# Algorithmic-Alignment-Lab/sco_py

Measured on AMD Instinct MI355X. Metric: SCO iters/sec (batch of N trajopt QPs), higher is better.
Workload: dtype f64

## Files before the change

### include/sco_hip.h

```cpp
#ifndef SCO_HIP_H
#define SCO_HIP_H

#ifdef __cplusplus
extern "C" {
#endif

#define SCO_OK              0
#define SCO_ERR_ARG        -1
#define SCO_ERR_DEVICE     -2
#define SCO_ERR_NO_GPU     -3
#define SCO_ERR_STATE      -4
#define SCO_ERR_CAPACITY   -5

#define SCO_QP_SOLVED                 1
#define SCO_QP_SOLVED_INACCURATE      2
#define SCO_QP_MAX_ITER_REACHED      -2
#define SCO_QP_PRIMAL_INFEASIBLE     -3
#define SCO_QP_PRIMAL_INFEASIBLE_INACCURATE 3
#define SCO_QP_DUAL_INFEASIBLE       -4
#define SCO_QP_DUAL_INFEASIBLE_INACCURATE   4
#define SCO_QP_NON_CVX               -7
#define SCO_QP_UNSOLVED             -10

const char *sco_last_error(void);
int sco_version(void);
int sco_device_count(int *count);


typedef struct sco_qp_settings {
  double rho;
  double sigma;
  double alpha;
  double eps_abs;
  double eps_rel;
  double eps_prim_inf;
  double eps_dual_inf;
  int max_iter;
  int check_termination;
  int scaling;
  int warm_start;
  int adaptive_rho;
  int adaptive_rho_interval;
  double adaptive_rho_tolerance;
} sco_qp_settings;

void sco_qp_default_settings(sco_qp_settings *s);

typedef struct sco_qp sco_qp;

int sco_qp_create(int device, int batch, int n, int m,
                  const int *P_colptr, const int *P_rowidx,
                  const int *A_colptr, const int *A_rowidx,
                  sco_qp **out);
int sco_qp_destroy(sco_qp *qp);

int sco_qp_load(sco_qp *qp, const double *P_val, const double *q,
                const double *A_val, const double *l, const double *u,
                const int *row_weight);

int sco_qp_set_bounds(sco_qp *qp, const double *l, const double *u);

int sco_qp_solve(sco_qp *qp, const sco_qp_settings *settings,
                 double *x, double *y, int *status, int *iters, double *resid);

int sco_qp_info(const sco_qp *qp, int info[4]);

int sco_qp_adaptive_info(sco_qp *qp, double *rho, int *updates);

int sco_qp_last_timing(const sco_qp *qp, double ms[2]);

#define SCO_QP_POLISH_OK       1
#define SCO_QP_POLISH_FAILED  -1
#define SCO_QP_POLISH_NOT_RUN  0
typedef struct sco_qp_polish_settings {
  double delta;
  int refine_iter;
} sco_qp_polish_settings;
void sco_qp_default_polish_settings(sco_qp_polish_settings *s);
int sco_qp_polish(sco_qp *qp, const sco_qp_polish_settings *s,
                  double *x, double *y, int *polish_status, double *resid);


typedef struct sco_sqp_params {
  double improve_ratio_threshold;
  double min_trust_region_size;
  double min_approx_improve;
  double trust_shrink_ratio;
  double trust_expand_ratio;
  double cnt_tolerance;
  double merit_coeff_increase_ratio;
  double initial_trust_region_size;
  double initial_penalty_coeff;
  int max_merit_coeff_increases;
  int compound_penalty;
  int duplicate_rows;
  int max_sqp_iters;
  int memoize_rounded;
  int warm_start_qps;
  int admm_slice;
} sco_sqp_params;

void sco_sqp_default_params(sco_sqp_params *p);

#define SCO_FAM_ARM_CIRCLES 1
#define SCO_FAM_ARM_REACH 2
#define SCO_FAM_POINT_CIRCLES 3
#define SCO_FAM_STATE_QUADRATIC 4
#define SCO_FAM_STATE_PROGRAM 5
#define SCO_OP_END 0
#define SCO_OP_X 1
#define SCO_OP_P 2
#define SCO_OP_C 3
#define SCO_OP_ADD 4
#define SCO_OP_SUB 5
#define SCO_OP_MUL 6
#define SCO_OP_DIV 7
#define SCO_OP_NEG 8
#define SCO_OP_SIN 9
#define SCO_OP_COS 10
#define SCO_OP_SQRT 11
#define SCO_OP_EXP 12
#define SCO_OP_SQUARE 13
#define SCO_PROGRAM_STACK 16
#define SCO_FAM_ARM_SPATIAL 7

#define SCO_FAM_FLAG_VEL_LIMITS 16
#define SCO_FAM_FLAG_JOINT_LIMITS 32
#define SCO_FAM_FLAG_EE_COST 64

#define SCO_FAM_FLAG_OBJ_PROGRAM 128

#define SCO_FAM_FLAG_ACC_COST 256

#define SCO_FAM_FLAG_OBJ_BLOCK 512

#define SCO_FAM_FLAG_OBJ_WIDE 1024

typedef struct sco_trajopt_desc {
  int batch;
  int dof;
  int horizon;
  int n_points;
  int n_obstacles;
  int family;
  int analytic_jac;
  int prox_count;
  int span;
  int n_eq_rows;
} sco_trajopt_desc;

typedef struct sco_sqp sco_sqp;

int sco_sqp_create(int device, const sco_trajopt_desc *desc, sco_sqp **out);
int sco_sqp_create_rows(int device, const sco_trajopt_desc *desc, int n_rows, const int *row_ptr, const int *col_idx,
                        const int *row_is_eq, sco_sqp **out);
int sco_sqp_load_linear_rows(sco_sqp *h, const double *vals, const double *rhs);
int sco_sqp_set_circle_rows(sco_sqp *h, int n_rows);
int sco_sqp_destroy(sco_sqp *h);

int sco_sqp_load(sco_sqp *h, const double *x0, const double *start, const double *goal,
                 const double *link_len, const int *point_link, const double *point_frac,
                 const double *obstacles);
int sco_sqp_load_target(sco_sqp *h, const double *target);
int sco_sqp_load_quadratic(sco_sqp *h, const double *Q, const double *a, const double *c);
int sco_sqp_load_spatial(sco_sqp *h,
    const double *joint_off,
    const double *joint_axis,
    const double *point_pos,
    const double *point_rad,
    const double *spheres);
int sco_sqp_load_program(sco_sqp *h, int n_words, const int *words, const int *row_ptr, int n_consts, const double *consts,
                         int n_params, const double *params);
int sco_sqp_load_program_steps(sco_sqp *h, int n_words, const int *words, const int *row_ptr, int n_consts, const double *consts,
                               int n_params, const double *params);
int sco_sqp_load_obj_weights(sco_sqp *h, const double *w);
int sco_sqp_load_acc_weights(sco_sqp *h, const double *a);
int sco_sqp_load_vel_limit(sco_sqp *h, const double *vmax);
int sco_sqp_load_joint_limits(sco_sqp *h, const double *lo, const double *hi);
int sco_sqp_load_ee_cost(sco_sqp *h, const double *weight, const double *target);

int sco_sqp_set_groups(sco_sqp *h, int n_groups, const unsigned int *block_mask);
int sco_sqp_fetch_groups(sco_sqp *h, unsigned int *nonconverged);
int sco_sqp_fetch_stalled_groups(sco_sqp *h, unsigned int *stalled);

int sco_sqp_solve(sco_sqp *h, const sco_sqp_params *params, const sco_qp_settings *qp_settings);

int sco_sqp_fetch(sco_sqp *h, double *x, int *success, int *sqp_iters, int *qp_solves,
                  long long *admm_iters, double *merit, double *max_violation);

#define SCO_SQP_FLAG_MEMO_FULL 1
#define SCO_SQP_FLAG_CAPPED 2
#define SCO_SQP_FLAG_TRACE_FULL 4
int sco_sqp_fetch_flags(sco_sqp *h, int *flags);
int sco_sqp_last_rounds(const sco_sqp *h, int *rounds);
int sco_sqp_last_launches(const sco_sqp *h, int *launches, int *groups);

int sco_sqp_last_tiers(const sco_sqp *h, double ms[2], long long iters[2], int launches[2]);

int sco_debug_sqp_mixed(const sco_sqp *h, int out[2]);
int sco_debug_mix_split(int live, int cus, int xcds, int slack, int per_cu);

int sco_debug_wv_gres_slot(int nstep, int pos, int out[5]);

int sco_debug_sqp_schedule(const int in[12], int plan[20], const int round_in[3], int round_out[8]);
int sco_debug_stage_sweep(int n, const double *begin_ms, const double *end_ms, const int *stage, double ms[5]);

int sco_debug_sqp_layout(const sco_trajopt_desc *desc, int n_rows, const int *row_ptr, const int *col_idx, const int *row_is_eq,
                         int dims[22], int sizes[15], int *ints, double *vals);
int sco_debug_sqp_check_program(const sco_trajopt_desc *desc, int n_circle_rows, int n_words, const int *words, const int *row_ptr,
                                int n_consts, int n_params);

int sco_debug_qp_launch_plan(const int *in, const double *tol, int *out);
int sco_debug_plan_tiers(int *mask);

int sco_debug_lanes(int device, int op, const double *a, const double *b, double *out_a, double *out_b);

int sco_sqp_trace(sco_sqp *h, int cap, double *trace, int *n_entries);

int sco_sqp_last_timing(const sco_sqp *h, double ms[5]);

#ifdef __cplusplus
}
#endif
#endif
```

### sco_py_amd/_lib.py

```python
import ctypes as C
import os

import numpy as np

from . import _build

SCO_OK = 0
ERR_NAMES = {-1: "SCO_ERR_ARG", -2: "SCO_ERR_DEVICE", -3: "SCO_ERR_NO_GPU",
             -4: "SCO_ERR_STATE", -5: "SCO_ERR_CAPACITY"}


class ScoHipError(RuntimeError):
    def __init__(self, code, msg):
        super().__init__("%s (%d): %s" % (ERR_NAMES.get(code, "SCO_ERR"), code, msg))
        self.code = code


class QpSettings(C.Structure):
    _fields_ = [
        ("rho", C.c_double), ("sigma", C.c_double), ("alpha", C.c_double),
        ("eps_abs", C.c_double), ("eps_rel", C.c_double),
        ("eps_prim_inf", C.c_double), ("eps_dual_inf", C.c_double),
        ("max_iter", C.c_int), ("check_termination", C.c_int), ("scaling", C.c_int),
        ("warm_start", C.c_int), ("adaptive_rho", C.c_int), ("adaptive_rho_interval", C.c_int),
        ("adaptive_rho_tolerance", C.c_double),
    ]


class PolishSettings(C.Structure):
    _fields_ = [("delta", C.c_double), ("refine_iter", C.c_int)]


class SqpParams(C.Structure):
    _fields_ = [
        ("improve_ratio_threshold", C.c_double), ("min_trust_region_size", C.c_double),
        ("min_approx_improve", C.c_double), ("trust_shrink_ratio", C.c_double),
        ("trust_expand_ratio", C.c_double), ("cnt_tolerance", C.c_double),
        ("merit_coeff_increase_ratio", C.c_double), ("initial_trust_region_size", C.c_double),
        ("initial_penalty_coeff", C.c_double),
        ("max_merit_coeff_increases", C.c_int), ("compound_penalty", C.c_int),
        ("duplicate_rows", C.c_int), ("max_sqp_iters", C.c_int),
        ("memoize_rounded", C.c_int), ("warm_start_qps", C.c_int), ("admm_slice", C.c_int),
    ]


class TrajoptDesc(C.Structure):
    _fields_ = [
        ("batch", C.c_int), ("dof", C.c_int), ("horizon", C.c_int), ("n_points", C.c_int),
        ("n_obstacles", C.c_int), ("family", C.c_int), ("analytic_jac", C.c_int),
        ("prox_count", C.c_int), ("span", C.c_int), ("n_eq_rows", C.c_int),
    ]


_DP = C.POINTER(C.c_double)
_IP = C.POINTER(C.c_int)
_LP = C.POINTER(C.c_longlong)

ABI = {
    "sco_last_error": (C.c_char_p, []),
    "sco_version": (C.c_int, []),
    "sco_device_count": (C.c_int, [_IP]),
    "sco_qp_default_settings": (None, [C.POINTER(QpSettings)]),
    "sco_qp_create": (C.c_int, [C.c_int, C.c_int, C.c_int, C.c_int, _IP, _IP, _IP, _IP, C.POINTER(C.c_void_p)]),
    "sco_qp_destroy": (C.c_int, [C.c_void_p]),
    "sco_qp_load": (C.c_int, [C.c_void_p, _DP, _DP, _DP, _DP, _DP, _IP]),
    "sco_qp_set_bounds": (C.c_int, [C.c_void_p, _DP, _DP]),
    "sco_qp_solve": (C.c_int, [C.c_void_p, C.POINTER(QpSettings), _DP, _DP, _IP, _IP, _DP]),
    "sco_qp_info": (C.c_int, [C.c_void_p, _IP]),
    "sco_qp_adaptive_info": (C.c_int, [C.c_void_p, _DP, _IP]),
    "sco_qp_last_timing": (C.c_int, [C.c_void_p, _DP]),
    "sco_qp_default_polish_settings": (None, [C.POINTER(PolishSettings)]),
    "sco_qp_polish": (C.c_int, [C.c_void_p, C.POINTER(PolishSettings), _DP, _DP, _IP, _DP]),
    "sco_sqp_default_params": (None, [C.POINTER(SqpParams)]),
    "sco_sqp_create": (C.c_int, [C.c_int, C.POINTER(TrajoptDesc), C.POINTER(C.c_void_p)]),
    "sco_sqp_create_rows": (C.c_int, [C.c_int, C.POINTER(TrajoptDesc), C.c_int, _IP, _IP, _IP, C.POINTER(C.c_void_p)]),
    "sco_sqp_destroy": (C.c_int, [C.c_void_p]),
    "sco_sqp_load": (C.c_int, [C.c_void_p, _DP, _DP, _DP, _DP, _IP, _DP, _DP]),
    "sco_sqp_load_target": (C.c_int, [C.c_void_p, _DP]),
    "sco_sqp_load_quadratic": (C.c_int, [C.c_void_p, _DP, _DP, _DP]),
    "sco_sqp_load_spatial": (C.c_int, [C.c_void_p, _DP, _DP, _DP, _DP, _DP]),
    "sco_sqp_load_program": (C.c_int, [C.c_void_p, C.c_int, _IP, _IP, C.c_int, _DP, C.c_int, _DP]),
    "sco_sqp_load_program_steps": (C.c_int, [C.c_void_p, C.c_int, _IP, _IP, C.c_int, _DP, C.c_int, _DP]),
    "sco_sqp_load_obj_weights": (C.c_int, [C.c_void_p, _DP]),
    "sco_sqp_load_acc_weights": (C.c_int, [C.c_void_p, _DP]),
    "sco_sqp_load_linear_rows": (C.c_int, [C.c_void_p, _DP, _DP]),
    "sco_sqp_set_circle_rows": (C.c_int, [C.c_void_p, C.c_int]),
    "sco_sqp_load_vel_limit": (C.c_int, [C.c_void_p, _DP]),
    "sco_sqp_load_joint_limits": (C.c_int, [C.c_void_p, _DP, _DP]),
    "sco_sqp_load_ee_cost": (C.c_int, [C.c_void_p, _DP, _DP]),
    "sco_sqp_set_groups": (C.c_int, [C.c_void_p, C.c_int, C.POINTER(C.c_uint)]),
    "sco_sqp_fetch_groups": (C.c_int, [C.c_void_p, C.POINTER(C.c_uint)]),
    "sco_sqp_fetch_stalled_groups": (C.c_int, [C.c_void_p, C.POINTER(C.c_uint)]),
    "sco_sqp_fetch_flags": (C.c_int, [C.c_void_p, _IP]),
    "sco_sqp_last_rounds": (C.c_int, [C.c_void_p, _IP]),
    "sco_sqp_last_launches": (C.c_int, [C.c_void_p, _IP, _IP]),
    "sco_sqp_last_tiers": (C.c_int, [C.c_void_p, _DP, _LP, _IP]),
    "sco_debug_sqp_mixed": (C.c_int, [C.c_void_p, _IP]),
    "sco_debug_mix_split": (C.c_int, [C.c_int, C.c_int, C.c_int, C.c_int, C.c_int]),
    "sco_debug_wv_gres_slot": (C.c_int, [C.c_int, C.c_int, _IP]),
    "sco_debug_sqp_schedule": (C.c_int, [_IP, _IP, _IP, _IP]),
    "sco_debug_stage_sweep": (C.c_int, [C.c_int, _DP, _DP, _IP, _DP]),
    "sco_debug_sqp_layout": (C.c_int, [C.POINTER(TrajoptDesc), C.c_int, _IP, _IP, _IP, _IP, _IP, _IP, _DP]),
    "sco_debug_sqp_check_program": (C.c_int, [C.POINTER(TrajoptDesc), C.c_int, C.c_int, _IP, _IP, C.c_int, C.c_int]),
    "sco_debug_qp_launch_plan": (C.c_int, [_IP, _DP, _IP]),
    "sco_debug_plan_tiers": (C.c_int, [_IP]),
    "sco_debug_lanes": (C.c_int, [C.c_int, C.c_int, _DP, _DP, _DP, _DP]),
    "sco_sqp_solve": (C.c_int, [C.c_void_p, C.POINTER(SqpParams), C.POINTER(QpSettings)]),
    "sco_sqp_fetch": (C.c_int, [C.c_void_p, _DP, _IP, _IP, _IP, _LP, _DP, _DP]),
    "sco_sqp_trace": (C.c_int, [C.c_void_p, C.c_int, _DP, _IP]),
    "sco_sqp_last_timing": (C.c_int, [C.c_void_p, _DP]),
}

_lib = None


def lib_path():
    return _build.LIB


def load():
    global _lib
    if _lib is not None:
        return _lib
    path = lib_path()
    if not os.path.exists(path):
        raise ScoHipError(-3, "libsco_hip.so not built (%s); run `python __graft_entry__.py` "
                              "or sco_py_amd._build.build() -- there is no CPU fallback" % path)
    lib = C.CDLL(path)
    for name, (res, args) in ABI.items():
        fn = getattr(lib, name)
        fn.restype = res
        fn.argtypes = args
    _lib = lib
    return lib


def check(code):
    if code != SCO_OK:
        msg = load().sco_last_error()
        raise ScoHipError(code, msg.decode() if msg else "")


def dptr(a):
    return None if a is None else a.ctypes.data_as(_DP)


def iptr(a):
    return None if a is None else a.ctypes.data_as(_IP)


def device_count():
    n = C.c_int(0)
    check(load().sco_device_count(C.byref(n)))
    return n.value


def default_qp_settings(**kw):
    s = QpSettings()
    load().sco_qp_default_settings(C.byref(s))
    for k, v in kw.items():
        if not hasattr(s, k):
            raise TypeError("unknown QP setting %r" % k)
        setattr(s, k, v)
    return s


def default_polish_settings(**kw):
    s = PolishSettings()
    load().sco_qp_default_polish_settings(C.byref(s))
    for k, v in kw.items():
        if not hasattr(s, k):
            raise TypeError("unknown polish setting %r" % k)
        setattr(s, k, v)
    return s


def default_sqp_params(**kw):
    p = SqpParams()
    load().sco_sqp_default_params(C.byref(p))
    for k, v in kw.items():
        if not hasattr(p, k):
            raise TypeError("unknown SQP parameter %r" % k)
        setattr(p, k, v)
    return p


class BatchedQP(object):

    def __init__(self, batch, n, m, Pp, Pi, Ap, Ai, device=0):
        self._h = C.c_void_p()
        self.batch, self.n, self.m = int(batch), int(n), int(m)
        self._pat = [np.ascontiguousarray(a, dtype=np.int32) for a in (Pp, Pi, Ap, Ai)]
        self.nnzP, self.nnzA = int(self._pat[0][-1]), int(self._pat[2][-1])
        check(load().sco_qp_create(device, self.batch, self.n, self.m,
                                   iptr(self._pat[0]), iptr(self._pat[1]),
                                   iptr(self._pat[2]), iptr(self._pat[3]), C.byref(self._h)))

    def close(self):
        if self._h:
            load().sco_qp_destroy(self._h)
            self._h = C.c_void_p()

    def __del__(self):
        try:
            self.close()
        except Exception:
            pass

    def _arr(self, a, shape, dtype=np.float64):
        a = np.ascontiguousarray(a, dtype=dtype)
        if a.shape != shape:
            raise ValueError("expected shape %r, got %r" % (shape, a.shape))
        return a

    def load(self, Pval, q, Aval, l, u, row_weight=None):
        B = self.batch
        Pval = self._arr(Pval, (B, self.nnzP)); q = self._arr(q, (B, self.n))
        Aval = self._arr(Aval, (B, self.nnzA)); l = self._arr(l, (B, self.m)); u = self._arr(u, (B, self.m))
        w = None if row_weight is None else self._arr(row_weight, (B, self.m), np.int32)
        check(load().sco_qp_load(self._h, dptr(Pval), dptr(q), dptr(Aval), dptr(l), dptr(u), iptr(w)))

    def set_bounds(self, l, u):
        l = self._arr(l, (self.batch, self.m)); u = self._arr(u, (self.batch, self.m))
        check(load().sco_qp_set_bounds(self._h, dptr(l), dptr(u)))

    def solve(self, settings=None):
        st = settings if settings is not None else default_qp_settings()
        B = self.batch
        x = np.zeros((B, self.n)); y = np.zeros((B, max(self.m, 1)))
        status = np.zeros(B, dtype=np.int32); iters = np.zeros(B, dtype=np.int32)
        resid = np.zeros((B, 2))
        check(load().sco_qp_solve(self._h, C.byref(st), dptr(x), dptr(y), iptr(status), iptr(iters), dptr(resid)))
        return x, y[:, : self.m], status, iters, resid

    def polish(self, settings=None):
        st = settings if settings is not None else default_polish_settings()
        B = self.batch
        x = np.zeros((B, self.n)); y = np.zeros((B, max(self.m, 1)))
        pstat = np.zeros(B, dtype=np.int32); resid = np.zeros((B, 2))
        check(load().sco_qp_polish(self._h, C.byref(st), dptr(x), dptr(y), iptr(pstat), dptr(resid)))
        return x, y[:, : self.m], pstat, resid

    def polish_info(self):
        lib = load()
        lib.sco_debug_polish_info.restype = C.c_int
        lib.sco_debug_polish_info.argtypes = [C.c_void_p, _DP, _IP]
        ms = np.zeros(4); k = np.zeros(self.batch, dtype=np.int32)
        check(lib.sco_debug_polish_info(self._h, dptr(ms), iptr(k)))
        return dict(active_ms=float(ms[0]), assemble_ms=float(ms[1]), factor_ms=float(ms[2]), solve_ms=float(ms[3])), k

    def info(self):
        out = np.zeros(4, dtype=np.int32)
        check(load().sco_qp_info(self._h, iptr(out)))
        return dict(n_elim=int(out[0]), n_core=int(out[1]), lds_admm=int(out[2]), ncpl=int(out[3]))

    def adaptive_info(self):
        rho = np.zeros(self.batch); upd = np.zeros(self.batch, dtype=np.int32)
        check(load().sco_qp_adaptive_info(self._h, dptr(rho), iptr(upd)))
        return rho, upd

    def last_timing(self):
        ms = np.zeros(2)
        check(load().sco_qp_last_timing(self._h, dptr(ms)))
        return dict(setup_ms=float(ms[0]), admm_ms=float(ms[1]))
```

### sco_py_amd/csrc/layout_wv.h

```cpp
#pragma once
#include "layout_qp.h"

#define WV_T 64
#define WV_MAXNS 4
#define WV_MAXNV 4
#ifndef WV_JREG
#define WV_JREG 1
#endif
SCO_HD constexpr bool wv_jreg(int NS, int BS) { return WV_JREG && NS * BS <= 28; }

SCO_HD inline size_t wv_tri(int i, int j) { return (size_t)i * (i + 1) / 2 + j; }

SCO_HD inline int wv_vidx(int npos, int pos, int k) { return (k >> 1) * 2 * npos + 2 * pos + (k & 1); }
SCO_HD inline int wv_gidx(int nstep, int pos, int i, int c) { return 64 * pos + 16 * (((c >> 1) + (pos > nstep ? 1 : 0)) & 3) + 2 * i + (c & 1); }

struct WvGresSlot { int pair, row, slot, vidx, eidx; };
SCO_HD inline WvGresSlot wv_gres_slot(int nstep, int pos) {
  const int hs = (nstep + 1) / 2, npos = 2 * nstep + 2;
  WvGresSlot s = {-1, -1, -1, -1, -1};
  if (pos < 0 || pos > 2 * nstep) return s;
  if (pos == nstep) { s.pair = 1; s.row = 0; s.slot = hs; }
  else {
    const int chain = pos > nstep ? 1 : 0, st = pos - (chain ? nstep + 1 : 0);
    s.pair = st >= hs ? 1 : 0; s.row = chain; s.slot = st - (s.pair ? hs : 0);
  }
  s.vidx = wv_vidx(npos, pos, 0); s.eidx = pos * 8;
  return s;
}
struct WvTab {
  int pos, hrow, hbrow, hevar, heidx, hepos, hbpos, hjpos, vvar, vrow, vpos, vpk, vpkm, vpkp, vpd, vpm, vpp, xrow, xpos, xpk, total;
  int lrow, lplo, lphi;
};
SCO_HD inline WvTab wv_tab_layout(int NS, int NV, int NL = 0) {
  WvTab t; int o = 0;
  t.pos = o; o += 1;
  t.hrow = o; o += NS; t.hbrow = o; o += NS; t.hevar = o; o += NS; t.heidx = o; o += NS; t.hepos = o; o += NS; t.hbpos = o; o += NS;
  t.hjpos = o; o += NS * 8;
  t.vvar = o; o += NV; t.vrow = o; o += NV; t.vpos = o; o += NV; t.vpk = o; o += NV; t.vpkm = o; o += NV; t.vpkp = o; o += NV;
  t.vpd = o; o += NV * 8; t.vpm = o; o += NV; t.vpp = o; o += NV;
  t.xrow = o; o += 1; t.xpos = o; o += 1; t.xpk = o; o += 1;
  t.lrow = o; o += NV * NL; t.lplo = o; o += NV * NL; t.lphi = o; o += NV * NL;
  t.total = o;
  return t;
}
SCO_HD inline int wv_cst_h(int q) { return 3 * q; }
SCO_HD inline int wv_cst_v(int NS, int v) { return 3 * NS + 13 * v; }
SCO_HD inline int wv_cst_x(int NS, int NV) { return 3 * NS + 13 * NV; }
SCO_HD inline int wv_cst_l(int NS, int NV, int i) { return 3 * NS + 13 * NV + 1 + i; }
SCO_HD constexpr int wv_cst_slots(int NS, int NV, int nl) { return 3 * NS + 13 * NV + 1 + nl; }
SCO_HD constexpr int wv_ck_h(int q) { return 3 * q; }
SCO_HD constexpr int wv_ck_v(int NS, int v) { return 3 * NS + 5 * v; }
SCO_HD constexpr int wv_ck_x(int NS, int NV) { return 3 * NS + 5 * NV; }
SCO_HD constexpr int wv_ck_slots(int NS, int NV) { return 3 * NS + 5 * NV + 1; }
SCO_HD constexpr bool wv_link_regs(int BS) { return BS != 7; }
```

### sco_py_amd/csrc/qp_debug.cpp

```cpp
#include "qp_tier_plans.h"
#include "layout_fast.h"
#include "layout_wv.h"

#include <algorithm>
#include <cstring>

static QpPlan g_dbg_plan;
extern "C" int sco_debug_plan_build(int n, int m, const int *Pp, const int *Pi, const int *Ap, const int *Ai,
                                    int allow_elim, int *sizes) {
  int rc = qp_plan_build(n, m, Pp, Pi, Ap, Ai, allow_elim, g_dbg_plan);
  if (rc) return SCO_ERR_ARG;
  const QpPlan &p = g_dbg_plan;
  sizes[0] = p.n_e; sizes[1] = p.n_c; sizes[2] = p.ncpl; sizes[3] = p.nS;
  sizes[4] = (int)p.cp_row.size(); sizes[5] = (int)p.sa_row.size(); sizes[6] = (int)p.ss_k1.size();
  sizes[7] = (int)p.Fi.size();
  return SCO_OK;
}
extern "C" int sco_debug_rl_plan(int *info) {
  RlHost rh;
  const bool ok = rl_plan_build(g_dbg_plan, rh, qp_create_env());
  info[0] = ok ? 1 : 0; info[1] = rh.CW; info[2] = rh.TR; info[3] = rh.TC; info[4] = (int)rh.lds_bytes; info[5] = rh.merged ? 1 : 0; info[6] = rh.aligned ? 1 : rh.lay8 ? 2 : 0; info[7] = rh.NS;
  return SCO_OK;
}
extern "C" int sco_debug_fast_plan(int *info) {
  FastHost fh;
  const bool ok = fast_plan_build(g_dbg_plan, fh);
  const int nq = fast_rows_per_thread(g_dbg_plan.m);
  info[0] = ok ? 1 : 0; info[1] = fh.TR; info[2] = fh.TC; info[3] = (fh.capped && nq == 2) ? 1 : 0; info[4] = nq; info[5] = (int)fh.lds_bytes;
  return SCO_OK;
}
extern "C" int sco_debug_reg_plan(int *info) {
  RegHost rh;
  int CW = 0, RW = 0, PX = 0;
  const bool ok = reg_caps_for(g_dbg_plan, &CW, &RW, &PX) && reg_plan_build(g_dbg_plan, CW, RW, PX, rh);
  info[0] = ok ? 1 : 0; info[1] = rh.TR; info[2] = rh.TC; info[3] = rh.CW; info[4] = rh.RW; info[5] = rh.PX; info[6] = (int)rh.lds_bytes;
  return SCO_OK;
}
static bool dbg_wv_plan(bool allow_links, int *info, WvHost &wh) {
  const bool ok = wv_plan_build(g_dbg_plan, wh, allow_links);
  info[0] = ok ? 1 : 0; info[1] = wh.bs; info[2] = wh.nb; info[3] = wh.lpb; info[4] = wh.BS; info[5] = wh.NS; info[6] = wh.NV;
  info[7] = wh.NSTEP; info[8] = (int)wh.lds_bytes; info[9] = wh.n_extra;
  return ok;
}
extern "C" int sco_debug_wv_plan(int *info) {
  WvHost wh;
  dbg_wv_plan(false, info, wh);
  return SCO_OK;
}
extern "C" int sco_debug_wv_link_plan(int *info) {
  WvHost wh;
  dbg_wv_plan(true, info, wh);
  info[10] = wh.n_link; info[11] = wh.NL; info[12] = wh.per_cu; info[13] = wh.why;
  return SCO_OK;
}
extern "C" int sco_debug_wv_stack_plan(int *info) {
  WvHost wh;
  dbg_wv_plan(true, info, wh);
  info[10] = wh.n_link; info[11] = wh.NL; info[12] = wh.per_cu; info[13] = wh.why; info[14] = wh.n_stack;
  return SCO_OK;
}
extern "C" int sco_debug_bt_plan(int *info) {
  BigHost bh; BtHost th;
  const bool ok = g_dbg_plan.n_c <= 1024 && big_plan_build(g_dbg_plan, bh) && bt_plan_build(g_dbg_plan, bh, th, qp_create_env().no_mfma);
  info[0] = ok ? 1 : 0; info[1] = th.bs; info[2] = th.nb; info[3] = th.use_mfma ? 1 : 0; info[4] = th.mf_why; info[5] = (int)th.lds_bytes;
  return SCO_OK;
}
extern "C" int sco_debug_plan_tiers(int *mask) {
  const QpPlan &p = g_dbg_plan;
  if (!mask || p.n <= 0) return SCO_ERR_ARG;
  QpTiers t;
  std::string err;
  if (const int rc = qp_choose_tiers(p.n, p.m, p.Pp.data(), p.Pi.data(), p.Ap.data(), p.Ai.data(), qp_create_env(), t, &err)) {
    sco_set_error(err);
    return rc;
  }
  *mask = qp_tier_mask(t);
  return SCO_OK;
}
extern "C" int sco_debug_plan_get(const char *name, int *out, int cap) {
  const QpPlan &p = g_dbg_plan;
  const std::vector<int> *v = nullptr;
#define F(x) if (!strcmp(name, #x)) v = &p.x;
  F(Rp) F(Rj) F(Rpos) F(Fp) F(Fi) F(Fpos) F(Pdiag) F(elim_var) F(core_var) F(elim_of) F(core_of)
  F(e_ptr) F(pair_core) F(pair_elim) F(cp_ptr) F(cp_row) F(cp_pa) F(cp_pe) F(a_ptr) F(a_pair)
  F(s_a) F(s_b) F(s_ppos) F(sa_ptr) F(sa_row) F(sa_pa) F(sa_pb) F(ss_ptr) F(ss_k1) F(ss_k2) F(ss_e)
#undef F
  if (!v) return SCO_ERR_ARG;
  if ((int)v->size() > cap) return SCO_ERR_CAPACITY;
  std::copy(v->begin(), v->end(), out);
  return (int)v->size();
}
extern "C" int sco_debug_wv_gres_slot(int nstep, int pos, int out[5]) {
  if (!out || nstep <= 0) return SCO_ERR_ARG;
  const WvGresSlot s = wv_gres_slot(nstep, pos);
  out[0] = s.pair; out[1] = s.row; out[2] = s.slot; out[3] = s.vidx; out[4] = s.eidx;
  return SCO_OK;
}
```

### sco_py_amd/csrc/qp_tier.cpp

```cpp
#include "qp_tier.h"

#include <algorithm>
#include <climits>
#include <cstdlib>

QpCreateEnv qp_create_env() {
  auto on = [](const char *name) { const char *v = getenv(name); return v && v[0] == '1'; };
  QpCreateEnv e;
  e.factor_cholesky = on("SCO_QP_FACTOR_CHOLESKY"); e.no_elim = on("SCO_QP_NO_ELIM");
  e.force_big = on("SCO_QP_FORCE_BIG"); e.no_bt = on("SCO_QP_NO_BT");
  e.no_rl = on("SCO_QP_NO_RL"); e.no_wv = on("SCO_QP_NO_WV"); e.no_reg = on("SCO_QP_NO_REG"); e.no_fast = on("SCO_QP_NO_FAST");
  e.no_mfma = on("SCO_QP_NO_MFMA");
  e.rl_closed = on("SCO_QP_RL_ALIGNED") || on("SCO_QP_RL_CLOSED"); e.rl_lay8 = on("SCO_QP_RL_LAY8");
  { const char *v = getenv("SCO_QP_RL_SPLIT"); e.rl_split_off = v && v[0] == '0'; }
  e.debug_plan = getenv("SCO_DEBUG_PLAN") != nullptr;
  return e;
}

int sco_wv_min_live(int cus, bool adaptive) {
  const char *e = getenv("SCO_WV_MIN_PER_CU");
  if (!e && adaptive) return INT_MAX;
  const double live = (e ? atof(e) : 2.75) * (cus > 0 ? cus : 256);
  return live >= (double)INT_MAX ? INT_MAX : (int)live;
}

int sco_qp_adaptive_interval(const sco_qp_settings *st) {
  if (st->adaptive_rho_interval > 0) {
    if (st->check_termination > 0)
      return std::max(1, (st->adaptive_rho_interval + st->check_termination / 2) / st->check_termination) * st->check_termination;
    return st->adaptive_rho_interval;
  }
  return st->check_termination > 0 ? 4 * st->check_termination : 100;
}

const char *qp_launch_err_text(int err) {
  switch (err) {
    case QP_ERR_WINDOW: return "sco_qp_launch_sliced: launch window not supported by this handle's tier";
    case QP_ERR_ADAPT_DENSE: return "adaptive_rho: the dense form of the global-memory tier cannot park a solve";
    case QP_ERR_ADAPT_SETTINGS: return "adaptive_rho needs adaptive_rho_tolerance > 1 and check_termination > 0";
    case QP_ERR_MIXED: return "sco_qp_launch_sliced: mixed round not supported by this handle or its side window is malformed";
  }
  return "";
}

bool qp_supports_windows(const QpLaunchIn &in) {
  if (in.adaptive_rho) return false;
  if (in.use_big) return in.use_bt;
  return in.kern == QP_K_RL && !in.factor_cholesky;
}

static QpLaunchPlan plan_error(QpLaunchPlan p, int rc, int err) { p.rc = rc; p.err = err; return p; }

QpLaunchPlan qp_launch_plan(const QpLaunchIn &in) {
  QpLaunchPlan p;
  const bool adaptive = in.adaptive_rho != 0;
  if (in.window && (!qp_supports_windows(in) || in.b0 < 0 || in.nb <= 0 || in.b0 + in.nb > in.batch))
    return plan_error(p, SCO_ERR_STATE, QP_ERR_WINDOW);
  if (adaptive) {
    if (in.use_big && !in.use_bt) return plan_error(p, SCO_ERR_CAPACITY, QP_ERR_ADAPT_DENSE);
    if (!(in.adaptive_rho_tolerance > 1.0) || in.check_termination <= 0) return plan_error(p, SCO_ERR_ARG, QP_ERR_ADAPT_SETTINGS);
  }
  const bool can_park = in.use_big ? in.use_bt : true;
  if (!can_park || in.check_termination <= 0 || (in.slice <= 0 && !adaptive)) {
    p.slice = 0;
  } else {
    const int want = in.slice <= 0 ? in.max_iter : in.slice;
    p.slice = std::max(1, (want + in.check_termination - 1) / in.check_termination) * in.check_termination;
  }
  p.nwg = in.window ? in.nb : in.batch;
  if (adaptive) {
    sco_qp_settings st{};
    st.adaptive_rho_interval = in.adaptive_rho_interval; st.check_termination = in.check_termination;
    p.ad_interval = sco_qp_adaptive_interval(&st);
  }
  p.mixed = in.window && in.tier == 3;
  if (p.mixed) {
    const bool at_end = in.side_b0 == in.b0 || in.side_b0 + in.side_nb == in.b0 + in.nb;
    if (!in.use_wv || in.kern != QP_K_RL || adaptive || p.slice <= 0 || !in.has_list || in.side_nb <= 0 || in.side_nb >= in.nb ||
        !at_end || in.side_slices <= 0 || !in.side_ready)
      return plan_error(p, SCO_ERR_STATE, QP_ERR_MIXED);
  }
  p.wv_now = in.use_wv && !(adaptive && in.wv_links) && (in.window && in.tier ? in.tier >= 2 : p.nwg >= in.wv_min);
  p.rho_init = adaptive && in.mask != QP_MASK_NONE;
  p.route = in.use_big ? (in.use_bt ? QP_ROUTE_BIG_BT : QP_ROUTE_BIG_DENSE) : QP_ROUTE_ONCHIP;
  if (p.route != QP_ROUTE_ONCHIP) { p.wv_now = false; return p; }
  p.need = p.wv_now ? (p.mixed ? QP_NEED_SIDE : QP_NEED_NONE) : (in.use_wv ? QP_NEED_WINDOW : QP_NEED_NONE);
  p.cholesky = in.factor_cholesky;
  const int nb4 = (in.n_c + 3) / 4, ntiles = nb4 * (nb4 + 1) / 2;
  p.sweep_nt = ntiles <= SCO_FACTOR_BLOCK ? 1 : ntiles <= 2 * SCO_FACTOR_BLOCK ? 2 : 3;
  switch (in.kern) {
    case QP_K_RL: p.admm = p.mixed ? QP_ADMM_MIXED : p.wv_now ? QP_ADMM_WV_RL : QP_ADMM_RL; break;
    case QP_K_REG: p.admm = QP_ADMM_REG; break;
    case QP_K_FAST: p.admm = QP_ADMM_FAST; break;
    default: p.admm = QP_ADMM_GENERIC;
  }
  return p;
}

// ... 21 lines not shown
```

### sco_py_amd/csrc/qp_tier.h

```cpp
#pragma once
#include "../../include/sco_hip.h"

#define SCO_FACTOR_BLOCK 1024

struct QpCreateEnv {
  bool factor_cholesky = false;
  bool no_elim = false;
  bool force_big = false;
  bool no_bt = false;
  bool no_rl = false, no_wv = false, no_reg = false, no_fast = false;
  bool no_mfma = false;
  bool rl_closed = false;
  bool rl_lay8 = false;
  bool rl_split_off = false;
  bool debug_plan = false;
};
QpCreateEnv qp_create_env();

int sco_wv_min_live(int cus, bool adaptive = false);
int sco_qp_adaptive_interval(const sco_qp_settings *st);

enum QpKernel { QP_K_RL = 0, QP_K_REG = 1, QP_K_FAST = 2, QP_K_GENERIC = 3 };
enum QpMaskKind { QP_MASK_ARRAY = 0, QP_MASK_ALL = 1, QP_MASK_NONE = 2 };

struct QpLaunchIn {
  int kern = QP_K_GENERIC;
  bool use_big = false, use_bt = false;
  bool use_wv = false;
  bool wv_links = false;
  bool factor_cholesky = false;
  int batch = 0, n_c = 0;
  int cus = 0;
  int adaptive_rho = 0, adaptive_rho_interval = 0, check_termination = 0, max_iter = 0;
  double adaptive_rho_tolerance = 0.0;
  int slice = 0;
  int mask = QP_MASK_ARRAY;
  int wv_min = 0;
  bool window = false;
  int b0 = 0, nb = 0, tier = 0;
  bool has_list = false;
  int side_b0 = 0, side_nb = 0, side_slices = 0;
  bool side_ready = false;
};

enum QpLaunchErr { QP_ERR_NONE = 0, QP_ERR_WINDOW, QP_ERR_ADAPT_DENSE, QP_ERR_ADAPT_SETTINGS, QP_ERR_MIXED };
const char *qp_launch_err_text(int err);
enum QpRoute { QP_ROUTE_BIG_DENSE = 0, QP_ROUTE_BIG_BT = 1, QP_ROUTE_ONCHIP = 2 };
enum QpNeed { QP_NEED_NONE = 0, QP_NEED_WINDOW = 1, QP_NEED_SIDE = 2 };
enum QpAdmmSeq { QP_ADMM_GENERIC = 0, QP_ADMM_FAST, QP_ADMM_REG, QP_ADMM_RL, QP_ADMM_WV_RL, QP_ADMM_MIXED };

struct QpLaunchPlan {
  int rc = SCO_OK, err = QP_ERR_NONE;
  int slice = -1;
  int nwg = 0;
  int ad_interval = 0;
  bool rho_init = false;
  int route = QP_ROUTE_ONCHIP;
  bool wv_now = false, mixed = false;
  int need = QP_NEED_NONE;
  bool cholesky = false;
  int sweep_nt = 1;
  int admm = QP_ADMM_GENERIC;
};
QpLaunchPlan qp_launch_plan(const QpLaunchIn &in);
bool qp_supports_windows(const QpLaunchIn &in);
```

### sco_py_amd/csrc/qp_tier_plans.h

```cpp
#pragma once
#include <cstddef>
#include <string>
#include <vector>

#include "../../include/sco_hip.h"
#include "layout_qp.h"
#include "qp_plan.h"
#include "qp_tier.h"

void sco_set_error(const std::string &msg);

struct SellHost {
  int nitems = 0, total = 0;
  std::vector<int> base, width, src;
  std::vector<unsigned short> idx;
};
struct FastHost { SellHost Ac, Ar, Ca, Ce; int TR = 1, TC = 2; bool capped = false; size_t lds_doubles = 0, lds_bytes = 0; };
bool fast_plan_build(const QpPlan &pl, FastHost &fh);

struct RegHost {
  int TR = 1, TC = 2, CW = 0, RW = 0, PX = 0;
  SellHost Ac, Ar, Ca, Ce;
  size_t lds_bytes = 0;
  std::vector<int> role;
  std::vector<unsigned short> off;
};
int reg_caps_for(const QpPlan &pl, int *CW, int *RW, int *PX);
size_t reg_static_lds();
bool reg_plan_build(const QpPlan &pl, int CW, int RW, int PX, RegHost &rh);

struct RlHost {
  int TR = 1, TC = 2, CW = 12;
  int pcw = 0;
  int zpos = 0;
  bool merged = false;
  bool aligned = false;
  bool split = false;
  bool lay8 = false;
  int NS = 2;
  SellHost Ac, Ar[3];
  size_t lds_bytes = 0;
  std::vector<unsigned short> off;
  std::vector<int> role, pc_ptr, pc_pos, pc_core;
};
size_t rl_reported_static_lds();
bool rl_plan_build(const QpPlan &pl, RlHost &rh, const QpCreateEnv &env);

#define SCO_WV_PER_CU 4
struct WvHost {
  int bs = 0, nb = 0, mid = 0, lpb = 0, n_extra = 0;
  int BS = 8, NS = 1, NV = 1, NSTEP = 4;
  int cst_slots = 0;
  size_t g_doubles = 0, lds_doubles = 0, lds_bytes = 0;
  std::vector<int> tab;
  int n_link = 0, NL = 0, per_cu = SCO_WV_PER_CU, why = 0;
  int n_stack = 0;
};
#define WV_NL 2
enum WvWhy { WV_OK = 0, WV_WHY_OTHER = 1, WV_WHY_LINKS_OFF = 2, WV_WHY_THIRD_LINK = 3, WV_WHY_SAME_BLOCK = 4, WV_WHY_FAR_BLOCKS = 5,
             WV_WHY_INDEX = 6, WV_WHY_THREE_CORE = 7, WV_WHY_LDS = 8, WV_WHY_SHAPE = 9,
             WV_WHY_STACKED = 10 };
bool wv_plan_build(const QpPlan &pl, WvHost &wh, bool allow_links);

struct BigHost {
  std::vector<int> row_elim, row_epos, er_ptr, er_row, free_rows, pc_ptr, pc_pos, pc_core;
  size_t ws_doubles = 0;
};
bool big_plan_build(const QpPlan &pl, BigHost &bh);
struct BtHost {
  int bs = 0, nb = 0, nchunks = 0, npart = 0;
  bool use_part = false;
  std::vector<int> cent;
  size_t blk_doubles = 0, ws_doubles = 0, lds_bytes = 0;
  std::vector<int> ch_desc, it;
  bool use_mfma = false;
  int mf_why = 0;
  std::vector<int> mf_id, mf_h0, mf_h1;
};
bool bt_plan_build(const QpPlan &pl, const BigHost &bh, BtHost &th, bool no_mfma);

struct QpTiers {
  QpPlan plan;
  size_t lds_setup = 0, lds_admm = 0;
  bool factor_cholesky = false;
  bool use_big = false, use_bt = false;
  int kern = QP_K_GENERIC;
  bool use_wv = false;
  BigHost big;
  BtHost bt;
  RlHost rl;
  WvHost wv;
  RegHost reg;
  FastHost fast;
};
int qp_choose_tiers(int n, int m, const int *Pp, const int *Pi, const int *Ap, const int *Ai, const QpCreateEnv &env, QpTiers &t,
                    std::string *err);
int qp_tier_mask(const QpTiers &t);
```

### sco_py_amd/csrc/sco_admm_wv.hip

```cpp
#include <algorithm>
#include <cstdio>
#include <cstdlib>
#include <cstring>
#include <type_traits>

#include "sco_admm_check.h"
#include "layout_wv.h"

#ifndef WV_PD
#define WV_PD 3
#endif
typedef double d2 __attribute__((ext_vector_type(2)));

#ifndef WV_KEEP
#define WV_KEEP 8
#endif
#ifndef WV_VARIANT
#define WV_VARIANT 0
#endif
#ifndef WV_GRES
#define WV_GRES 1
#endif
#ifndef WV_ROWS_EARLY
#define WV_ROWS_EARLY 1
#endif
#ifndef WV_MV_INIT
#define WV_MV_INIT 1
#endif
#ifndef WV_HANDOVER
#define WV_HANDOVER 1
#endif
#if WV_VARIANT == 1
#define WV_FMAC_DPP(acc, w, g, k) asm("v_fmac_f64 %0, %1, %2" : "+v"(acc) : "v"(w), "v"(g))
#endif

__device__ __forceinline__ double wv_recip(double x) { return x != 0.0 ? __builtin_amdgcn_rcp(x) : 0.0; }

int wv_upload(const WvHost &wh, int batch, int n, int m, std::vector<void *> &allocs, WvDev &wd) {
  void *p = nullptr;
  SCO_HIP(hipMalloc(&p, wh.tab.size() * sizeof(int))); allocs.push_back(p);
  SCO_HIP(hipMemcpy(p, wh.tab.data(), wh.tab.size() * sizeof(int), hipMemcpyHostToDevice)); wd.tab = (const int *)p;
  SCO_HIP(hipMalloc(&p, (size_t)batch * wh.g_doubles * sizeof(double))); allocs.push_back(p); wd.G = (double *)p;
  SCO_HIP(hipMalloc(&p, (size_t)batch * wh.cst_slots * 64 * sizeof(double))); allocs.push_back(p); wd.cst = (double *)p;
  SCO_HIP(hipMalloc(&p, (size_t)batch * sizeof(double))); allocs.push_back(p); wd.wc = (double *)p;
  SCO_HIP(hipMalloc(&p, (size_t)batch * sizeof(int))); allocs.push_back(p); wd.ok = (int *)p;
  SCO_HIP(hipMemset(p, 0, (size_t)batch * sizeof(int)));
  SCO_HIP(hipMalloc(&p, (size_t)batch * sizeof(int))); allocs.push_back(p); wd.rl_need = (int *)p;
  SCO_HIP(hipMemset(p, 0, (size_t)batch * sizeof(int)));
  SCO_HIP(hipMalloc(&p, sizeof(unsigned long long))); allocs.push_back(p); wd.it_count = (unsigned long long *)p;
  SCO_HIP(hipMemset(p, 0, sizeof(unsigned long long)));
  SCO_HIP(hipMalloc(&p, (size_t)batch * sizeof(int))); allocs.push_back(p); wd.pflag = (int *)p;
  SCO_HIP(hipMemset(p, 0, (size_t)batch * sizeof(int)));
  SCO_HIP(hipMalloc(&p, (size_t)batch * sizeof(int))); allocs.push_back(p); wd.w_ready = (int *)p;
  SCO_HIP(hipMemset(p, 0, (size_t)batch * sizeof(int)));
  SCO_HIP(hipMalloc(&p, (size_t)batch * (size_t)(n + m) * sizeof(double))); allocs.push_back(p); wd.scr = (double *)p;
  return SCO_OK;
}

struct WvArgs {
  int n, m, n_e, n_c, nnzA, nnzP, max_iter, check, slice;
  int b0; const int *list;
  int bs, nb, mid, lpb, n_extra, NS, NV, NSTEP, cst_slots, NL; size_t g_doubles;
  double rho, sigma, alpha, eps_abs, eps_rel, eps_prim_inf, eps_dual_inf;
  const int *tab;
  double *G, *cst, *wc, *scr; int *ok, *rl_need, *w_ready, *pflag; unsigned long long *it_count;
  const double *As, *Ps, *qs, *ls, *us, *rhov, *kee_inv, *cscale, *D, *E, *S;
  const int *w, *active, *setup_active;
  const int *Ap, *Ai, *Rp, *Rj, *Rpos, *Fp, *Fi, *Fpos;
  double *x, *y, *resid; int *status, *iters, *prog;
  double *sx, *sz, *sy, *st, *sg;
  int ablate;
  int warm, ad_interval; double ad_tol; double *rho_b; int *rflag, *smask, *nupd;
};

__device__ __forceinline__ double wv_wmax(double v) { return wave_reduce_all<true>(v); }
__device__ __forceinline__ double wv_wsum(double v) { return wave_reduce_all<false>(v); }
template <bool DIRECT>
__device__ __forceinline__ void wv_meet(double vlast, int chain, double &vA, double &vB) {
  if (DIRECT) {
    vA = vlast; vB = vlast;
    lane_swap<16>(vA, vB);
  } else {
    lane_u2 lo, hi;
    lane_swap_halves<16>(vlast, vlast, lo, hi);
    const double vother = chain ? __hiloint2double((int)hi.x, (int)lo.x) : __hiloint2double((int)hi.y, (int)lo.y);
    vA = chain ? vother : vlast; vB = chain ? vlast : vother;
  }
}
#define WV_BIG (SCO_INFTY * SCO_MIN_SCALING)

template <int LNK>
__global__ __launch_bounds__(WV_T) void qp_wv_factor_kernel(WvArgs a) {
  const int g = blockIdx.x, lane = threadIdx.x;
  const int b = a.list ? a.list[g + a.b0] : g + a.b0;
  if (b < 0) return;
  if (a.setup_active && !a.setup_active[b]) { if (lane == 0) a.rl_need[b] = 0; return; }
  const int n = a.n, m = a.m, bs = a.bs, nb = a.nb, mid = a.mid, NS = a.NS, NV = a.NV, NSTEP = a.NSTEP;
  const WvTab T = wv_tab_layout(NS, NV, LNK);
  const int *tab = a.tab;
  const double *ls = a.ls + (size_t)b * m, *us = a.us + (size_t)b * m, *rho = a.rhov + (size_t)b * m;
  const int *w = a.w + (size_t)b * m;
  const double *D = a.D + (size_t)b * n, *E = a.E + (size_t)b * m, *Ps = a.Ps + (size_t)b * a.nnzP;
  double *cst = a.cst + (size_t)b * a.cst_slots * 64;
  const double rho_base = a.rho_b ? a.rho_b[b] : a.rho;
  int bad = 0, wk = 0, offd = 0;
  for (int q = 0; q < NS; q++) { const int h = tab[(T.hrow + q) * 64 + lane]; if (h >= 0) wk = max(wk, w[h]); }
  wk = (int)wv_wmax((double)wk);
  for (int q = 0; q < NS; q++) {
    const int h = tab[(T.hrow + q) * 64 + lane], br = tab[(T.hbrow + q) * 64 + lane], ev = tab[(T.hevar + q) * 64 + lane];
    double eh = 0.0, eb = 0.0, de = 0.0;
    if (h >= 0) {
      if (!(ls[h] < -WV_BIG) || rho[h] != rho_base || w[h] != wk) bad = 1;
      if (!(us[br] > WV_BIG) || ls[br] != 0.0 || rho[br] != rho_base || w[br] != 1) bad = 1;
      eh = E[h]; eb = E[br]; de = D[ev];
    }
    double *c = cst + (size_t)wv_cst_h(q) * 64 + lane;
    c[0] = h >= 0 ? 1.0 / eh : 0.0; c[64] = h >= 0 ? 1.0 / eb : 0.0; c[128] = h >= 0 ? 1.0 / de : 0.0;
  }
  for (int v = 0; v < NV; v++) {
    const int var = tab[(T.vvar + v) * 64 + lane], r0 = tab[(T.vrow + v) * 64 + lane];
    double *c = cst + (size_t)wv_cst_v(NS, v) * 64 + lane;
    if (r0 >= 0 && (rho[r0] != rho_base || w[r0] != 1)) bad = 1;
    c[0] = var >= 0 ? 1.0 / D[var] : 0.0;
    c[64] = r0 >= 0 ? 1.0 / E[r0] : 0.0;
    const int pm = tab[(T.vpm + v) * 64 + lane], pp = tab[(T.vpp + v) * 64 + lane];
    c[2 * 64] = pm >= 0 ? Ps[pm] : 0.0; c[3 * 64] = pp >= 0 ? Ps[pp] : 0.0;
    const int kown = (tab[(T.vpk + v) * 64 + lane] / (2 * (2 * NSTEP + 2)) << 1) | (tab[(T.vpk + v) * 64 + lane] & 1);
    double pdiag = 0.0;
    for (int k = 0; k < 8; k++) {
      const int pd = tab[(T.vpd + v * 8 + k) * 64 + lane];
      const double pv = pd >= 0 ? Ps[pd] : 0.0;
      c[(5 + k) * 64] = pv;
      if (var >= 0 && k == kown) pdiag = pv; else if (var >= 0 && pv != 0.0) offd = 1;
    }
    c[4 * 64] = pdiag;
  }
  {
    const int xr = tab[T.xrow * 64 + lane];
    double *c = cst + (size_t)wv_cst_x(NS, NV) * 64 + lane;
    c[0] = xr >= 0 ? 1.0 / E[xr] : 0.0;
  }
  if constexpr (LNK > 0) {
    for (int i = 0; i < NV * LNK; i++) {
      const int lr = tab[(T.lrow + i) * 64 + lane];
      if (lr >= 0 && (rho[lr] != rho_base || w[lr] != 1)) bad = 1;
      cst[(size_t)wv_cst_l(NS, NV, i) * 64 + lane] = lr >= 0 ? 1.0 / E[lr] : 0.0;
    }
  }
  bad = (int)wv_wmax((double)bad); offd = (int)wv_wmax((double)offd);
  if (lane == 0) a.pflag[b] = offd;
  if (lane == 0) { a.ok[b] = !bad; a.rl_need[b] = bad; a.w_ready[b] = bad; a.wc[b] = (double)wk; }
  if (bad) return;
  const double *S = a.S + (size_t)b * a.n_c * a.n_c;
  double *G = a.G + (size_t)b * a.g_doubles;
  const int npos = 2 * NSTEP + 2;
  double *ef = G + (size_t)npos * 64, *en = ef + npos * 8, *em = en + npos * 8;
  for (size_t t = lane; t < a.g_doubles; t += WV_T) G[t] = 0.0;
  __threadfence_block(); __syncthreads();
  const int i = lane >> 3, j = lane & 7;
  auto Sblk = [&](int t) -> double {
    if (i >= bs || j >= bs) return i == j ? 1.0 : 0.0;
    const int ca = t * bs + max(i, j), cb = t * bs + min(i, j);
    return S[wv_tri(ca, cb)];
  };
  auto Soff = [&](int t, int k) -> double {
    return (k < bs && t >= 0 && t + 1 < nb) ? S[wv_tri((t + 1) * bs + k, t * bs + k)] : 0.0;
  };
  auto invert = [&](double M) -> double {
    for (int p = 0; p < 8; p++) {
      const double piv = __shfl(M, p * 8 + p), rowp = __shfl(M, p * 8 + j), colp = __shfl(M, i * 8 + p);
      const double inv = 1.0 / piv;
      if (i == p && j == p) M = inv;
      else if (i == p) M = rowp * inv;
      else if (j == p) M = -colp * inv;
      else M = M - colp * rowp * inv;
    }
    return M;
  };
  double Gmid_corr = 0.0;
  for (int chain = 0; chain < 2; chain++) {
    const int len = chain ? nb - 1 - mid : mid, p0 = chain ? 2 * NSTEP + 1 - len : NSTEP - len;
    double Gp = 0.0;
    for (int s = 0; s < len; s++) {
      const int t = chain ? nb - 1 - s : s, p = p0 + s;
      const int tl = chain ? t : t - 1;
      const double ei = s > 0 ? Soff(tl, i) : 0.0, ej = s > 0 ? Soff(tl, j) : 0.0;
      const double M = Sblk(t) - ei * Gp * ej;
      Gp = invert(M);
      G[wv_gidx(NSTEP, p, i, j)] = Gp;
      const int tn = chain ? t - 1 : t;
      if (lane < 8) { ef[p * 8 + lane] = s > 0 ? Soff(tl, lane) : 0.0; en[p * 8 + lane] = Soff(tn, lane); }
    }
    if (len > 0) {
      const int tl = chain ? mid : mid - 1;
      Gmid_corr += Soff(tl, i) * Gp * Soff(tl, j);
    }
  }
// ... 5 lines not shown
}


__device__ __forceinline__ double wv_min(double a, double b) { double r; asm("v_min_f64 %0, %1, %2" : "=v"(r) : "v"(a), "v"(b)); return r; }
__device__ __forceinline__ double wv_max(double a, double b) { double r; asm("v_max_f64 %0, %1, %2" : "=v"(r) : "v"(a), "v"(b)); return r; }

template <int BS> struct WvRow { d2 a, b, c; d2 d; };
template <int BS>
__device__ __forceinline__ WvRow<BS> wv_row(const double *p, const double *pd) {
  WvRow<BS> r;
  r.a = *(const d2 *)p; r.b = *(const d2 *)(p + 16); r.c = *(const d2 *)(p + 32);
  if (BS > 7) r.d = *(const d2 *)pd; else { r.d.x = pd[0]; r.d.y = 0.0; }
  return r;
}

#define WV_DPP_STEP(acc, g, k) "v_fmac_f64_dpp " acc ", %2, " g " row_newbcast:" #k " row_mask:0xf bank_mask:0xf\n\t"
#define WV_DPP_CHAIN7 WV_DPP_STEP("%0", "%3", 0) WV_DPP_STEP("%1", "%4", 1) WV_DPP_STEP("%0", "%5", 2) WV_DPP_STEP("%1", "%6", 3) \
                      WV_DPP_STEP("%0", "%7", 4) WV_DPP_STEP("%1", "%8", 5) WV_DPP_STEP("%0", "%9", 6)
#define WV_G7 "v"(g0.x), "v"(g0.y), "v"(g1.x), "v"(g1.y), "v"(g2.x), "v"(g2.y), "v"(g3.x)

template <int BS, bool ZERO, bool INIT>
__device__ __forceinline__ double wv_matvec(double init, double w, const WvRow<BS> &g) {
  const d2 g0 = g.a, g1 = g.b, g2 = g.c, g3 = g.d;
#if WV_VARIANT == 1
  double acc = ZERO ? 0.0 : init, acc2 = 0.0;
  WV_FMAC_DPP(acc, w, g0.x, 0); WV_FMAC_DPP(acc2, w, g0.y, 1);
  WV_FMAC_DPP(acc, w, g1.x, 2); WV_FMAC_DPP(acc2, w, g1.y, 3);
  WV_FMAC_DPP(acc, w, g2.x, 4); WV_FMAC_DPP(acc2, w, g2.y, 5); WV_FMAC_DPP(acc, w, g3.x, 6);
  if (BS > 7) WV_FMAC_DPP(acc2, w, g3.y, 7);
#else
  double acc = ZERO ? 0.0 : init, acc2 = 0.0;
  if (!INIT) {
    if (BS > 7) asm("s_nop 1\n\t" WV_DPP_CHAIN7 WV_DPP_STEP("%1", "%10", 7) : "+v"(acc), "+v"(acc2) : "v"(w), WV_G7, "v"(g3.y));
    else asm("s_nop 1\n\t" WV_DPP_CHAIN7 : "+v"(acc), "+v"(acc2) : "v"(w), WV_G7);
  } else if (BS > 7) {
    if (ZERO) asm("v_mov_b64 %1, 0\n\tv_mov_b64 %0, 0\n\t" WV_DPP_CHAIN7 WV_DPP_STEP("%1", "%10", 7) : "=&v"(acc), "=&v"(acc2) : "v"(w), WV_G7, "v"(g3.y));
    else asm("v_mov_b64 %1, 0\n\tv_mov_b64 %0, %11\n\t" WV_DPP_CHAIN7 WV_DPP_STEP("%1", "%10", 7) : "=&v"(acc), "=&v"(acc2) : "v"(w), WV_G7, "v"(g3.y), "v"(init));
  } else {
    if (ZERO) asm("v_mov_b64 %1, 0\n\tv_mov_b64 %0, 0\n\t" WV_DPP_CHAIN7 : "=&v"(acc), "=&v"(acc2) : "v"(w), WV_G7);
    else asm("v_mov_b64 %1, 0\n\tv_mov_b64 %0, %10\n\t" WV_DPP_CHAIN7 : "=&v"(acc), "=&v"(acc2) : "v"(w), WV_G7, "v"(init));
  }
#endif
  return acc + acc2;
}
#undef WV_G7
#undef WV_DPP_CHAIN7
#undef WV_DPP_STEP

#define WV_SYNC() do { __builtin_amdgcn_fence(__ATOMIC_ACQ_REL, "wavefront"); __builtin_amdgcn_wave_barrier(); } while (0)

template <typename T>
__device__ __forceinline__ const T *wv_opaque(const T *p) { asm volatile("" : "+v"(p)); return p; }

template <int NV, int LNK, bool REG> struct WvLinks {
  static constexpr int N = NV * LNK;
  double alo[REG ? N : 1], ahi[REG ? N : 1], l[REG ? N : 1], u[REG ? N : 1], z[N], y[N], d[N], xp[NV];
  double *lkl;
  __device__ __forceinline__ void consts(int v, double (&la)[LNK], double (&lh)[LNK], double (&ll)[LNK], double (&lu)[LNK]) const {
#pragma unroll
    for (int s = 0; s < LNK; s++) {
      const int i = v * LNK + s;
      if constexpr (REG) { la[s] = alo[i]; lh[s] = ahi[i]; ll[s] = l[i]; lu[s] = u[i]; }
      else {
        const d2 ca = *(const d2 *)(lkl + (2 * i) * 128), cb = *(const d2 *)(lkl + (2 * i + 1) * 128);
        la[s] = ca.x; lh[s] = ca.y; ll[s] = cb.x; lu[s] = cb.y;
      }
    }
  }
};
template <int NV, bool REG> struct WvLinks<NV, 0, REG> {};

constexpr bool wv_gres_fits(int BS, int NS, int NV, int NSTEP, int LPB, int EXT) {
  return WV_GRES != 0 && NSTEP % 2 == 0 && !(BS == 7 && (EXT & 2));
}
constexpr bool wv_rows_early(int BS, int NS, int NV, int NSTEP, int LPB, int EXT, int LNK) {
  return WV_ROWS_EARLY != 0 && LNK == 0 && LPB > 0 && !(EXT & 2);
}
constexpr int wv_slots(int BS, int NS, int NV, int NSTEP, int LPB, int EXT, int LNK) {
  int sl = (WV_MV_INIT ? 1 : 0) | (WV_HANDOVER ? 4 : 0);
  if (LNK > 0) sl &= 1;
  if (BS == 7 && LPB == 3 && EXT == 1) sl &= 4;
  return sl;
}
template <int BS, int NS, int NV, int NSTEP, int LPB, int EXT, int LNK>
__global__ __launch_bounds__(WV_T) void qp_admm_wv_kernel(WvArgs a) {
  constexpr bool ADAPT = (EXT & 2) != 0;
  static_assert(!(LNK > 0 && ADAPT), "adaptive rho on link patterns stays on the row-local kernel (qp_launch_plan)");
  constexpr int NLK = LNK > 0 ? NV * LNK : 1;
  constexpr bool LREG = wv_link_regs(BS);
  constexpr bool GRES = wv_gres_fits(BS, NS, NV, NSTEP, LPB, EXT);
  constexpr bool EARLY = wv_rows_early(BS, NS, NV, NSTEP, LPB, EXT, LNK);
  constexpr int SL = wv_slots(BS, NS, NV, NSTEP, LPB, EXT, LNK);
  constexpr int HS = (NSTEP + 1) / 2, H2 = NSTEP - HS;
  const int g = blockIdx.x, lane = threadIdx.x;
  const int b = a.list ? a.list[g + a.b0] : g + a.b0;
  if (b < 0 || (a.active && !a.active[b])) return;
  if (!a.ok[b]) return;
#ifdef WV_ABLATE
  const int ablate = a.ablate;
#else
  constexpr int ablate = 0;
#endif
  const int n = a.n, m = a.m, lpb = LPB > 0 ? LPB : a.lpb;
  constexpr int NPOS = 2 * NSTEP + 2;
  constexpr bool JREG = wv_jreg(NS, BS);
  constexpr int oG = 0, oEF = oG + NPOS * 64, oEN = oEF + NPOS * 8, oEM = oEN + NPOS * 8, oR = oEM + 8, oXT = oR + NPOS * 8,
                oXC = oXT + NPOS * 8, oEX = oXC + NPOS * 8, oLK = oEX + NPOS * 8, oJ = oLK + (LNK > 0 ? NPOS * 8 : 0),
                oPART = oJ + (JREG ? 0 : NS * 512);
  constexpr int NVEC = LNK > 0 ? 5 : 4;
  extern __shared__ __attribute__((aligned(16))) double lds[];
  const int *tab0 = a.tab;
  constexpr int oPOS = 0, oHROW = 1, oHBROW = oHROW + NS, oHEVAR = oHBROW + NS, oHEIDX = oHEVAR + NS, oHEPOS = oHEIDX + NS,
                oHBPOS = oHEPOS + NS, oHJPOS = oHBPOS + NS, oVVAR = oHJPOS + 8 * NS, oVROW = oVVAR + NV, oVPOS = oVROW + NV,
                oVPK = oVPOS + NV, oVPKM = oVPK + NV, oVPKP = oVPKM + NV, oXROW = oVPKP + NV + 8 * NV + 2 * NV, oXPOS = oXROW + 1,
                oXPK = oXPOS + 1, oLROW = oXPK + 1, oLPLO = oLROW + NV * LNK, oLPHI = oLPLO + NV * LNK;
  const double *As = a.As + (size_t)b * a.nnzA, *qs = a.qs + (size_t)b * n, *lsg = a.ls + (size_t)b * m, *usg = a.us + (size_t)b * m;
  const double *cstg0 = a.cst + (size_t)b * a.cst_slots * 64 + lane;
  double rho_in = a.rho;
  if constexpr (ADAPT) {
    rho_in = a.rho_b[b];
    if (lane == 0) { a.rflag[b] = 0; a.smask[b] = 0; }
  }
  const double rho0 = rho_in, rinv0 = 1.0 / rho0, wc = a.wc[b], rw = wc * rho0;
  const double sigma = a.sigma, alpha = a.alpha, oma = 1.0 - alpha;
  const double cscale = a.cscale[b], cinv = 1.0 / cscale;
  const int it0 = a.slice > 0 ? a.prog[b] : 0;
  const bool resume = it0 > 0;
  const double *sxg = a.sx + (size_t)b * n, *szg = a.sz + (size_t)b * m, *syg = a.sy + (size_t)b * m;

  {
    const double *Gg = a.G + (size_t)b * a.g_doubles;
    for (int t = lane; t < oR; t += WV_T) lds[t] = Gg[t];
    for (int t = lane; t < NVEC * NPOS * 8; t += WV_T) lds[oR + t] = 0.0;
    for (int t = lane; t < NPOS * lpb * 8; t += WV_T) lds[oPART + t] = 0.0;
  }
  constexpr bool CKG = LNK > 0 && !LREG;
  const int oCK = oPART + NPOS * lpb * 8;
  double *const ckl = lds + oCK + lane;
  if constexpr (!CKG) {
#pragma unroll
    for (int q = 0; q < NS; q++)
#pragma unroll
      for (int k = 0; k < 3; k++) ckl[(wv_ck_h(q) + k) * 64] = cstg0[(wv_cst_h(q) + k) * 64];
#pragma unroll
    for (int v = 0; v < NV; v++)
#pragma unroll
      for (int k = 0; k < 5; k++) ckl[(wv_ck_v(NS, v) + k) * 64] = cstg0[(wv_cst_v(NS, v) + k) * 64];
    ckl[wv_ck_x(NS, NV) * 64] = cstg0[wv_cst_x(NS, NV) * 64];
  }
#define CKH(q, k) (CKG ? wv_opaque(cstg0)[(wv_cst_h(q) + (k)) * 64] : ckl[(wv_ck_h(q) + (k)) * 64])
#define CKV(v, k) (CKG ? wv_opaque(cstg0)[(wv_cst_v(NS, v) + (k)) * 64] : ckl[(wv_ck_v(NS, v) + (k)) * 64])
#define CKX (CKG ? wv_opaque(cstg0)[wv_cst_x(NS, NV) * 64] : ckl[wv_ck_x(NS, NV) * 64])
#define CKL(i) wv_opaque(cstg0)[wv_cst_l(NS, NV, i) * 64]
  const int pos_r = tab0[oPOS * 64 + lane];
  double *const xt_p = lds + oXT + pos_r * 2;
  const int nslot2 = NPOS * lpb * 2;
  double *const part_p = lds + oPART + (pos_r * lpb + (lane & 15) % lpb) * 2;
  double *const jl_p = lds + oJ + lane * 2;
  bool h_on[NS];
  double h_ae[NS], h_ab[NS], h_u[NS], h_q[NS], h_kinv[NS], h_z[NS], h_y[NS], h_zb[NS], h_yb[NS], h_xe[NS], h_ge[NS];
  double hJ[JREG ? NS : 1][8];
#pragma unroll
  for (int q = 0; q < NS; q++) {
    const int h = tab0[(oHROW + q) * 64 + lane], br = tab0[(oHBROW + q) * 64 + lane], ev = tab0[(oHEVAR + q) * 64 + lane];
    const bool on = h >= 0;
    h_on[q] = on;
    h_ae[q] = on ? As[tab0[(oHEPOS + q) * 64 + lane]] : 0.0;
    h_ab[q] = on ? As[tab0[(oHBPOS + q) * 64 + lane]] : 0.0;
    h_u[q] = on ? usg[h] : 0.0;
    h_q[q] = on ? qs[ev] : 0.0;
    h_kinv[q] = on ? a.kee_inv[(size_t)b * a.n_e + tab0[(oHEIDX + q) * 64 + lane]] : 0.0;
    h_z[q] = on && resume ? szg[h] : 0.0; h_y[q] = on && resume ? syg[h] : 0.0;
    h_zb[q] = on && resume ? szg[br] : 0.0; h_yb[q] = on && resume ? syg[br] : 0.0;
    h_xe[q] = on && resume ? sxg[ev] : 0.0; h_ge[q] = 0.0;
#pragma unroll
    for (int k = 0; k < 4; k++) {
      const int j0 = on ? tab0[(oHJPOS + q * 8 + 2 * k) * 64 + lane] : -1, j1 = on ? tab0[(oHJPOS + q * 8 + 2 * k + 1) * 64 + lane] : -1;
      d2 v; v.x = j0 >= 0 ? As[j0] : 0.0; v.y = j1 >= 0 ? As[j1] : 0.0;
      if (JREG) { hJ[q][2 * k] = v.x; hJ[q][2 * k + 1] = v.y; }
      else *(d2 *)(jl_p + (q * 4 + k) * 128) = v;
    }
  }
  double *v_p[NV];
  const double *v_pp[NV];
  bool v_on[NV], v_r0on[NV];
  int v_pkm[NV], v_pkp[NV];
  double v_x[NV], v_q[NV], v_a[NV], v_l[NV], v_u[NV], v_z[NV], v_y[NV];
#pragma unroll
  for (int v = 0; v < NV; v++) {
    const int var = tab0[(oVVAR + v) * 64 + lane], r0 = tab0[(oVROW + v) * 64 + lane];
    const int vix = tab0[(oVPK + v) * 64 + lane], vk = ((vix / (2 * NPOS)) << 1) | (vix & 1), vpos = (vix % (2 * NPOS)) >> 1;
    v_on[v] = var >= 0; v_p[v] = lds + oXT + vix;
    v_pp[v] = lds + oPART + (vk >> 1) * nslot2 + vpos * lpb * 2 + (vk & 1);
    v_q[v] = var >= 0 ? qs[var] : 0.0; v_x[v] = var >= 0 && resume ? sxg[var] : 0.0;
    v_a[v] = r0 >= 0 ? As[tab0[(oVPOS + v) * 64 + lane]] : 0.0;
    v_l[v] = r0 >= 0 ? lsg[r0] : 0.0; v_u[v] = r0 >= 0 ? usg[r0] : 0.0;
    v_z[v] = r0 >= 0 && resume ? szg[r0] : 0.0; v_y[v] = r0 >= 0 && resume ? syg[r0] : 0.0;
    v_r0on[v] = r0 >= 0; v_pkm[v] = tab0[(oVPKM + v) * 64 + lane]; v_pkp[v] = tab0[(oVPKP + v) * 64 + lane];
  }
  const int x_row = tab0[oXROW * 64 + lane];
  double *const x_p = lds + oXT + tab0[oXPK * 64 + lane];
  const double x_a = x_row >= 0 ? As[tab0[oXPOS * 64 + lane]] : 0.0, x_l = x_row >= 0 ? lsg[x_row] : 0.0, x_u = x_row >= 0 ? usg[x_row] : 0.0;
  const double x_rho = x_row >= 0 ? a.rhov[(size_t)b * m + x_row] : 1.0, x_rinv = 1.0 / x_rho, x_w = x_row >= 0 ? (double)a.w[(size_t)b * m + x_row] : 0.0;
  double x_z = x_row >= 0 && resume ? szg[x_row] : 0.0, x_y = x_row >= 0 && resume ? syg[x_row] : 0.0;
  WvLinks<NV, LNK, LREG> lk;
  constexpr int NL1 = LNK > 0 ? LNK : 1;
  if constexpr (LNK > 0) {
    lk.lkl = lds + oCK + lane * 2;
#pragma unroll
    for (int i = 0; i < NLK; i++) {
      const int lr = tab0[(oLROW + i) * 64 + lane], lph = tab0[(oLPHI + i) * 64 + lane];
      d2 ca, cb;
      ca.x = lr >= 0 ? As[tab0[(oLPLO + i) * 64 + lane]] : 0.0; ca.y = lr >= 0 && lph >= 0 ? As[lph] : 0.0;
      cb.x = lr >= 0 ? lsg[lr] : 0.0; cb.y = lr >= 0 ? usg[lr] : 0.0;
      if constexpr (LREG) { lk.alo[i] = ca.x; lk.ahi[i] = ca.y; lk.l[i] = cb.x; lk.u[i] = cb.y; }
      else { *(d2 *)(lk.lkl + (2 * i) * 128) = ca; *(d2 *)(lk.lkl + (2 * i + 1) * 128) = cb; }
      lk.z[i] = lr >= 0 && resume ? szg[lr] : 0.0; lk.y[i] = lr >= 0 && resume ? syg[lr] : 0.0;
    }
  }
  const int srow = lane >> 4, k8 = lane & 7, chain = srow & 1, half = GRES ? srow >> 1 : 0;
  const bool sw_store = (GRES || srow < 2) && (lane & 15) < 8;
  const int pos0 = (chain ? NSTEP + 1 : 0) + half * HS;
  const WvGresSlot sl0 = wv_gres_slot(NSTEP, pos0);
  const double *const sw_g = lds + oG + pos0 * 64 + k8 * 2 + (chain ? 16 : 0);
  const double *const sw_gd = lds + oG + pos0 * 64 + k8 * 2 + (chain ? 0 : 48);
  double *const sw_v = lds + oR + sl0.vidx + wv_vidx(NPOS, 0, k8);
  const double *const sw_e = lds + oEF + sl0.eidx + k8;
  const double *const md_g = lds + oG + NSTEP * 64 + k8 * 2;
  double *const md_v = lds + oR + wv_vidx(NPOS, NSTEP, k8);
  const double *const md_e = lds + oEF + NSTEP * 8 + k8;
  WvRow<BS> gr[GRES ? HS : 1], gmd;
  auto load_g = [&]() {
    static_assert(!GRES || H2 == HS, "the second half recomputes the first on its idle rows: both halves need the same step count");
#pragma unroll
    for (int s = 0; s < HS; s++) gr[s] = wv_row<BS>(sw_g + s * 64, sw_gd + s * 64);
    gmd = wv_row<BS>(md_g, md_g + 48);
  };
  WV_SYNC();

  double c_ndy = 0.0, c_lhs = 0.0, c_ndx = 0.0, c_qdx = 0.0;
  const int pdense = (ablate & 32) ? 1 : a.pflag[b];
  struct { double h[NS], b[NS], e[NS], r0[NV], var[NV], x; } dsv;
  auto rows = [&](auto mode_tag) {
    constexpr int MODE = decltype(mode_tag)::value;
    double xt[8], xtx = 0.0, xtv[NV];
    if (MODE) {
      const d2 a0 = *(const d2 *)xt_p, a1 = *(const d2 *)(xt_p + 2 * NPOS), a2 = *(const d2 *)(xt_p + 4 * NPOS), a3 = *(const d2 *)(xt_p + 6 * NPOS);
      xtx = x_p[0];
#pragma unroll
      for (int v = 0; v < NV; v++) xtv[v] = v_p[v][0];
      xt[0] = a0.x; xt[1] = a0.y; xt[2] = a1.x; xt[3] = a1.y; xt[4] = a2.x; xt[5] = a2.y; xt[6] = a3.x; xt[7] = a3.y;
    }
    if constexpr (LNK > 0) {
      if (MODE) {
#pragma unroll
        for (int v = 0; v < NV; v++) lk.xp[v] = lds[oXT + v_pkp[v]];
      }
    }
    double part[8] = {0, 0, 0, 0, 0, 0, 0, 0};
    d2 jn0, jn1, jn2, jn3;
    if (!JREG) { const d2 *jp = (const d2 *)jl_p; jn0 = jp[0]; jn1 = jp[64]; jn2 = jp[128]; jn3 = jp[192]; }
#pragma unroll
    for (int q = 0; q < NS; q++) {
      double J[8];
      if (JREG) {
#pragma unroll
        for (int k = 0; k < 8; k++) J[k] = hJ[q][k];
      } else {
        J[0] = jn0.x; J[1] = jn0.y; J[2] = jn1.x; J[3] = jn1.y; J[4] = jn2.x; J[5] = jn2.y; J[6] = jn3.x; J[7] = jn3.y;
        if (q + 1 < NS) { const d2 *jp = (const d2 *)(jl_p + (q + 1) * 512); jn0 = jp[0]; jn1 = jp[64]; jn2 = jp[128]; jn3 = jp[192]; }
      }
      const double ae = h_ae[q], ab = h_ab[q], kinv = h_kinv[q];
      const double c2 = rw * ae;
      if (MODE) {
        double s = J[0] * xt[0];
#pragma unroll
        for (int k = 1; k < BS; k++) s = __builtin_fma(J[k], xt[k], s);
        const double xte = h_ge[q] - (kinv * c2) * s;
        const double zth = __builtin_fma(ae, xte, s), ztb = ab * xte;
        {
          const double zr = alpha * zth + oma * h_z[q];
          const double zn = wv_min(zr + rinv0 * h_y[q], h_u[q]);
          const double dy = rho0 * (zr - zn);
          h_y[q] += dy; h_z[q] = zn;
          if (MODE == 2) {
            const double dc = fmax(dy, 0.0);
            c_ndy = fmax(c_ndy, wv_recip(CKH(q, 0)) * fabs(dc)); c_lhs += wc * (h_u[q] * dc);
            dsv.h[q] = dc;
          }
        }
        {
          const double zr = alpha * ztb + oma * h_zb[q];
          const double zn = wv_max(zr + rinv0 * h_yb[q], 0.0);
          const double dy = rho0 * (zr - zn);
          h_yb[q] += dy; h_zb[q] = zn;
          if (MODE == 2) {
            const double dc = fmin(dy, 0.0);
            c_ndy = fmax(c_ndy, wv_recip(CKH(q, 1)) * fabs(dc));
            dsv.b[q] = dc;
          }
        }
        const double xo = h_xe[q], xn = alpha * xte + oma * xo;
        h_xe[q] = xn;
        if (MODE == 2) {
          const double dx = xn - xo;
          c_ndx = fmax(c_ndx, wv_recip(CKH(q, 2)) * fabs(dx)); c_qdx += h_q[q] * dx;
          dsv.e[q] = dx;
        }
      }
      const double th = wc * (rho0 * h_z[q] - h_y[q]);
      const double tb = rho0 * h_zb[q] - h_yb[q];
      const double rhs = ae * th + ab * tb + (sigma * h_xe[q] - h_q[q]);
      const double ge = rhs * kinv;
      h_ge[q] = ge;
      const double tp = th - c2 * ge;
#pragma unroll
      for (int k = 0; k < BS; k++) part[k] = __builtin_fma(J[k], tp, part[k]);
    }
    {
      d2 v0, v1, v2, v3;
      v0.x = part[0]; v0.y = part[1]; v1.x = part[2]; v1.y = part[3]; v2.x = part[4]; v2.y = part[5]; v3.x = part[6]; v3.y = BS > 7 ? part[7] : 0.0;
      *(d2 *)part_p = v0; *(d2 *)(part_p + nslot2) = v1; *(d2 *)(part_p + 2 * nslot2) = v2; *(d2 *)(part_p + 3 * nslot2) = v3;
    }
    {
      if (MODE) {
        const double xtc = xtx;
        const double zt = x_a * xtc, zr = alpha * zt + oma * x_z;
        const double zn = wv_min(wv_max(zr + x_rinv * x_y, x_l), x_u);
        const double dy = x_rho * (zr - zn);
        x_y += dy; x_z = zn;
        if (MODE == 2) {
          const double d1 = upper_is_infinite(x_u) ? fmin(dy, 0.0) : dy, dc = lower_is_infinite(x_l) ? fmax(d1, 0.0) : d1;
          c_ndy = fmax(c_ndy, wv_recip(CKX) * fabs(dc)); c_lhs += x_w * (x_u * fmax(dc, 0.0) + x_l * fmin(dc, 0.0));
          dsv.x = dc;
        }
      }
      const double t = x_w * (x_rho * x_z - x_y);
      if (x_row >= 0) x_p[oEX - oXT] = x_a * t;
    }
    double s_ex[NV], s_pt[NV][LPB > 0 ? LPB : 1];
    if constexpr (EARLY) {
      WV_SYNC();
#pragma unroll
      for (int v = 0; v < NV; v++) {
        s_ex[v] = v_p[v][oEX - oXT];
#pragma unroll
        for (int s2 = 0; s2 < LPB; s2++) s_pt[v][s2] = v_pp[v][s2 * 2];
      }
      __builtin_amdgcn_sched_barrier(0);
    }
    double own[NV];
#pragma unroll
    for (int v = 0; v < NV; v++) {
      if (MODE) {
        const double xtc = xtv[v];
        const double zt = v_a[v] * xtc, zr = alpha * zt + oma * v_z[v];
        const double zn = wv_min(wv_max(zr + rinv0 * v_y[v], v_l[v]), v_u[v]);
        const double dy = rho0 * (zr - zn);
        v_y[v] += dy; v_z[v] = zn;
        const double xo = v_x[v], xn = alpha * xtc + oma * xo;
        v_x[v] = xn;
        if (MODE == 2) {
          const double d1 = upper_is_infinite(v_u[v]) ? fmin(dy, 0.0) : dy, dc = lower_is_infinite(v_l[v]) ? fmax(d1, 0.0) : d1;
          if (v_r0on[v]) { c_ndy = fmax(c_ndy, wv_recip(CKV(v, 1)) * fabs(dc)); c_lhs += v_u[v] * fmax(dc, 0.0) + v_l[v] * fmin(dc, 0.0); }
          dsv.r0[v] = dc;
          const double dx = xn - xo;
          if (v_on[v]) { c_ndx = fmax(c_ndx, wv_recip(CKV(v, 0)) * fabs(dx)); c_qdx += v_q[v] * dx; }
          dsv.var[v] = dx;
        }
      }
      const double t0 = rho0 * v_z[v] - v_y[v];
      own[v] = v_a[v] * t0 + (sigma * v_x[v] - v_q[v]);
      if constexpr (LNK > 0) {
        double ps = 0.0, la[NL1], lh[NL1], ll[NL1], lu[NL1];
        lk.consts(v, la, lh, ll, lu);
#pragma unroll
        for (int s = 0; s < LNK; s++) {
          const int i = v * LNK + s;
          if (MODE) {
            const double zt = __builtin_fma(lh[s], lk.xp[v], la[s] * xtv[v]), zr = alpha * zt + oma * lk.z[i];
            const double zn = wv_min(wv_max(zr + rinv0 * lk.y[i], ll[s]), lu[s]);
            const double dy = rho0 * (zr - zn);
            lk.y[i] += dy; lk.z[i] = zn;
            if (MODE == 2) {
              const double d1 = upper_is_infinite(lu[s]) ? fmin(dy, 0.0) : dy, dc = lower_is_infinite(ll[s]) ? fmax(d1, 0.0) : d1;
              c_ndy = fmax(c_ndy, wv_recip(CKL(i)) * fabs(dc)); c_lhs += lu[s] * fmax(dc, 0.0) + ll[s] * fmin(dc, 0.0);
              lk.d[i] = dc;
            }
          }
          const double t = rho0 * lk.z[i] - lk.y[i];
          own[v] = __builtin_fma(la[s], t, own[v]); ps = __builtin_fma(lh[s], t, ps);
        }
        lds[oLK + v_pkp[v]] = ps;
      }
    }
    if constexpr (EARLY) __builtin_amdgcn_sched_barrier(0); else WV_SYNC();
    double rsum[NV];
#pragma unroll
    for (int v = 0; v < NV; v++) {
      double r = own[v] + (EARLY ? s_ex[v] : v_p[v][oEX - oXT]);
// ... 98 lines not shown
      const double rr = rq[i % PD], ee = eq[i % PD];
      fetch_fwd(i + PD, rq[i % PD], eq[i % PD]);
      const double w = __builtin_fma(-ee, vprev, rr);
      vprev = wv_matvec<BS, true, (SL & 1) != 0>(0.0, w, gr[s]);
      vs[s] = vprev;
    }
    const double emk = lds[oEM + k8], vlast = vprev;
    double vA, vB;
    wv_meet<(SL & 4) != 0>(vlast, chain, vA, vB);
    const double rm = rq[NSTEP % PD], em_ = eq[NSTEP % PD];
#pragma unroll
    for (int j = 0; j < PD; j++) fetch_bwd(j, eb[j]);
    double w = __builtin_fma(-em_, vA, rm);
    w = __builtin_fma(-emk, vB, w);
    double xn = wv_matvec<BS, true, (SL & 1) != 0>(0.0, w, gmd);
    double xmid = xn;
#pragma unroll
    for (int j = 0; j < NSTEP; j++) {
      if (j == H2) {
        double sx = xn, sy = (SL & 4) ? xmid : xn;
        lane_swap<32>(sx, sy);
        xn = (SL & 4) ? sy : (half ? xmid : sy);
        if (SL & 4) xmid = sy;
      }
      const int s = bslot(j);
      const double ee = eb[j % PD];
      fetch_bwd(j + PD, eb[j % PD]);
      const double u = -(ee * xn);
      xn = wv_matvec<BS, false, (SL & 1) != 0>(vs[s], u, gr[s]);
      xs[s] = xn;
    }
    if (sw_store) {
#pragma unroll
      for (int s = 0; s < HS; s++) sw_v[s * 2 + (oXT - oR)] = xs[s];
      if (srow == 2) md_v[oXT - oR] = xmid;
    }
    WV_SYNC();
  };
  auto sweep = [&]() { if constexpr (GRES) sweep_res(); else sweep_lds(); };

  if ((EXT & 1) && a.warm && !resume) {
    const double *Dg = a.D + (size_t)b * n, *Eg = a.E + (size_t)b * m;
    const double *xg = a.x + (size_t)b * n, *yg = a.y + (size_t)b * m;
#pragma unroll
    for (int v = 0; v < NV; v++) {
      const int var = tab0[(oVVAR + v) * 64 + lane], r0 = tab0[(oVROW + v) * 64 + lane];
      v_x[v] = var >= 0 ? xg[var] / Dg[var] : 0.0;
      v_z[v] = v_a[v] * v_x[v];
      v_y[v] = r0 >= 0 ? yg[r0] * cscale / Eg[r0] : 0.0;
      v_p[v][oXC - oXT] = v_x[v];
    }
    WV_SYNC();
    if (x_row >= 0) { x_z = x_a * x_p[oXC - oXT]; x_y = yg[x_row] * cscale / (Eg[x_row] * x_w); }
    if constexpr (LNK > 0) {
#pragma unroll
      for (int v = 0; v < NV; v++) {
        double la[NL1], lh[NL1], ll[NL1], lu[NL1];
        lk.consts(v, la, lh, ll, lu);
#pragma unroll
        for (int s = 0; s < LNK; s++) {
          const int i = v * LNK + s, lr = tab0[(oLROW + i) * 64 + lane];
          lk.z[i] = __builtin_fma(lh[s], lds[oXC + v_pkp[v]], la[s] * v_x[v]);
          lk.y[i] = lr >= 0 ? yg[lr] * cscale / Eg[lr] : 0.0;
        }
      }
    }
    const double *xq = xt_p + (oXC - oXT);
    const d2 a0 = *(const d2 *)xq, a1 = *(const d2 *)(xq + 2 * NPOS), a2 = *(const d2 *)(xq + 4 * NPOS), a3 = *(const d2 *)(xq + 6 * NPOS);
    const double xc[8] = {a0.x, a0.y, a1.x, a1.y, a2.x, a2.y, a3.x, a3.y};
#pragma unroll
    for (int q = 0; q < NS; q++) {
      const int h = tab0[(oHROW + q) * 64 + lane], br = tab0[(oHBROW + q) * 64 + lane], ev = tab0[(oHEVAR + q) * 64 + lane];
      double J[8];
      if (JREG) {
#pragma unroll
        for (int k = 0; k < 8; k++) J[k] = hJ[q][k];
      } else {
        const d2 *jp = (const d2 *)(jl_p + q * 512);
        const d2 j0 = jp[0], j1 = jp[64], j2 = jp[128], j3 = jp[192];
        J[0] = j0.x; J[1] = j0.y; J[2] = j1.x; J[3] = j1.y; J[4] = j2.x; J[5] = j2.y; J[6] = j3.x; J[7] = j3.y;
      }
      double s = J[0] * xc[0];
#pragma unroll
      for (int k = 1; k < BS; k++) s = __builtin_fma(J[k], xc[k], s);
      if (h >= 0) {
        h_xe[q] = xg[ev] / Dg[ev];
        h_z[q] = s + h_ae[q] * h_xe[q]; h_zb[q] = h_ab[q] * h_xe[q];
        h_y[q] = yg[h] * cscale / (Eg[h] * wc); h_yb[q] = yg[br] * cscale / Eg[br];
      }
    }
    WV_SYNC();
  }
  rows(std::integral_constant<int, 0>{});

  int status = 0, iter = it0;
  double pri = 0.0, dua = 0.0;
  double rho_new = 0.0;
  const int stop = (a.slice > 0 && it0 + a.slice < a.max_iter) ? it0 + a.slice : a.max_iter;
  while (!status && iter < stop && !(ADAPT && rho_new > 0.0)) {
    int next = stop;
    if constexpr (GRES) load_g();
    if (a.check > 0) { next = (iter / a.check + 1) * a.check; if (next > stop) next = stop; }
    while (iter + 2 < next) { iter++; if (!(ablate & 1)) sweep(); if (!(ablate & 2)) rows(std::integral_constant<int, 1>{}); }
    if (iter + 1 < next) { iter++; if (!(ablate & 1)) sweep(); if (!(ablate & 2)) rows(std::integral_constant<int, 1>{}); }
    iter++;
    c_ndy = 0.0; c_lhs = 0.0; c_ndx = 0.0; c_qdx = 0.0;
    sweep(); rows(std::integral_constant<int, 2>{});
    if (ablate & 16) continue;
    const bool adapt_pt = ADAPT && iter % a.ad_interval == 0 && iter < a.max_iter;
    double v_pri = 0.0, v_pn = 0.0, v_dua = 0.0, v_dn = 0.0;
    for (int approximate = 0; approximate < 2 && !status; approximate++) {
      if (approximate && iter < a.max_iter) break;
      double ea = a.eps_abs, er = a.eps_rel, epi = a.eps_prim_inf, edi = a.eps_dual_inf;
      if (approximate) { ea *= 10; er *= 10; epi *= 10; edi *= 10; }
      double w_pri = 0.0, w_pn = 0.0, w_dua = 0.0, w_dn = 0.0;
      {
        const double *xq = xt_p + (oXC - oXT);
        const d2 a0 = *(const d2 *)xq, a1 = *(const d2 *)(xq + 2 * NPOS), a2 = *(const d2 *)(xq + 4 * NPOS), a3 = *(const d2 *)(xq + 6 * NPOS);
        const double xc[8] = {a0.x, a0.y, a1.x, a1.y, a2.x, a2.y, a3.x, a3.y};
        double part[8] = {0, 0, 0, 0, 0, 0, 0, 0};
#pragma unroll
        for (int q = 0; q < NS; q++) {
          double J[8];
          if (JREG) {
#pragma unroll
            for (int k = 0; k < 8; k++) J[k] = hJ[q][k];
          } else {
            const d2 *jp = (const d2 *)(jl_p + q * 512);
            const d2 j0 = jp[0], j1 = jp[64], j2 = jp[128], j3 = jp[192];
            J[0] = j0.x; J[1] = j0.y; J[2] = j1.x; J[3] = j1.y; J[4] = j2.x; J[5] = j2.y; J[6] = j3.x; J[7] = j3.y;
          }
          double s = J[0] * xc[0];
#pragma unroll
          for (int k = 1; k < BS; k++) s = __builtin_fma(J[k], xc[k], s);
          const double ax = s + h_ae[q] * h_xe[q], axb = h_ab[q] * h_xe[q];
          const double eh = CKH(q, 0), eb = CKH(q, 1), de = CKH(q, 2);
          w_pri = fmax(w_pri, fmax(eh * fabs(ax - h_z[q]), eb * fabs(axb - h_zb[q])));
          w_pn = fmax(w_pn, fmax(eh * fmax(fabs(h_z[q]), fabs(ax)), eb * fmax(fabs(h_zb[q]), fabs(axb))));
          const double wy = wc * h_y[q];
          const double aty = h_ae[q] * wy + h_ab[q] * h_yb[q];
          w_dua = fmax(w_dua, de * fabs(h_q[q] + aty));
          w_dn = fmax(w_dn, de * fmax(fabs(h_q[q]), fabs(aty)));
          if (ADAPT && adapt_pt) {
            v_pri = fmax(v_pri, fmax(fabs(ax - h_z[q]), fabs(axb - h_zb[q])));
            v_pn = fmax(v_pn, fmax(fmax(fabs(h_z[q]), fabs(h_zb[q])), fmax(fabs(ax), fabs(axb))));
            v_dua = fmax(v_dua, fabs(h_q[q] + aty)); v_dn = fmax(v_dn, fmax(fabs(h_q[q]), fabs(aty)));
          }
#pragma unroll
          for (int k = 0; k < BS; k++) part[k] = __builtin_fma(J[k], wy, part[k]);
        }
        d2 v0, v1, v2, v3;
        v0.x = part[0]; v0.y = part[1]; v1.x = part[2]; v1.y = part[3]; v2.x = part[4]; v2.y = part[5]; v3.x = part[6]; v3.y = BS > 7 ? part[7] : 0.0;
        *(d2 *)part_p = v0; *(d2 *)(part_p + nslot2) = v1; *(d2 *)(part_p + 2 * nslot2) = v2; *(d2 *)(part_p + 3 * nslot2) = v3;
      }
      {
        const double xcv = x_p[oXC - oXT], ax = x_a * xcv, ex = CKX;
        w_pri = fmax(w_pri, ex * fabs(ax - x_z)); w_pn = fmax(w_pn, ex * fmax(fabs(x_z), fabs(ax)));
        if (ADAPT && adapt_pt) { v_pri = fmax(v_pri, fabs(ax - x_z)); v_pn = fmax(v_pn, fmax(fabs(x_z), fabs(ax))); }
        if (x_row >= 0) x_p[oEX - oXT] = x_a * (x_w * x_y);
      }
      if constexpr (LNK > 0) {
#pragma unroll
        for (int v = 0; v < NV; v++) {
          double ps = 0.0, la[NL1], lh[NL1], ll[NL1], lu[NL1];
          lk.consts(v, la, lh, ll, lu);
#pragma unroll
          for (int s = 0; s < LNK; s++) ps = __builtin_fma(lh[s], lk.y[v * LNK + s], ps);
          lds[oLK + v_pkp[v]] = ps;
        }
      }
      WV_SYNC();
#pragma unroll
      for (int v = 0; v < NV; v++) {
        const double c[5] = {CKV(v, 0), CKV(v, 1), CKV(v, 2), CKV(v, 3), CKV(v, 4)};
        const int vix = (int)(v_p[v] - (lds + oXT)), p = (vix % (2 * NPOS)) >> 1;
        const double dj = c[0], e0 = c[1];
        const double ax = v_a[v] * v_x[v];
        w_pri = fmax(w_pri, e0 * fabs(ax - v_z[v])); w_pn = fmax(w_pn, e0 * fmax(fabs(v_z[v]), fabs(ax)));
        if (ADAPT && adapt_pt) { v_pri = fmax(v_pri, fabs(ax - v_z[v])); v_pn = fmax(v_pn, fmax(fabs(v_z[v]), fabs(ax))); }
        double aty = v_a[v] * v_y[v] + v_p[v][oEX - oXT];
        if constexpr (LNK > 0) {
          const double xp = lds[oXC + v_pkp[v]];
          double la[NL1], lh[NL1], ll[NL1], lu[NL1];
          lk.consts(v, la, lh, ll, lu);
          aty += v_p[v][oLK - oXT];
#pragma unroll
          for (int s = 0; s < LNK; s++) {
            const int i = v * LNK + s;
            const double axl = __builtin_fma(lh[s], xp, la[s] * v_x[v]), el = CKL(i);
            w_pri = fmax(w_pri, el * fabs(axl - lk.z[i])); w_pn = fmax(w_pn, el * fmax(fabs(lk.z[i]), fabs(axl)));
            aty = __builtin_fma(la[s], lk.y[i], aty);
          }
        }
        const double *pp = v_pp[v];
        if (LPB > 0) {
#pragma unroll
          for (int s2 = 0; s2 < LPB; s2++) aty += pp[s2 * 2];
        } else {
          for (int s2 = 0; s2 < lpb; s2++) aty += pp[s2 * 2];
        }
        double px = c[2] * lds[oXC + v_pkm[v]] + c[3] * lds[oXC + v_pkp[v]];
        if (pdense) {
          const double *cd = wv_opaque(cstg0) + (size_t)(wv_cst_v(NS, v) + 5) * 64;
#pragma unroll
          for (int k2 = 0; k2 < BS; k2++) px = __builtin_fma(cd[k2 * 64], lds[oXC + wv_vidx(NPOS, p, k2)], px);
        } else {
          px = __builtin_fma(c[4], v_x[v], px);
        }
        if (v_on[v]) {
          w_dua = fmax(w_dua, dj * fabs(v_q[v] + px + aty));
          w_dn = fmax(w_dn, dj * fmax(fabs(v_q[v]), fmax(fabs(aty), fabs(px))));
          if (ADAPT && adapt_pt) {
            v_dua = fmax(v_dua, fabs(v_q[v] + px + aty));
            v_dn = fmax(v_dn, fmax(fabs(v_q[v]), fmax(fabs(aty), fabs(px))));
          }
        }
      }
      WV_SYNC();
      w_pri = wv_wmax(w_pri); w_pn = wv_wmax(w_pn); w_dua = wv_wmax(w_dua); w_dn = wv_wmax(w_dn);
      const double ndy = wv_wmax(c_ndy), ndx = wv_wmax(c_ndx), lhs = wv_wsum(c_lhs), qdx = wv_wsum(c_qdx);
      pri = w_pri; dua = cinv * w_dua;
      if (!(pri <= SCO_INFTY) || !(dua <= SCO_INFTY)) { status = SCO_QP_NON_CVX; break; }
      const double eps_p = ea + er * w_pn, eps_d = ea + er * cinv * w_dn;
      const bool prim_ok = (m == 0) || (pri < eps_p), dual_ok = dua < eps_d;
      if (prim_ok && dual_ok) { status = approximate ? SCO_QP_SOLVED_INACCURATE : SCO_QP_SOLVED; break; }
      if ((ablate & 64) == 0 && !prim_ok && ndy > epi && lhs < -epi * ndy) {
        double nat = 0.0;
        {
          double part[8] = {0, 0, 0, 0, 0, 0, 0, 0};
#pragma unroll
          for (int q = 0; q < NS; q++) {
            double J[8];
            if (JREG) {
#pragma unroll
              for (int k = 0; k < 8; k++) J[k] = hJ[q][k];
            } else {
              const d2 *jp = (const d2 *)(jl_p + q * 512);
              const d2 j0 = jp[0], j1 = jp[64], j2 = jp[128], j3 = jp[192];
              J[0] = j0.x; J[1] = j0.y; J[2] = j1.x; J[3] = j1.y; J[4] = j2.x; J[5] = j2.y; J[6] = j3.x; J[7] = j3.y;
            }
            const double wd = wc * dsv.h[q];
            nat = fmax(nat, CKH(q, 2) * fabs(h_ae[q] * wd + h_ab[q] * dsv.b[q]));
#pragma unroll
            for (int k = 0; k < BS; k++) part[k] = __builtin_fma(J[k], wd, part[k]);
          }
          d2 v0, v1, v2, v3;
          v0.x = part[0]; v0.y = part[1]; v1.x = part[2]; v1.y = part[3]; v2.x = part[4]; v2.y = part[5]; v3.x = part[6]; v3.y = BS > 7 ? part[7] : 0.0;
          *(d2 *)part_p = v0; *(d2 *)(part_p + nslot2) = v1; *(d2 *)(part_p + 2 * nslot2) = v2; *(d2 *)(part_p + 3 * nslot2) = v3;
        }
        if (x_row >= 0) x_p[oEX - oXT] = x_a * (x_w * dsv.x);
        if constexpr (LNK > 0) {
#pragma unroll
          for (int v = 0; v < NV; v++) {
            double ps = 0.0, la[NL1], lh[NL1], ll[NL1], lu[NL1];
            lk.consts(v, la, lh, ll, lu);
#pragma unroll
            for (int s = 0; s < LNK; s++) ps = __builtin_fma(lh[s], lk.d[v * LNK + s], ps);
            lds[oLK + v_pkp[v]] = ps;
          }
        }
        WV_SYNC();
#pragma unroll
        for (int v = 0; v < NV; v++) {
          double aty = v_a[v] * dsv.r0[v] + v_p[v][oEX - oXT];
          if constexpr (LNK > 0) {
            double la[NL1], lh[NL1], ll[NL1], lu[NL1];
            lk.consts(v, la, lh, ll, lu);
            aty += v_p[v][oLK - oXT];
#pragma unroll
            for (int s = 0; s < LNK; s++) aty = __builtin_fma(la[s], lk.d[v * LNK + s], aty);
          }
          const double *pp = v_pp[v];
          if (LPB > 0) {
#pragma unroll
            for (int s2 = 0; s2 < LPB; s2++) aty += pp[s2 * 2];
          } else {
            for (int s2 = 0; s2 < lpb; s2++) aty += pp[s2 * 2];
          }
          if (v_on[v]) nat = fmax(nat, CKV(v, 0) * fabs(aty));
        }
        WV_SYNC();
        nat = wv_wmax(nat);
        if ((status = osqp_primal_inf_status(nat, ndy, epi, approximate))) break;
      }
      if ((ablate & 64) == 0 && !dual_ok && ndx > edi && qdx < -cscale * edi * ndx) {
#pragma unroll
        for (int v = 0; v < NV; v++) v_p[v][oXC - oXT] = dsv.var[v];
        WV_SYNC();
        double npx = 0.0;
#pragma unroll
        for (int v = 0; v < NV; v++) {
          const double c[5] = {CKV(v, 0), CKV(v, 1), CKV(v, 2), CKV(v, 3), CKV(v, 4)};
          const int vix = (int)(v_p[v] - (lds + oXT)), p = (vix % (2 * NPOS)) >> 1;
          double px = c[2] * lds[oXC + v_pkm[v]] + c[3] * lds[oXC + v_pkp[v]];
          if (pdense) {
            const double *cd = wv_opaque(cstg0) + (size_t)(wv_cst_v(NS, v) + 5) * 64;
#pragma unroll
            for (int k2 = 0; k2 < BS; k2++) px = __builtin_fma(cd[k2 * 64], lds[oXC + wv_vidx(NPOS, p, k2)], px);
          } else {
            px = __builtin_fma(c[4], dsv.var[v], px);
          }
          if (v_on[v]) npx = fmax(npx, c[0] * fabs(px));
        }
        npx = wv_wmax(npx);
        if (npx < cscale * edi * ndx) {
          const double thr = edi * ndx;
          double badv = 0.0;
          const double *xq = xt_p + (oXC - oXT);
          const d2 a0 = *(const d2 *)xq, a1 = *(const d2 *)(xq + 2 * NPOS), a2 = *(const d2 *)(xq + 4 * NPOS), a3 = *(const d2 *)(xq + 6 * NPOS);
          const double dxb[8] = {a0.x, a0.y, a1.x, a1.y, a2.x, a2.y, a3.x, a3.y};
#pragma unroll
          for (int q = 0; q < NS; q++) {
            double J[8];
            if (JREG) {
#pragma unroll
              for (int k = 0; k < 8; k++) J[k] = hJ[q][k];
            } else {
              const d2 *jp = (const d2 *)(jl_p + q * 512);
              const d2 j0 = jp[0], j1 = jp[64], j2 = jp[128], j3 = jp[192];
              J[0] = j0.x; J[1] = j0.y; J[2] = j1.x; J[3] = j1.y; J[4] = j2.x; J[5] = j2.y; J[6] = j3.x; J[7] = j3.y;
            }
            double s2 = J[0] * dxb[0];
#pragma unroll
            for (int k = 1; k < BS; k++) s2 = __builtin_fma(J[k], dxb[k], s2);
            const double adh = CKH(q, 0) * (s2 + h_ae[q] * dsv.e[q]), adb = CKH(q, 1) * (h_ab[q] * dsv.e[q]);
            if (h_on[q] && ((h_u[q] < WV_BIG && adh > thr) || adb < -thr)) badv = 1.0;
          }
#pragma unroll
          for (int v = 0; v < NV; v++) {
            const double adx = CKV(v, 1) * (v_a[v] * dsv.var[v]);
            if (v_r0on[v] && ((v_u[v] < WV_BIG && adx > thr) || (v_l[v] > -WV_BIG && adx < -thr))) badv = 1.0;
            if constexpr (LNK > 0) {
              const double dxp = lds[oXC + v_pkp[v]];
              double la[NL1], lh[NL1], ll[NL1], lu[NL1];
              lk.consts(v, la, lh, ll, lu);
#pragma unroll
              for (int s = 0; s < LNK; s++) {
                const double adl = CKL(v * LNK + s) * __builtin_fma(lh[s], dxp, la[s] * dsv.var[v]);
                if (osqp_row_leaves_cone(adl, ll[s], lu[s], thr)) badv = 1.0;
              }
            }
          }
          if (x_row >= 0) {
            const double adx = CKX * (x_a * x_p[oXC - oXT]);
            if ((x_u < WV_BIG && adx > thr) || (x_l > -WV_BIG && adx < -thr)) badv = 1.0;
          }
          badv = wv_wmax(badv);
          if ((status = osqp_dual_inf_status(badv, approximate))) break;
        }
        WV_SYNC();
#pragma unroll
        for (int v = 0; v < NV; v++) v_p[v][oXC - oXT] = v_x[v];
        WV_SYNC();
      }
    }
    if (ADAPT && adapt_pt && !status) {
      const double vs[7] = {wv_wmax(v_pri), wv_wmax(v_pn), 0.0, wv_wmax(v_dua), wv_wmax(v_dn), 0.0, 0.0};
      const double est = osqp_rho_estimate(vs, rho0);
      if (osqp_rho_must_change(est, rho0, a.ad_tol)) rho_new = est;
    }
  }
  if (!status && iter < a.max_iter) {
    if (ADAPT && rho_new > 0.0 && lane == 0) { a.rho_b[b] = rho_new; a.rflag[b] = 1; a.smask[b] = 1; a.nupd[b] += 1; }
    double *sx = a.sx + (size_t)b * n, *sz = a.sz + (size_t)b * m, *sy = a.sy + (size_t)b * m;
    double *stp = a.st + (size_t)b * m, *sgp = a.sg + (size_t)b * a.n_e;
    const int *tab = wv_opaque(tab0);
#pragma unroll
    for (int q = 0; q < NS; q++) {
      const int h = tab[(oHROW + q) * 64 + lane], br = tab[(oHBROW + q) * 64 + lane], ev = tab[(oHEVAR + q) * 64 + lane];
      if (h >= 0) {
        sz[h] = h_z[q]; sy[h] = h_y[q]; sz[br] = h_zb[q]; sy[br] = h_yb[q]; sx[ev] = h_xe[q];
        const double th = wc * (rho0 * h_z[q] - h_y[q]), tb = rho0 * h_zb[q] - h_yb[q];
        stp[h] = th - (rw * h_ae[q]) * h_ge[q]; stp[br] = tb - (rho0 * h_ab[q]) * h_ge[q];
        sgp[tab[(oHEIDX + q) * 64 + lane]] = h_ge[q];
      }
    }
#pragma unroll
    for (int v = 0; v < NV; v++) {
      const int var = tab[(oVVAR + v) * 64 + lane], r0 = tab[(oVROW + v) * 64 + lane];
      if (var >= 0) sx[var] = v_x[v];
      if (r0 >= 0) { sz[r0] = v_z[v]; sy[r0] = v_y[v]; stp[r0] = rho0 * v_z[v] - v_y[v]; }
    }
    if (x_row >= 0) { sz[x_row] = x_z; sy[x_row] = x_y; stp[x_row] = x_w * (x_rho * x_z - x_y); }
    if constexpr (LNK > 0) {
#pragma unroll
      for (int i = 0; i < NLK; i++) {
        const int lr = tab[(oLROW + i) * 64 + lane];
        if (lr >= 0) { sz[lr] = lk.z[i]; sy[lr] = lk.y[i]; stp[lr] = rho0 * lk.z[i] - lk.y[i]; }
      }
    }
    if (lane == 0) { a.prog[b] = iter; a.status[b] = 0; a.iters[b] = iter; atomicAdd(a.it_count, (unsigned long long)(iter - it0)); }
    return;
  }
  if (a.slice > 0 && lane == 0) a.prog[b] = 0;
  if (!status) status = SCO_QP_MAX_ITER_REACHED;
  if (iter > a.max_iter) iter = a.max_iter;
  {
    const double *Dg = a.D + (size_t)b * n, *Eg = a.E + (size_t)b * m;
    double *xo = a.x + (size_t)b * n, *yo = a.y + (size_t)b * m;
    const int *tab = wv_opaque(tab0);
#pragma unroll
    for (int q = 0; q < NS; q++) {
      const int h = tab[(oHROW + q) * 64 + lane], br = tab[(oHBROW + q) * 64 + lane], ev = tab[(oHEVAR + q) * 64 + lane];
      if (h >= 0) {
        xo[ev] = Dg[ev] * h_xe[q];
        yo[h] = cinv * Eg[h] * h_y[q] * wc;
        yo[br] = cinv * Eg[br] * h_yb[q];
      }
    }
#pragma unroll
    for (int v = 0; v < NV; v++) {
      const int var = tab[(oVVAR + v) * 64 + lane], r0 = tab[(oVROW + v) * 64 + lane];
      if (var >= 0) xo[var] = Dg[var] * v_x[v];
      if (r0 >= 0) yo[r0] = cinv * Eg[r0] * v_y[v];
    }
    if (x_row >= 0) yo[x_row] = cinv * Eg[x_row] * x_y * x_w;
    if constexpr (LNK > 0) {
#pragma unroll
      for (int i = 0; i < NLK; i++) {
        const int lr = tab[(oLROW + i) * 64 + lane];
        if (lr >= 0) yo[lr] = cinv * Eg[lr] * lk.y[i];
      }
    }
    if (lane == 0) {
      a.status[b] = status; a.iters[b] = iter; a.resid[2 * (size_t)b] = pri; a.resid[2 * (size_t)b + 1] = dua;
      atomicAdd(a.it_count, (unsigned long long)(iter - it0));
    }
  }
}

static void wv_fill_args(const AdmmArgs &aa, const WvHost &wh, const WvDev &wd, const int *setup_mask, WvArgs &a) {
  const QpDev &d = aa.d;
  a.n = d.n; a.m = d.m; a.n_e = d.n_e; a.n_c = d.n_c; a.nnzA = d.nnzA; a.nnzP = d.nnzP;
  a.max_iter = aa.max_iter; a.check = aa.check; a.slice = aa.slice; a.b0 = d.b0; a.list = d.list;
  a.bs = wh.bs; a.nb = wh.nb; a.mid = wh.mid; a.lpb = wh.lpb; a.n_extra = wh.n_extra; a.NS = wh.NS; a.NV = wh.NV; a.NSTEP = wh.NSTEP;
  a.cst_slots = wh.cst_slots; a.NL = wh.NL; a.g_doubles = wh.g_doubles;
  a.rho = aa.rho; a.sigma = aa.sigma; a.alpha = aa.alpha; a.eps_abs = aa.eps_abs; a.eps_rel = aa.eps_rel;
  a.eps_prim_inf = aa.eps_prim_inf; a.eps_dual_inf = aa.eps_dual_inf;
  a.tab = wd.tab; a.G = wd.G; a.cst = wd.cst; a.wc = wd.wc; a.scr = wd.scr; a.ok = wd.ok; a.rl_need = wd.rl_need; a.w_ready = wd.w_ready; a.pflag = wd.pflag; a.it_count = wd.it_count;
  a.As = d.As; a.Ps = d.Ps; a.qs = d.qs; a.ls = d.ls; a.us = d.us; a.rhov = d.rho; a.kee_inv = d.kee_inv; a.cscale = d.cscale;
  a.D = d.D; a.E = d.E; a.S = d.W; a.w = d.w; a.active = d.active; a.setup_active = setup_mask;
  a.Ap = d.Ap; a.Ai = d.Ai; a.Rp = d.Rp; a.Rj = d.Rj; a.Rpos = d.Rpos; a.Fp = d.Fp; a.Fi = d.Fi; a.Fpos = d.Fpos;
  a.x = d.x; a.y = d.y; a.resid = d.resid; a.status = d.status; a.iters = d.iters; a.prog = d.prog;
  a.sx = d.sx; a.sz = d.sz; a.sy = d.sy; a.st = d.st; a.sg = d.sg;
  a.warm = aa.warm; a.ad_interval = aa.adaptive ? aa.ad_interval : 0; a.ad_tol = aa.ad_tol;
  a.rho_b = aa.adaptive ? d.rho_b : nullptr; a.rflag = aa.adaptive ? d.rflag : nullptr;
  a.smask = aa.adaptive ? d.smask : nullptr; a.nupd = aa.adaptive ? d.nupd : nullptr;
#ifdef WV_ABLATE
  { const char *ab = getenv("SCO_WV_ABLATE"); a.ablate = ab ? atoi(ab) : 0; }
#else
  a.ablate = 0;
#endif
}

__global__ void qp_wv_need_kernel(int b0, const int *list, int nb, const int *setup_mask, const int *active, int *w_ready, int *need) {
  const int g = blockIdx.x * blockDim.x + threadIdx.x;
  if (g >= nb) return;
  const int b = list ? list[g + b0] : g + b0;
  if (b < 0) return;
  const int nd = (setup_mask ? setup_mask[b] != 0 : 1) || ((!active || active[b]) && !w_ready[b]);
  need[b] = nd;
  if (nd) w_ready[b] = 1;
}

int wv_launch_need(const AdmmArgs &aa, const int *setup_mask, const WvDev &wd, hipStream_t st) {
  const int nwg = qp_launch_nwg(aa.d);
  hipLaunchKernelGGL(qp_wv_need_kernel, dim3((nwg + 255) / 256), dim3(256), 0, st, aa.d.b0, aa.d.list, nwg, setup_mask, aa.d.active,
                     wd.w_ready, wd.rl_need);
  SCO_HIP(hipGetLastError());
  return SCO_OK;
}

int wv_launch_factor(const AdmmArgs &aa, const int *setup_mask, const WvHost &wh, const WvDev &wd, hipStream_t st) {
  WvArgs a; wv_fill_args(aa, wh, wd, setup_mask, a);
  const int nwg = qp_launch_nwg(aa.d);
  if (wh.NL) hipLaunchKernelGGL(qp_wv_factor_kernel<WV_NL>, dim3(nwg), dim3(WV_T), 0, st, a);
  else hipLaunchKernelGGL(qp_wv_factor_kernel<0>, dim3(nwg), dim3(WV_T), 0, st, a);
  SCO_HIP(hipGetLastError());
  return SCO_OK;
}

template <int BS, int NS, int NV, int NSTEP, int LPB, int EXT, int LNK>
static int wv_launch_k(const WvArgs &a, int nwg, size_t lds, hipStream_t st) {
  static bool attr_done[64] = {};
  SCO_LDS_ATTR((qp_admm_wv_kernel<BS, NS, NV, NSTEP, LPB, EXT, LNK>), 64 * 1024, attr_done);
  hipLaunchKernelGGL((qp_admm_wv_kernel<BS, NS, NV, NSTEP, LPB, EXT, LNK>), dim3(nwg), dim3(WV_T), lds, st, a);
  SCO_HIP(hipGetLastError());
  return SCO_OK;
}

template <int BS, int NS, int NV, int NSTEP, int LPB>
static int wv_launch_one(const WvArgs &a, int nwg, size_t lds, hipStream_t st) {
  if (a.NL) {
    if (LPB > 0 || a.ad_interval > 0) { sco_set_error("wv_launch: no instantiation with link rows for this launch"); return SCO_ERR_STATE; }
    if constexpr (LPB == 0 && BS == 7) return wv_launch_k<BS, NS, NV, NSTEP, LPB, 1, WV_NL>(a, nwg, lds, st);
    else if constexpr (LPB == 0) return a.warm ? wv_launch_k<BS, NS, NV, NSTEP, LPB, 1, WV_NL>(a, nwg, lds, st) : wv_launch_k<BS, NS, NV, NSTEP, LPB, 0, WV_NL>(a, nwg, lds, st);
  }
  if (a.ad_interval > 0) return wv_launch_k<BS, NS, NV, NSTEP, LPB, 3, 0>(a, nwg, lds, st);
  return a.warm ? wv_launch_k<BS, NS, NV, NSTEP, LPB, 1, 0>(a, nwg, lds, st) : wv_launch_k<BS, NS, NV, NSTEP, LPB, 0, 0>(a, nwg, lds, st);
}

int wv_launch(const AdmmArgs &aa, const WvHost &wh, const WvDev &wd, hipStream_t st) {
  WvArgs a; wv_fill_args(aa, wh, wd, nullptr, a);
  const int nwg = qp_launch_nwg(aa.d);
  const size_t lds = std::max(wh.lds_bytes, (size_t)36 * 1024);
  if (wh.NSTEP == 10 && wh.NS == 4 && wh.lpb == 3 && !wh.NL) return wv_launch_one<7, 4, 3, 10, 3>(a, nwg, lds, st);
  if (wh.NSTEP == 10 && wh.NS == 4) return wv_launch_one<7, 4, 3, 10, 0>(a, nwg, lds, st);
  if (wh.NSTEP == 10) return wv_launch_one<8, 2, 2, 10, 0>(a, nwg, lds, st);
  if (wh.NSTEP == 4) return wv_launch_one<8, 1, 1, 4, 0>(a, nwg, lds, st);
  return wv_launch_one<8, 2, 2, 8, 0>(a, nwg, lds, st);
}
```

### sco_py_amd/csrc/sco_qp.hip

```cpp
#include "sco_admm_check.h"

#include <algorithm>
#include <climits>
#include <cmath>
#include <cstdio>
#include <cstdlib>
#include <cstring>

static thread_local std::string g_err;
void sco_set_error(const std::string &msg) { g_err = msg; }
int sco_hip_fail(hipError_t e, const char *what) {
  g_err = std::string(what) + ": " + hipGetErrorString(e);
  return SCO_ERR_DEVICE;
}
extern "C" const char *sco_last_error(void) { return g_err.c_str(); }
extern "C" int sco_version(void) { return 100; }

extern "C" int sco_device_count(int *count) {
  if (!count) return SCO_ERR_ARG;
  int n = 0;
  hipError_t e = hipGetDeviceCount(&n);
  if (e != hipSuccess) { *count = 0; (void)hipGetLastError(); return SCO_OK; }
  *count = n;
  return SCO_OK;
// ... 636 lines not shown
  UP(s_a) UP(s_b) UP(s_ppos) UP(sa_ptr) UP(sa_row) UP(sa_pa) UP(sa_pb) UP(ss_ptr) UP(ss_k1) UP(ss_k2) UP(ss_e)
#undef UP
  SCO_TRY(sco_upload<int>(qp->allocs, pl.Pp, &qp->Pp_dev));
  SCO_TRY(sco_upload<int>(qp->allocs, pl.Pi, &qp->Pi_dev));
  const size_t B = (size_t)batch;
#define AL(field, count) SCO_TRY(sco_alloc_zeroed(qp->allocs, (count), &d.field));
  AL(Pval, B * pl.nnzP) AL(q, B * n) AL(Aval, B * pl.nnzA) AL(l, B * m) AL(u, B * m) AL(w, B * m)
  AL(Ps, B * pl.nnzP) AL(As, B * pl.nnzA) AL(qs, B * n) AL(ls, B * m) AL(us, B * m) AL(D, B * n) AL(E, B * m)
  AL(cscale, B) AL(rho, B * m) AL(kee_inv, B * pl.n_e) AL(cpl, B * pl.ncpl) AL(W, (qp->use_bt ? 1 : B) * pl.n_c * pl.n_c)
  AL(x, B * n) AL(y, B * m) AL(resid, B * 2) AL(status, B) AL(iters, B)
  AL(prog, B) AL(sx, B * n) AL(sz, B * m) AL(sy, B * m) AL(st, B * m) AL(sg, B * pl.n_e)
  AL(rho_b, B) AL(rflag, B) AL(smask, B) AL(nupd, B) AL(amask, B)
#undef AL
  SCO_HIP(hipFuncSetAttribute((const void *)qp_setup_kernel, hipFuncAttributeMaxDynamicSharedMemorySize, (int)LDS_CAP));
  SCO_HIP(hipFuncSetAttribute((const void *)qp_factor_kernel, hipFuncAttributeMaxDynamicSharedMemorySize, (int)LDS_CAP));
  SCO_HIP(hipFuncSetAttribute((const void *)qp_admm_kernel, hipFuncAttributeMaxDynamicSharedMemorySize, (int)LDS_CAP));
  if (qp->use_big) {
    SCO_TRY(big_upload(qp->big, qp->use_bt ? 1 : batch, qp->allocs, qp->bigd));
    if (qp->use_bt) SCO_TRY(bt_upload(qp->bt, batch, qp->allocs, qp->btd));
    return SCO_OK;
  }
  if (qp->kern == QP_K_RL) SCO_TRY(rl_upload(qp->rl, qp->allocs, qp->rld));
  if (qp->use_wv) SCO_TRY(wv_upload(qp->wv, batch, n, m, qp->allocs, qp->wvd));
  if (qp->kern == QP_K_REG) SCO_TRY(reg_upload(qp->reg, qp->allocs, qp->regd));
  if (qp->kern == QP_K_FAST) SCO_TRY(fast_upload(qp->fast, qp->allocs, qp->fastd));
  return SCO_OK;
}

extern "C" int sco_qp_create(int device, int batch, int n, int m, const int *Pp, const int *Pi,
                             const int *Ap, const int *Ai, sco_qp **out) {
  return sco_qp_create_on_stream(device, batch, n, m, Pp, Pi, Ap, Ai, nullptr, out);
}

extern "C" int sco_qp_destroy(sco_qp *qp) {
  if (!qp) return SCO_OK;
  ScoDeviceGuard sco_guard_(qp->device);
  if (qp->stream) (void)hipStreamSynchronize(qp->stream);
  for (void *p : qp->allocs) (void)hipFree(p);
  qp_polish_free(qp);
  for (auto &e : qp->ev) if (e) (void)hipEventDestroy(e);
  if (qp->own_stream && qp->stream) (void)hipStreamDestroy(qp->stream);
  delete qp;
  return SCO_OK;
}

extern "C" int sco_qp_load(sco_qp *qp, const double *P_val, const double *q, const double *A_val,
                           const double *l, const double *u, const int *row_weight) {
  if (!qp || !q || (qp->d.nnzP && !P_val) || (qp->d.nnzA && !A_val) || (qp->d.m && (!l || !u))) {
    sco_set_error("sco_qp_load: null pointer"); return SCO_ERR_ARG;
  }
  SCO_ON_DEVICE(qp->device);
  const QpDev &d = qp->d; const size_t B = d.batch;
  if (d.nnzP) SCO_HIP(hipMemcpyAsync(d.Pval, P_val, B * d.nnzP * sizeof(double), hipMemcpyHostToDevice, qp->stream));
  SCO_HIP(hipMemcpyAsync(d.q, q, B * d.n * sizeof(double), hipMemcpyHostToDevice, qp->stream));
  if (d.nnzA) SCO_HIP(hipMemcpyAsync(d.Aval, A_val, B * d.nnzA * sizeof(double), hipMemcpyHostToDevice, qp->stream));
  if (d.m) {
    SCO_HIP(hipMemcpyAsync(d.l, l, B * d.m * sizeof(double), hipMemcpyHostToDevice, qp->stream));
    SCO_HIP(hipMemcpyAsync(d.u, u, B * d.m * sizeof(double), hipMemcpyHostToDevice, qp->stream));
    if (row_weight) SCO_HIP(hipMemcpyAsync(d.w, row_weight, B * d.m * sizeof(int), hipMemcpyHostToDevice, qp->stream));
    else {
      std::vector<int> ones(B * d.m, 1);
      SCO_HIP(hipMemcpyAsync(d.w, ones.data(), ones.size() * sizeof(int), hipMemcpyHostToDevice, qp->stream));
      SCO_HIP(hipStreamSynchronize(qp->stream));
    }
  }
  SCO_HIP(hipStreamSynchronize(qp->stream));
  qp->loaded = true;
  qp->polish_ready = false;
  return SCO_OK;
}

extern "C" int sco_qp_set_bounds(sco_qp *qp, const double *l, const double *u) {
  if (!qp || !l || !u) { sco_set_error("sco_qp_set_bounds: null pointer"); return SCO_ERR_ARG; }
  if (!qp->loaded) { sco_set_error("sco_qp_set_bounds: call sco_qp_load first"); return SCO_ERR_STATE; }
  SCO_ON_DEVICE(qp->device);
  qp->polish_ready = false;
  const QpDev &d = qp->d; const size_t B = d.batch;
  SCO_HIP(hipMemcpyAsync(d.l, l, B * d.m * sizeof(double), hipMemcpyHostToDevice, qp->stream));
  SCO_HIP(hipMemcpyAsync(d.u, u, B * d.m * sizeof(double), hipMemcpyHostToDevice, qp->stream));
  SCO_HIP(hipStreamSynchronize(qp->stream));
  return SCO_OK;
}

int sco_qp_launch(sco_qp *qp, const sco_qp_settings *st, const int *active_dev, hipEvent_t mid) {
  return sco_qp_launch_sliced(qp, st, active_dev, active_dev, 0, mid, nullptr);
}

int sco_qp_wv_iters(const sco_qp *qp, unsigned long long *out) {
  *out = 0;
  if (!qp->use_wv) return SCO_OK;
  SCO_HIP(hipMemcpy(out, qp->wvd.it_count, sizeof(unsigned long long), hipMemcpyDeviceToHost));
  return SCO_OK;
}
void sco_qp_wv_iters_reset(sco_qp *qp, hipStream_t st) { if (qp->use_wv) (void)hipMemsetAsync(qp->wvd.it_count, 0, sizeof(unsigned long long), st); }
bool sco_qp_has_wv(const sco_qp *qp) { return qp->use_wv; }
bool sco_qp_wv_links(const sco_qp *qp) { return qp->use_wv && qp->wv.NL > 0; }
bool sco_qp_can_adapt(const sco_qp *qp) { return !(qp->use_big && !qp->use_bt); }

static QpLaunchIn qp_launch_in(const sco_qp *qp, const sco_qp_settings *st) {
  QpLaunchIn in;
  in.kern = qp->kern; in.use_big = qp->use_big; in.use_bt = qp->use_bt; in.use_wv = qp->use_wv; in.wv_links = sco_qp_wv_links(qp);
  in.factor_cholesky = qp->factor_cholesky; in.batch = qp->d.batch; in.n_c = qp->d.n_c; in.cus = qp->cus;
  in.adaptive_rho = st->adaptive_rho; in.adaptive_rho_interval = st->adaptive_rho_interval;
  in.adaptive_rho_tolerance = st->adaptive_rho_tolerance; in.check_termination = st->check_termination; in.max_iter = st->max_iter;
  return in;
}

bool sco_qp_supports_groups(const sco_qp *qp, const sco_qp_settings *st) { return qp_supports_windows(qp_launch_in(qp, st)); }

static QpLaunchPlan qp_plan_launch(const sco_qp *qp, const sco_qp_settings *st, const int *setup_mask, int slice, const QpGroup *grp) {
  QpLaunchIn in = qp_launch_in(qp, st);
  in.slice = slice;
  in.mask = setup_mask == SCO_MASK_ALL ? QP_MASK_ALL : setup_mask == SCO_MASK_NONE ? QP_MASK_NONE : QP_MASK_ARRAY;
  in.wv_min = sco_wv_min_live(qp->cus, st->adaptive_rho != 0);
  if (grp) {
    in.window = true; in.b0 = grp->b0; in.nb = grp->nb; in.tier = grp->tier; in.has_list = grp->list != nullptr;
    in.side_b0 = grp->side_b0; in.side_nb = grp->side_nb; in.side_slices = grp->side_slices;
    in.side_ready = grp->side_stream && grp->side_ev[0] && grp->side_ev[1] && grp->side_ev[2];
  }
  return qp_launch_plan(in);
}

static int qp_launch_rho_init(const QpDev &d, const int *setup_mask, double rho, hipStream_t stream) {
  RhoInitArgs ra{d, setup_mask == SCO_MASK_ALL ? nullptr : setup_mask, setup_mask == SCO_MASK_ALL ? 1 : 0, rho};
  hipLaunchKernelGGL(qp_rho_init_kernel, dim3((d.batch + 255) / 256), dim3(256), 0, stream, ra);
  SCO_HIP(hipGetLastError());
  return SCO_OK;
}

static int qp_launch_setup_factor(sco_qp *qp, const QpLaunchPlan &pl, const sco_qp_settings *st, const AdmmArgs &aa,
                                  const int *setup_active, const QpGroup *grp, hipStream_t stream) {
  QpDev dsetup = aa.d; dsetup.active = setup_active;
  const size_t ntri = (size_t)dsetup.n_c * (dsetup.n_c + 1) / 2;
  SetupArgs sa{dsetup, qp->Pp_dev, qp->Pi_dev, st->rho, st->sigma, st->scaling, st->adaptive_rho ? 1 : 0};
  hipLaunchKernelGGL(qp_setup_kernel, dim3(pl.nwg), dim3(SCO_BLOCK), qp->lds_setup - ntri * sizeof(double), stream, sa);
  SCO_HIP(hipGetLastError());
  if (pl.wv_now) SCO_TRY(wv_launch_factor(aa, setup_active, qp->wv, qp->wvd, stream));
  if (pl.need == QP_NEED_SIDE) {
    AdmmArgs as = aa; as.d.b0 = grp->side_b0; as.d.nb = grp->side_nb;
    SCO_TRY(wv_launch_need(as, setup_active, qp->wvd, stream));
  } else if (pl.need == QP_NEED_WINDOW) {
    SCO_TRY(wv_launch_need(aa, setup_active, qp->wvd, stream));
  }
  if (pl.wv_now || pl.need != QP_NEED_NONE) dsetup.active = qp->wvd.rl_need;
  if (pl.cholesky)
    hipLaunchKernelGGL(qp_factor_kernel, dim3(dsetup.batch), dim3(SCO_FACTOR_BLOCK), (ntri + dsetup.n_c) * sizeof(double), stream, dsetup);
  else if (pl.sweep_nt == 1) hipLaunchKernelGGL(qp_sweep_kernel<1>, dim3(pl.nwg), dim3(SCO_FACTOR_BLOCK), 0, stream, dsetup);
  else if (pl.sweep_nt == 2) hipLaunchKernelGGL(qp_sweep_kernel<2>, dim3(pl.nwg), dim3(SCO_FACTOR_BLOCK), 0, stream, dsetup);
  else hipLaunchKernelGGL(qp_sweep_kernel<3>, dim3(pl.nwg), dim3(SCO_FACTOR_BLOCK), 0, stream, dsetup);
  SCO_HIP(hipGetLastError());
  return SCO_OK;
}

static int qp_launch_mixed(sco_qp *qp, const AdmmArgs &aa, const QpGroup *grp, hipStream_t stream) {
  AdmmArgs as = aa; as.d.b0 = grp->side_b0; as.d.nb = grp->side_nb; as.slice = grp->side_slices * aa.slice;
  AdmmArgs aw = aa;
  aw.d.b0 = grp->side_b0 == grp->b0 ? grp->b0 + grp->side_nb : grp->b0; aw.d.nb = grp->nb - grp->side_nb;
  SCO_HIP(hipEventRecord(grp->side_ev[0], stream));
  SCO_HIP(hipStreamWaitEvent(grp->side_stream, grp->side_ev[0], 0));
  SCO_HIP(hipEventRecord(grp->side_ev[1], grp->side_stream));
  SCO_TRY(rl_launch(as, qp->rl, qp->rld, grp->side_stream));
  SCO_HIP(hipEventRecord(grp->side_ev[2], grp->side_stream));
  SCO_HIP(hipStreamWaitEvent(stream, grp->side_ev[1], 0));
  SCO_TRY(wv_launch(aw, qp->wv, qp->wvd, stream));
  aw.skip = qp->wvd.ok;
  SCO_TRY(rl_launch(aw, qp->rl, qp->rld, stream));
// ... 64 lines not shown
  if (settings->max_iter <= 0 || !(settings->rho > 0) || !(settings->sigma > 0) || settings->scaling < 0) {
    sco_set_error("sco_qp_solve: bad settings"); return SCO_ERR_ARG;
  }
  SCO_ON_DEVICE(qp->device);
  qp->polish_ready = false;
  const QpDev &d = qp->d; const size_t B = d.batch;
  int rc;
  if (settings->adaptive_rho) {
    SCO_HIP(hipMemsetAsync(d.prog, 0, B * sizeof(int), qp->stream));
    std::vector<int> prog(B);
    const long long cap = (long long)settings->max_iter / sco_qp_adaptive_interval(settings) + 2;
    float ms_setup = 0, ms_admm = 0;
    for (long long round = 0; round < cap; round++) {
      rc = sco_qp_launch_sliced(qp, settings, round == 0 ? SCO_MASK_ALL : SCO_MASK_NONE, round == 0 ? nullptr : d.amask,
                                0, nullptr, nullptr);
      if (rc) return rc;
      SCO_HIP(hipMemcpyAsync(prog.data(), d.prog, B * sizeof(int), hipMemcpyDeviceToHost, qp->stream));
      SCO_HIP(hipStreamSynchronize(qp->stream));
      float t0 = 0, t1 = 0;
      SCO_HIP(hipEventElapsedTime(&t0, qp->ev[0], qp->ev[1]));
      SCO_HIP(hipEventElapsedTime(&t1, qp->ev[1], qp->ev[2]));
      ms_setup += t0; ms_admm += t1;
      bool parked = false;
      for (size_t b = 0; b < B; b++) { prog[b] = prog[b] > 0 ? 1 : 0; parked = parked || prog[b]; }
      if (!parked) break;
      SCO_HIP(hipMemcpyAsync(d.amask, prog.data(), B * sizeof(int), hipMemcpyHostToDevice, qp->stream));
    }
    SCO_TRY(qp_copy_back(qp, x, y, status, iters, resid));
    qp->last_ms[0] = ms_setup; qp->last_ms[1] = ms_admm;
    qp->polish_ready = true;
    return SCO_OK;
  }
  rc = sco_qp_launch(qp, settings, nullptr, nullptr);
  if (rc) return rc;
  SCO_TRY(qp_copy_back(qp, x, y, status, iters, resid));
  float ms0 = 0, ms1 = 0;
  SCO_HIP(hipEventElapsedTime(&ms0, qp->ev[0], qp->ev[1]));
  SCO_HIP(hipEventElapsedTime(&ms1, qp->ev[1], qp->ev[2]));
  qp->last_ms[0] = ms0; qp->last_ms[1] = ms1;
  qp->polish_ready = true;
  return SCO_OK;
}

extern "C" int sco_qp_adaptive_info(sco_qp *qp, double *rho, int *updates) {
  if (!qp) return SCO_ERR_ARG;
  SCO_ON_DEVICE(qp->device);
  const QpDev &d = qp->d;
  if (rho) SCO_HIP(hipMemcpy(rho, d.rho_b, (size_t)d.batch * sizeof(double), hipMemcpyDeviceToHost));
  if (updates) SCO_HIP(hipMemcpy(updates, d.nupd, (size_t)d.batch * sizeof(int), hipMemcpyDeviceToHost));
  return SCO_OK;
}

static size_t qp_admm_lds_bytes(const sco_qp *qp) {
  if (qp->use_big) return qp->use_bt ? qp->bt.lds_bytes : 0;
  switch (qp->kern) {
    case QP_K_RL: return rl_reported_static_lds() + qp->rl.lds_bytes;
    case QP_K_REG: return reg_static_lds() + qp->reg.lds_bytes;
    case QP_K_FAST: return qp->fast.lds_bytes;
  }
  return qp->lds_admm;
}

extern "C" int sco_qp_info(const sco_qp *qp, int info[4]) {
  if (!qp || !info) return SCO_ERR_ARG;
  info[0] = qp->plan.n_e; info[1] = qp->plan.n_c;
  info[2] = (int)qp_admm_lds_bytes(qp); info[3] = qp->plan.ncpl;
  return SCO_OK;
}

extern "C" int sco_qp_last_timing(const sco_qp *qp, double ms[2]) {
  if (!qp || !ms) return SCO_ERR_ARG;
  ms[0] = qp->last_ms[0]; ms[1] = qp->last_ms[1];
  return SCO_OK;
}

extern "C" int sco_debug_qp_tiers(const sco_qp *qp) {
  if (!qp) return SCO_ERR_ARG;
  return qp_tier_mask(*qp);
}
extern "C" int sco_debug_qp_wv_iters(const sco_qp *qp, unsigned long long *out) {
  if (!qp || !out) return SCO_ERR_ARG;
  return sco_qp_wv_iters(qp, out);
}
```

### sco_py_amd/csrc/sco_sqp.hip

```cpp
#include "sco_admm_check.h"
#include "sqp_layout.h"
#include "sqp_rows.h"
#include "sqp_sched.h"

#include <algorithm>

#include <cmath>
#include <cstdio>
#include <cstdlib>
#include <cstring>

enum { ST_PROJECT = 0, ST_CONVEXIFY = 1, ST_TRIAL = 2, ST_DONE = 3 };
enum { STEP_PROJECT = 0, STEP_ACCEPT = 1, STEP_SHRINK = 2, STEP_YCONV = 3, STEP_XCONV = 4, STEP_BAD = 5, STEP_GROUP = 6 };

#define TRACE_W 8

struct SqpScalars {
  double penalty, trust, slack_cost, merit, merit_viol;
  long long admm_iters;
  int state, k, sqp_iters, qp_solves, success, escalations, n_trace, spawned;
  int flags;
};

struct EventPool {
// ... 847 lines not shown
  AL(bmod, (size_t)B * m_nl) AL(trace, (size_t)B * s.trace_cap * TRACE_W) AL(mask, (size_t)B * m_nl * ds)
  AL(sc, (size_t)B) AL(active, (size_t)B) AL(n_active, SQP_MAX_GROUPS) AL(newqp, (size_t)B) AL(list_buf, (size_t)B)
  s.H = 40; s.HC = 24;
  AL(hkey, (size_t)B * s.NB * s.H * ds) AL(hval, (size_t)B * s.NB * s.H * s.RM) AL(ckey, (size_t)B * s.NB * s.HC * ds)
  AL(cJ, (size_t)B * s.NB * s.HC * s.RM * ds) AL(cb, (size_t)B * s.NB * s.HC * s.RM) AL(hn, (size_t)B * s.NB)
  AL(cn, (size_t)B * s.NB)
  AL(cw, (size_t)B) AL(ctgt, (size_t)B * 2)
  {
    const size_t NO = oblk ? NBt : T, dO = oblk ? ds : d;
    if (desc->family & SCO_FAM_FLAG_OBJ_WIDE) {
      void *p = nullptr;
      const size_t bytes = (size_t)B * NO * dO * dO * sizeof(double);
      if (hipMalloc(&p, bytes) != hipSuccess) {
        (void)hipGetLastError();
        char buf[200];
        snprintf(buf, sizeof buf, "sco_sqp_create: the objective terms' Hessians (batch x terms x n^2 doubles) need %zu bytes of "
                 "device memory; use a smaller batch", bytes);
        sco_set_error(buf); return SCO_ERR_CAPACITY;
      }
      h->allocs.push_back(p); s.oH = (double *)p;
      SCO_HIP(hipMemset(p, 0, bytes));
    } else {
      AL(oH, cost ? (size_t)B * NO * dO * dO : 1)
    }
    AL(oA, cost ? (size_t)B * NO * dO : 1) AL(ob, cost ? (size_t)B * NO : 1)
  }
  AL(mvec, (size_t)B * 32) AL(nonconv, (size_t)B) AL(stalled, (size_t)B)
#undef AL
  { int *p; if ((rc = sq_alloc(h, (size_t)K, &p))) return rc; s.point_link = p; }
  { double *p; if ((rc = sq_alloc(h, (size_t)K, &p))) return rc; s.point_frac = p; }
  { unsigned int *p; if ((rc = sq_alloc(h, (size_t)s.NB, &p))) return rc; s.gmask = p; }
  { unsigned int *p; if ((rc = sq_alloc(h, (size_t)32, &p))) return rc; s.goverlap = p; }
  s.G = 0;
  if ((rc = sq_upload(h, L.ppos, &s.ppos)) || (rc = sq_upload(h, L.jpos, &s.jpos)) || (rc = sq_upload(h, L.epos, &s.epos)) ||
      (rc = sq_upload(h, L.a0c, &s.a0c)) || (rc = sq_upload(h, L.a1c, &s.a1c))) return rc;
  s.gen_eq = s.gpos0 = s.gpos1 = nullptr; s.gen_rhs = s.gen_val = nullptr;
  if (L.m_gen) {
    double *q;
    if ((rc = sq_upload(h, L.gen_eq, &s.gen_eq)) || (rc = sq_upload(h, L.gpos0, &s.gpos0)) || (rc = sq_upload(h, L.gpos1, &s.gpos1))) return rc;
    if ((rc = sq_alloc(h, (size_t)B * L.m_gen, &q))) return rc; s.gen_rhs = q;
    if ((rc = sq_alloc(h, (size_t)B * L.nnz_gen, &q))) return rc; s.gen_val = q;
  }
  return SCO_OK;
}

extern "C" int sco_sqp_destroy(sco_sqp *h) {
  if (!h) return SCO_OK;
  ScoDeviceGuard sco_guard_(h->device);
  if (h->stream) (void)hipStreamSynchronize(h->stream);
  if (h->qp0) sco_qp_destroy(h->qp0);
  if (h->qp1) sco_qp_destroy(h->qp1);
  for (void *p : h->allocs) (void)hipFree(p);
  for (void *p : h->prog_buf) if (p) (void)hipFree(p);
  if (h->objw_buf) (void)hipFree(h->objw_buf);
  if (h->accw_buf) (void)hipFree(h->accw_buf);
  h->events.destroy(); h->done.destroy(); h->mix_events.destroy();
  for (auto &ge : h->gevents) ge.destroy();
  for (auto gs : h->gstream) if (gs) { (void)hipStreamSynchronize(gs); (void)hipStreamDestroy(gs); }
  if (h->host_active) (void)hipHostFree(h->host_active);
  if (h->stream) (void)hipStreamDestroy(h->stream);
  delete h;
  return SCO_OK;
}

extern "C" int sco_sqp_load(sco_sqp *h, const double *x0, const double *start, const double *goal,
                            const double *link_len, const int *point_link, const double *point_frac,
                            const double *obstacles) {
  if (!h || !x0 || !start || !goal || !link_len || !point_link || !point_frac || !obstacles) {
    sco_set_error("sco_sqp_load: null pointer"); return SCO_ERR_ARG;
  }
  const SqpDev &s = h->d;
  for (int k = 0; k < s.K; k++)
    if (point_link[k] < 0 || point_link[k] >= s.d) { sco_set_error("sco_sqp_load: point_link out of range"); return SCO_ERR_ARG; }
  SCO_ON_DEVICE(h->device);
  const size_t B = s.batch;
  SCO_HIP(hipMemcpyAsync(s.x0, x0, B * s.n_x * sizeof(double), hipMemcpyHostToDevice, h->stream));
  SCO_HIP(hipMemcpyAsync(s.start, start, B * s.d * sizeof(double), hipMemcpyHostToDevice, h->stream));
  SCO_HIP(hipMemcpyAsync(s.goal, goal, B * s.d * sizeof(double), hipMemcpyHostToDevice, h->stream));
  SCO_HIP(hipMemcpyAsync(s.link_len, link_len, B * s.d * sizeof(double), hipMemcpyHostToDevice, h->stream));
  SCO_HIP(hipMemcpyAsync(s.obstacles, obstacles, B * s.O * 3 * sizeof(double), hipMemcpyHostToDevice, h->stream));
  SCO_HIP(hipMemcpyAsync((void *)s.point_link, point_link, s.K * sizeof(int), hipMemcpyHostToDevice, h->stream));
  SCO_HIP(hipMemcpyAsync((void *)s.point_frac, point_frac, s.K * sizeof(double), hipMemcpyHostToDevice, h->stream));
  SCO_HIP(hipStreamSynchronize(h->stream));
  h->loaded = true; h->solved = false;
  return SCO_OK;
}

extern "C" int sco_sqp_load_ee_cost(sco_sqp *h, const double *weight, const double *target) {
  if (!h || !weight || !target) { sco_set_error("sco_sqp_load_ee_cost: null pointer"); return SCO_ERR_ARG; }
  if (!(h->desc.family & SCO_FAM_FLAG_EE_COST)) { sco_set_error("sco_sqp_load_ee_cost: family has no objective term"); return SCO_ERR_ARG; }
  if (!h->loaded) { sco_set_error("sco_sqp_load_ee_cost: call sco_sqp_load first"); return SCO_ERR_STATE; }
  for (int b = 0; b < h->d.batch; b++)
    if (!(weight[b] >= 0.0)) { sco_set_error("sco_sqp_load_ee_cost: weight must be >= 0"); return SCO_ERR_ARG; }
  SCO_ON_DEVICE(h->device);
  SCO_HIP(hipMemcpyAsync(h->d.cw, weight, (size_t)h->d.batch * sizeof(double), hipMemcpyHostToDevice, h->stream));
  SCO_HIP(hipMemcpyAsync(h->d.ctgt, target, (size_t)h->d.batch * 2 * sizeof(double), hipMemcpyHostToDevice, h->stream));
  SCO_HIP(hipStreamSynchronize(h->stream));
  h->cost_loaded = true; h->solved = false;
  return SCO_OK;
}

extern "C" int sco_sqp_load_target(sco_sqp *h, const double *target) {
  if (!h || !target) { sco_set_error("sco_sqp_load_target: null pointer"); return SCO_ERR_ARG; }
  if ((h->desc.family & 15) != SCO_FAM_ARM_REACH) { sco_set_error("sco_sqp_load_target: family has no target"); return SCO_ERR_ARG; }
  if (!h->loaded) { sco_set_error("sco_sqp_load_target: call sco_sqp_load first"); return SCO_ERR_STATE; }
  SCO_ON_DEVICE(h->device);
  SCO_HIP(hipMemcpyAsync(h->d.target, target, (size_t)h->d.batch * 2 * sizeof(double), hipMemcpyHostToDevice, h->stream));
  SCO_HIP(hipStreamSynchronize(h->stream));
  h->target_loaded = true; h->solved = false;
  return SCO_OK;
}

extern "C" int sco_sqp_load_vel_limit(sco_sqp *h, const double *vmax) {
  if (!h || !vmax) { sco_set_error("sco_sqp_load_vel_limit: null pointer"); return SCO_ERR_ARG; }
  if (!(h->desc.family & SCO_FAM_FLAG_VEL_LIMITS)) { sco_set_error("sco_sqp_load_vel_limit: family has no velocity limits"); return SCO_ERR_ARG; }
  if (!h->loaded) { sco_set_error("sco_sqp_load_vel_limit: call sco_sqp_load first"); return SCO_ERR_STATE; }
  for (int b = 0; b < h->d.batch; b++)
    if (!(vmax[b] > 0.0)) { sco_set_error("sco_sqp_load_vel_limit: vmax must be positive"); return SCO_ERR_ARG; }
  SCO_ON_DEVICE(h->device);
  SCO_HIP(hipMemcpyAsync(h->d.vmax, vmax, (size_t)h->d.batch * sizeof(double), hipMemcpyHostToDevice, h->stream));
  SCO_HIP(hipStreamSynchronize(h->stream));
  h->vel_loaded = true; h->solved = false;
  return SCO_OK;
}

extern "C" int sco_sqp_load_joint_limits(sco_sqp *h, const double *lo, const double *hi) {
  if (!h || !lo || !hi) { sco_set_error("sco_sqp_load_joint_limits: null pointer"); return SCO_ERR_ARG; }
  if (!(h->desc.family & SCO_FAM_FLAG_JOINT_LIMITS)) { sco_set_error("sco_sqp_load_joint_limits: family has no joint limits"); return SCO_ERR_ARG; }
  if (!h->loaded) { sco_set_error("sco_sqp_load_joint_limits: call sco_sqp_load first"); return SCO_ERR_STATE; }
  const size_t cnt = (size_t)h->d.batch * h->d.d;
  for (size_t k = 0; k < cnt; k++)
    if (!(lo[k] < hi[k])) { sco_set_error("sco_sqp_load_joint_limits: need lo < hi"); return SCO_ERR_ARG; }
  SCO_ON_DEVICE(h->device);
  SCO_HIP(hipMemcpyAsync(h->d.jlo, lo, cnt * sizeof(double), hipMemcpyHostToDevice, h->stream));
  SCO_HIP(hipMemcpyAsync(h->d.jhi, hi, cnt * sizeof(double), hipMemcpyHostToDevice, h->stream));
  SCO_HIP(hipStreamSynchronize(h->stream));
  h->jl_loaded = true; h->solved = false;
  return SCO_OK;
}

extern "C" int sco_sqp_load_quadratic(sco_sqp *h, const double *Q, const double *a, const double *c) {
  if (!h || !Q || !a || !c) { sco_set_error("sco_sqp_load_quadratic: null pointer"); return SCO_ERR_ARG; }
  if ((h->desc.family & 15) != SCO_FAM_STATE_QUADRATIC) { sco_set_error("sco_sqp_load_quadratic: family has no quadratic rows"); return SCO_ERR_ARG; }
  if (!h->loaded) { sco_set_error("sco_sqp_load_quadratic: call sco_sqp_load first"); return SCO_ERR_STATE; }
  const size_t B = h->d.batch, O = h->d.O, d = h->d.d;
  for (size_t k = 0; k < B * O; k++)
    for (size_t i = 0; i < d; i++)
      for (size_t j = 0; j < i; j++)
        if (Q[k * d * d + i * d + j] != Q[k * d * d + j * d + i]) { sco_set_error("sco_sqp_load_quadratic: Q must be symmetric"); return SCO_ERR_ARG; }
  SCO_ON_DEVICE(h->device);
  SCO_HIP(hipMemcpyAsync(h->d.qQ, Q, B * O * d * d * sizeof(double), hipMemcpyHostToDevice, h->stream));
  SCO_HIP(hipMemcpyAsync(h->d.qa, a, B * O * d * sizeof(double), hipMemcpyHostToDevice, h->stream));
  SCO_HIP(hipMemcpyAsync(h->d.qc, c, B * O * sizeof(double), hipMemcpyHostToDevice, h->stream));
  SCO_HIP(hipStreamSynchronize(h->stream));
  h->quad_loaded = true; h->solved = false;
  return SCO_OK;
}

extern "C" int sco_sqp_load_spatial(sco_sqp *h, const double *joint_off, const double *joint_axis, const double *point_pos,
                                    const double *point_rad, const double *spheres) {
  if (!h || !joint_off || !joint_axis || !point_pos || !point_rad || !spheres) { sco_set_error("sco_sqp_load_spatial: null pointer"); return SCO_ERR_ARG; }
  if ((h->desc.family & 15) != SCO_FAM_ARM_SPATIAL) { sco_set_error("sco_sqp_load_spatial: family has no spatial arm"); return SCO_ERR_ARG; }
  if (!h->loaded) { sco_set_error("sco_sqp_load_spatial: call sco_sqp_load first"); return SCO_ERR_STATE; }
  const SqpDev &s = h->d;
  const size_t B = s.batch, d = s.d, K = s.K, O = s.O;
  const double *arr[5] = {joint_off, joint_axis, point_pos, point_rad, spheres};
// ... 548 lines not shown
  h->rounds = 1;
  SCO_TRY(sqp_reset_penalty_qp(h, params, qs, &L.qsl));
  L.sc = sqp_plan(h, params->admm_slice, L.qsl, L.p.max_qp_solves, n_active);
  SCO_TRY(sqp_loop_start(L));
  if (n_active > 0) SCO_TRY(sqp_run_rounds(L));
  SCO_TRY(sqp_store_counters(L));
  sqp_stage_times(L);
  h->solved = true;
  return SCO_OK;
}

extern "C" int sco_sqp_fetch(sco_sqp *h, double *x, int *success, int *sqp_iters, int *qp_solves,
                             long long *admm_iters, double *merit, double *max_violation) {
  if (!h) return SCO_ERR_ARG;
  if (!h->solved) { sco_set_error("sco_sqp_fetch: call sco_sqp_solve first"); return SCO_ERR_STATE; }
  SCO_ON_DEVICE(h->device);
  const SqpDev &s = h->d; const size_t B = s.batch;
  if (x) SCO_HIP(hipMemcpy(x, s.x, B * s.n_x * sizeof(double), hipMemcpyDeviceToHost));
  std::vector<SqpScalars> sc(B);
  SCO_HIP(hipMemcpy(sc.data(), s.sc, B * sizeof(SqpScalars), hipMemcpyDeviceToHost));
  for (size_t b = 0; b < B; b++) {
    if (success) success[b] = sc[b].success;
    if (sqp_iters) sqp_iters[b] = sc[b].sqp_iters;
    if (qp_solves) qp_solves[b] = sc[b].qp_solves;
    if (admm_iters) admm_iters[b] = sc[b].admm_iters;
  }
  if (merit || max_violation) {
    double *dm = h->fetch_buf, *dv = h->fetch_buf + B;
    hipLaunchKernelGGL(sqp_final_kernel, dim3(s.batch), dim3(SCO_BLOCK), 0, h->stream, s, dm, dv);
    SCO_HIP(hipGetLastError());
    SCO_HIP(hipStreamSynchronize(h->stream));
    if (merit) SCO_HIP(hipMemcpy(merit, dm, B * sizeof(double), hipMemcpyDeviceToHost));
    if (max_violation) SCO_HIP(hipMemcpy(max_violation, dv, B * sizeof(double), hipMemcpyDeviceToHost));
  }
  return SCO_OK;
}

extern "C" int sco_sqp_trace(sco_sqp *h, int cap, double *trace, int *n_entries) {
  if (!h || !trace || !n_entries || cap <= 0) return SCO_ERR_ARG;
  if (!h->solved) { sco_set_error("sco_sqp_trace: call sco_sqp_solve first"); return SCO_ERR_STATE; }
  SCO_ON_DEVICE(h->device);
  const SqpDev &s = h->d; const size_t B = s.batch;
  std::vector<double> tr(B * s.trace_cap * TRACE_W);
  std::vector<SqpScalars> sc(B);
  SCO_HIP(hipMemcpy(tr.data(), s.trace, tr.size() * sizeof(double), hipMemcpyDeviceToHost));
  SCO_HIP(hipMemcpy(sc.data(), s.sc, B * sizeof(SqpScalars), hipMemcpyDeviceToHost));
  for (size_t b = 0; b < B; b++) {
    n_entries[b] = sc[b].n_trace;
    const int rows = std::min(std::min(sc[b].n_trace, s.trace_cap), cap);
    for (int r = 0; r < rows; r++)
      memcpy(trace + (b * cap + r) * TRACE_W, tr.data() + (b * s.trace_cap + r) * TRACE_W, TRACE_W * sizeof(double));
  }
  return SCO_OK;
}

extern "C" int sco_sqp_last_rounds(const sco_sqp *h, int *rounds) {
  if (!h || !rounds) return SCO_ERR_ARG;
  *rounds = h->rounds;
  return SCO_OK;
}

extern "C" int sco_debug_sqp_layout(const sco_trajopt_desc *desc, int n_rows, const int *row_ptr, const int *col_idx, const int *row_is_eq,
                                    int dims[22], int sizes[15], int *ints, double *vals) {
  if (!dims || !sizes) { sco_set_error("sco_debug_sqp_layout: null pointer"); return SCO_ERR_ARG; }
  const char *err = "";
  if (int rc = sqp_check_desc(desc, n_rows, row_ptr, col_idx, row_is_eq, &err)) { sco_set_error(err); return rc; }
  const SqpLayout L = sqp_layout_build(*desc, n_rows, row_ptr, col_idx, row_is_eq);
  const int dm[22] = {L.NE, L.S, L.ds, L.NBt, L.Req, L.m_pin, L.m_vel, L.m_jl, L.m_gen, L.nnz_gen, L.R, L.n_x, L.n_slack, L.n,
                      L.m_lin, L.m_nl, L.m, L.NB, L.RM, L.point, L.cost, L.acc};
  memcpy(dims, dm, sizeof dm);
  const std::vector<int> *iv[13] = {&L.qp0.Pp, &L.qp0.Pi, &L.qp0.Ap, &L.qp0.Ai, &L.qp1.Pp, &L.qp1.Pi, &L.qp1.Ap, &L.qp1.Ai,
                                    &L.jpos, &L.epos, &L.ppos, &L.gpos0, &L.gpos1};
  const std::vector<double> *dv[2] = {&L.a0c, &L.a1c};
  for (int k = 0; k < 13; k++) {
    sizes[k] = (int)iv[k]->size();
    if (ints) ints = std::copy(iv[k]->begin(), iv[k]->end(), ints);
  }
  for (int k = 0; k < 2; k++) {
    sizes[13 + k] = (int)dv[k]->size();
    if (vals) vals = std::copy(dv[k]->begin(), dv[k]->end(), vals);
  }
  return SCO_OK;
}
extern "C" int sco_debug_sqp_check_program(const sco_trajopt_desc *desc, int n_circle_rows, int n_words, const int *words,
                                           const int *row_ptr, int n_consts, int n_params) {
  const char *err = "";
  if (int rc = sqp_check_desc(desc, 0, nullptr, nullptr, nullptr, &err)) { sco_set_error(err); return rc; }
  if (!words || !row_ptr) { sco_set_error("sco_sqp_load_program: null pointer"); return SCO_ERR_ARG; }
  if ((desc->family & 15) != SCO_FAM_STATE_PROGRAM) { sco_set_error("sco_sqp_load_program: family has no row programs"); return SCO_ERR_ARG; }
  const SqpLayout L = sqp_layout_build(*desc, 0, nullptr, nullptr, nullptr);
  if (n_circle_rows < 0 || n_circle_rows >= desc->n_obstacles) { sco_set_error("sco_debug_sqp_check_program: bad circle-row count"); return SCO_ERR_ARG; }
  const int rc = sqp_check_program(desc->n_obstacles - n_circle_rows, L.cost, L.ds, desc->dof, n_words, words, row_ptr, n_consts, n_params, &err);
  if (rc) sco_set_error(err);
  return rc;
}

extern "C" int sco_debug_sqp_wv_rounds(const sco_sqp *h) { return h ? h->wv_rounds : -1; }
extern "C" int sco_debug_sqp_mixed(const sco_sqp *h, int out[2]) {
  if (!h || !out) return SCO_ERR_ARG;
  out[0] = h->mixed_rounds; out[1] = h->mixed_side;
  return SCO_OK;
}
extern "C" int sco_sqp_last_tiers(const sco_sqp *h, double ms[2], long long iters[2], int launches[2]) {
  if (!h || !ms || !iters || !launches) return SCO_ERR_ARG;
  SCO_ON_DEVICE(h->device);
  unsigned long long wv_it = 0;
  if (sco_qp_wv_iters(h->qp1, &wv_it)) return SCO_ERR_DEVICE;
  ms[0] = h->wv_ms; ms[1] = h->last_ms[2] - h->wv_ms;
  iters[0] = (long long)wv_it; iters[1] = -1;
  launches[0] = h->wv_rounds; launches[1] = h->launches - h->wv_rounds + h->mixed_rounds;
  return SCO_OK;
}
extern "C" int sco_sqp_last_launches(const sco_sqp *h, int *launches, int *groups) {
  if (!h) return SCO_ERR_ARG;
  if (launches) *launches = h->launches;
  if (groups) *groups = h->groups_used;
  return SCO_OK;
}

extern "C" int sco_sqp_last_timing(const sco_sqp *h, double ms[5]) {
  if (!h || !ms) return SCO_ERR_ARG;
  memcpy(ms, h->last_ms, 5 * sizeof(double));
  return SCO_OK;
}
```

### sco_py_amd/csrc/sqp_layout.cpp

```cpp
#include "sqp_layout.h"

#include <algorithm>
#include <utility>

int sqp_check_desc(const sco_trajopt_desc *desc, int n_rows, const int *row_ptr, const int *col_idx, const int *row_is_eq,
                   const char **err) {
  auto refuse = [&](const char *text) { *err = text; return SCO_ERR_ARG; };
  if (!desc) return refuse("sco_sqp_create: null pointer");
  if (n_rows < 0 || n_rows > 65536 || (n_rows > 0 && (!row_ptr || !col_idx || !row_is_eq))) return refuse("sco_sqp_create_rows: bad row pattern");
  if (n_rows > 0) {
    if (row_ptr[0] != 0) return refuse("sco_sqp_create_rows: bad row pattern");
    const long long nx = (long long)desc->dof * desc->horizon;
    for (int r = 0; r < n_rows; r++) {
      if (row_ptr[r + 1] <= row_ptr[r] || row_ptr[r + 1] - row_ptr[r] > nx) return refuse("sco_sqp_create_rows: bad row pattern (empty row or row_ptr not increasing)");
      for (int k = row_ptr[r]; k < row_ptr[r + 1]; k++)
        if (col_idx[k] < 0 || col_idx[k] >= nx || (k > row_ptr[r] && col_idx[k] <= col_idx[k - 1]))
          return refuse("sco_sqp_create_rows: column indices must lie in [0, dof * horizon) and increase inside a row");
    }
  }
  const int family = desc->family, fam = family & 15, span = desc->span > 0 ? desc->span : 1, dof = desc->dof;
  const bool arm = fam == SCO_FAM_ARM_CIRCLES || fam == SCO_FAM_ARM_REACH, pointfam = fam == SCO_FAM_POINT_CIRCLES;
  const bool spatial = fam == SCO_FAM_ARM_SPATIAL;
  const bool progfam = fam == SCO_FAM_STATE_PROGRAM, statefam = fam == SCO_FAM_STATE_QUADRATIC || progfam;
  const bool ee = (family & SCO_FAM_FLAG_EE_COST) != 0, objprog = (family & SCO_FAM_FLAG_OBJ_PROGRAM) != 0;
// ... 59 lines not shown
      if (t >= 1) { Ai.push_back(m_pin + (t - 1) * d + j); Av.push_back(1.0); }
      if (t <= T - 2) { Ai.push_back(m_pin + t * d + j); Av.push_back(-1.0); }
      if (t >= 1) { Ai.push_back(m_pin + dT1 + (t - 1) * d + j); Av.push_back(-1.0); }
      if (t <= T - 2) { Ai.push_back(m_pin + dT1 + t * d + j); Av.push_back(1.0); }
    }
    if (jl) {
      Ai.push_back(m_pin + m_vel + t * d + j); Av.push_back(1.0);
      Ai.push_back(m_pin + m_vel + d * T + t * d + j); Av.push_back(-1.0);
    }
    for (const auto &rk : gen_of_col[t * d + j]) {
      gpos[rk.second] = (int)Ai.size();
      Ai.push_back(m_pin + m_vel + m_jl + rk.first); Av.push_back(0.0);
    }
  };
  {
    std::vector<int> &Pp = L.qp0.Pp, &Pi = L.qp0.Pi, &Ap = L.qp0.Ap, &Ai = L.qp0.Ai;
    Pp.resize(n_x + 1); Pi.resize(n_x); Ap.resize(n_x + 1);
    for (int i = 0; i < n_x; i++) { Pp[i] = i; Pi[i] = i; }
    Pp[n_x] = n_x;
    for (int col = 0; col < n_x; col++) {
      Ap[col] = (int)Ai.size();
      const int t = col / d, j = col % d;
      linear_entries(t, j, Ai, L.a0c, L.gpos0);
      Ai.push_back(m_lin + col); L.a0c.push_back(1.0);
    }
    Ap[n_x] = (int)Ai.size();
  }
  L.jpos.assign(n_x, 0); L.epos.assign(d, 0); L.ppos.assign(n_x, 0);
  {
    std::vector<int> &Pp = L.qp1.Pp, &Pi = L.qp1.Pi, &Ap = L.qp1.Ap, &Ai = L.qp1.Ai;
    std::vector<int> &jpos = L.jpos, &epos = L.epos, &ppos = L.ppos;
    std::vector<double> &a1c = L.a1c;
    Pp.resize(n + 1); Ap.resize(n + 1);
    for (int col = 0; col < n; col++) {
      Pp[col] = (int)Pi.size();
      if (col < n_x && oblk) {
        const int t = col / d, r0 = std::max(0, t - S + 1) * d;
        if (acc && S == 2 && t > 1) Pi.push_back(col - 2 * d);
        ppos[col] = (int)Pi.size() - r0;
        for (int r = r0; r <= col; r++) Pi.push_back(r);
      } else if (col < n_x) {
        if (acc && col / d > 1) Pi.push_back(col - 2 * d);
        if (col / d > 0) Pi.push_back(col - d);
        ppos[col] = (int)Pi.size();
        if (cost) for (int i = 0; i < col % d; i++) Pi.push_back(col - col % d + i);
        else ppos[col] -= col % d;
        Pi.push_back(col);
      }
    }
    Pp[n] = (int)Pi.size();
    for (int col = 0; col < n; col++) {
      Ap[col] = (int)Ai.size();
      if (col < n_x) {
        const int t = col / d, j = col % d;
        linear_entries(t, j, Ai, a1c, L.gpos1);
        jpos[col] = (int)Ai.size();
        for (int blk = std::max(0, t - S + 1); blk <= std::min(t, NBt - 1); blk++)
          for (int r = 0; r < R; r++) { Ai.push_back(m_lin + blk * R + r); a1c.push_back(0.0); }
        if (t == T - 1 && reach) {
          epos[j] = (int)Ai.size();
          for (int r = 0; r < NE; r++) { Ai.push_back(m_lin + NBt * R + r); a1c.push_back(0.0); }
        }
        Ai.push_back(m_lin + m_nl + col); a1c.push_back(1.0);
      } else {
        const int sidx = col - n_x;
        int row; double sgn = -1.0;
        if (sidx < NBt * SB) {
          const int blk = sidx / SB, k = sidx % SB, nh = R - Req;
          if (k < nh) row = blk * R + k;
          else { row = blk * R + nh + (k - nh) / 2; if ((k - nh) & 1) sgn = 1.0; }
        } else {
          const int ke = sidx - NBt * SB;
          row = NBt * R + ke / 2; if (ke & 1) sgn = 1.0;
        }
        Ai.push_back(m_lin + row); a1c.push_back(sgn);
        Ai.push_back(m_lin + m_nl + col); a1c.push_back(1.0);
      }
    }
    Ap[n] = (int)Ai.size();
  }
  return L;
}

int sqp_check_program(int n_prog_rows, int cost, int ds, int dof, int n_words, const int *words, const int *row_ptr,
                      int n_consts, int n_params, const char **err) {
  auto refuse = [&](const char *text) { *err = text; return SCO_ERR_ARG; };
  const int R = n_prog_rows + (obj_is_program(cost) ? 1 : 0);
  if (n_words <= 0 || n_consts < 0 || n_params < 0) return refuse("sco_sqp_load_program: bad program layout");
  if (row_ptr[0] != 0) return refuse("sco_sqp_load_program: bad program layout");
  for (int r = 0; r < R; r++)
    if (row_ptr[r + 1] <= row_ptr[r] || row_ptr[r + 1] > n_words) return refuse("sco_sqp_load_program: bad program layout");
  if (row_ptr[R] != n_words) return refuse("sco_sqp_load_program: bad program layout");
  for (int r = 0; r < R; r++) {
    if (words[2 * (row_ptr[r + 1] - 1)] != SCO_OP_END) return refuse("sco_sqp_load_program: a row's program must end with SCO_OP_END");
    const int nx = (r < n_prog_rows || cost == OBJ_BLOCK) ? ds : dof;
    int sp = 0;
    for (int w = row_ptr[r]; w < row_ptr[r + 1] - 1; w++) {
      const int op = words[2 * w], arg = words[2 * w + 1];
      bool ok = true;
      if (op == SCO_OP_X) { ok = arg >= 0 && arg < nx; sp++; }
      else if (op == SCO_OP_P) { ok = arg >= 0 && arg < n_params; sp++; }
      else if (op == SCO_OP_C) { ok = arg >= 0 && arg < n_consts; sp++; }
      else if (op >= SCO_OP_ADD && op <= SCO_OP_DIV) { ok = sp >= 2; sp--; }
      else if (op >= SCO_OP_NEG && op <= SCO_OP_SQUARE) ok = sp >= 1;
      else ok = false;
      if (!ok || sp > SCO_PROGRAM_STACK) return refuse("sco_sqp_load_program: malformed program (operand index, stack depth or opcode)");
    }
    if (sp != 1) return refuse("sco_sqp_load_program: a row's program must leave exactly one value");
  }
  return SCO_OK;
}
```

### sco_py_amd/csrc/sqp_layout.h

```cpp
#pragma once
#include "../../include/sco_hip.h"

#include <vector>

#define OBJ_DMAX 16
#define SPATIAL_DMAX 16
#define SCO_STATE_MAX 32

enum RowFamily {
  ROWS_ARM = 0,
  ROWS_POINT = 1,
  ROWS_QUADRATIC = 2,
  ROWS_PROGRAM = 3,
  ROWS_SPATIAL = 4
};
enum ObjKind {
  OBJ_NONE = 0,
  OBJ_EE = 1,
  OBJ_PROGRAM = 2,
  OBJ_BLOCK = 3
};
constexpr bool obj_is_program(int kind) { return kind >= OBJ_PROGRAM; }

int sqp_check_desc(const sco_trajopt_desc *desc, int n_rows, const int *row_ptr, const int *col_idx, const int *row_is_eq,
                   const char **err);

struct SqpQpPattern { std::vector<int> Pp, Pi, Ap, Ai; };

struct SqpLayout {
  int NE, S, ds, NBt, Req;
  int m_pin, m_vel, m_jl, m_gen, nnz_gen;
  int R, n_x, n_slack, n, m_lin, m_nl, m, NB, RM;
  int point, cost, acc;
  SqpQpPattern qp0, qp1;
  std::vector<double> a0c, a1c;
  std::vector<int> jpos, epos, ppos, gpos0, gpos1;
  std::vector<int> gen_eq;
};
SqpLayout sqp_layout_build(const sco_trajopt_desc &desc, int m_gen, const int *gen_ptr, const int *gen_col, const int *gen_iseq);

int sqp_check_program(int n_prog_rows, int cost, int ds, int dof, int n_words, const int *words, const int *row_ptr,
                      int n_consts, int n_params, const char **err);
```

### sco_py_amd/csrc/sqp_rows.h

```cpp
#pragma once
#include <hip/hip_runtime.h>

#include "sqp_layout.h"

#define FD_LEVELS 4
#define FD_BASE (1.0 / 64.0)

__device__ __forceinline__ double arm_row(const double *th, const double *len, int lk, double frac,
                                          double cx, double cy, double rad, int pert, double h) {
  double phi = 0.0, px = 0.0, py = 0.0;
  for (int i = 0; i <= lk; i++) {
    double a = th[i];
    if (i == pert) a += h;
    phi += a;
    double s, c;
    sincos(phi, &s, &c);
    const double L = (i == lk) ? frac * len[i] : len[i];
    px += L * c; py += L * s;
  }
  const double dx = px - cx, dy = py - cy;
  return rad - sqrt(dx * dx + dy * dy);
}

__device__ __forceinline__ double arm_row_grad(const double *th, const double *len, int lk, double frac,
// ... 187 lines not shown
    }
  }
  return st[0];
}
__device__ __forceinline__ double prog_dual(const RowCtx &c, const double *par, int o, const double *th, int j) {
#pragma clang fp contract(off)
  double sv[SCO_PROGRAM_STACK], sd[SCO_PROGRAM_STACK];
  int sp = 0;
  for (int w = c.pptr[o];; w++) {
    const int op = c.pw[2 * w], arg = c.pw[2 * w + 1];
    if (op == SCO_OP_END) break;
    switch (op) {
      case SCO_OP_X: sv[sp] = th[arg]; sd[sp++] = (arg == j) ? 1.0 : 0.0; break;
      case SCO_OP_P: sv[sp] = par[arg]; sd[sp++] = 0.0; break;
      case SCO_OP_C: sv[sp] = c.pconst[arg]; sd[sp++] = 0.0; break;
      case SCO_OP_ADD: sp--; sv[sp - 1] = sv[sp - 1] + sv[sp]; sd[sp - 1] = sd[sp - 1] + sd[sp]; break;
      case SCO_OP_SUB: sp--; sv[sp - 1] = sv[sp - 1] - sv[sp]; sd[sp - 1] = sd[sp - 1] - sd[sp]; break;
      case SCO_OP_MUL: sp--; sd[sp - 1] = sd[sp - 1] * sv[sp] + sv[sp - 1] * sd[sp]; sv[sp - 1] = sv[sp - 1] * sv[sp]; break;
      case SCO_OP_DIV: { sp--; const double qv = sv[sp - 1] / sv[sp]; sd[sp - 1] = (sd[sp - 1] - qv * sd[sp]) / sv[sp]; sv[sp - 1] = qv; break; }
      case SCO_OP_NEG: sv[sp - 1] = -sv[sp - 1]; sd[sp - 1] = -sd[sp - 1]; break;
      case SCO_OP_SIN: sd[sp - 1] = cos(sv[sp - 1]) * sd[sp - 1]; sv[sp - 1] = sin(sv[sp - 1]); break;
      case SCO_OP_COS: sd[sp - 1] = -(sin(sv[sp - 1]) * sd[sp - 1]); sv[sp - 1] = cos(sv[sp - 1]); break;
      case SCO_OP_SQRT: { const double r = sqrt(sv[sp - 1]); sd[sp - 1] = sd[sp - 1] / (2.0 * r); sv[sp - 1] = r; break; }
      case SCO_OP_EXP: { const double ev = exp(sv[sp - 1]); sd[sp - 1] = ev * sd[sp - 1]; sv[sp - 1] = ev; break; }
      default: sd[sp - 1] = (2.0 * sv[sp - 1]) * sd[sp - 1]; sv[sp - 1] = sv[sp - 1] * sv[sp - 1]; break;
    }
  }
  return sd[0];
}
__device__ __forceinline__ double row_value(const RowCtx &c, const RowRef &q, const double *th, int pert, double h) {
  if (q.eq == ROW_REACH_EQ) return arm_ee(th, c.len, c.d, q.r, pert, h);
  const int kp = q.r / c.O, o = q.r % c.O;
  if (c.point == ROWS_SPATIAL)
    return spatial_row(th, c.joff, c.jaxis, c.point_link[kp], c.ppos + 3 * kp, c.prad[kp], c.sph + 4 * o, pert, h);
  if (c.point == ROWS_PROGRAM) {
    if (q.r < c.R1) {
      const double dx = th[0] + (pert == 0 ? h : 0.0) - c.obs[3 * q.r], dy = th[1] + (pert == 1 ? h : 0.0) - c.obs[3 * q.r + 1];
      return c.obs[3 * q.r + 2] - sqrt(dx * dx + dy * dy);
    }
    return prog_eval(c, c.ppar + q.t * c.par_step, q.r - c.R1, th, pert, h, -1, 0.0);
  }
  if (c.point == ROWS_QUADRATIC) {
    const double *Q = c.qQ + (size_t)o * c.d * c.d, *av = c.qa + (size_t)o * c.d;
    double val = c.qc[o];
    for (int i = 0; i < c.d; i++) {
      const double xi = th[i] + (i == pert ? h : 0.0);
      double qx = 0.0;
      for (int j2 = 0; j2 < c.d; j2++) qx += Q[i * c.d + j2] * (th[j2] + (j2 == pert ? h : 0.0));
      val += xi * (av[i] + 0.5 * qx);
    }
    return val;
  }
  if (c.point == ROWS_POINT) {
    const double dx = th[0] + (pert == 0 ? h : 0.0) - c.obs[3 * o], dy = th[1] + (pert == 1 ? h : 0.0) - c.obs[3 * o + 1];
    return c.obs[3 * o + 2] - sqrt(dx * dx + dy * dy);
  }
  return arm_row(th, c.len, c.point_link[kp], c.point_frac[kp], c.obs[3 * o], c.obs[3 * o + 1], c.obs[3 * o + 2], pert, h);
}
__device__ __forceinline__ double row_grad(const RowCtx &c, const RowRef &q, const double *th, int j) {
  if (q.eq == ROW_REACH_EQ) return arm_ee_grad(th, c.len, c.d, q.r, j);
  const int kp = q.r / c.O, o = q.r % c.O;
  if (c.point == ROWS_SPATIAL) return spatial_row_grad(th, c.joff, c.jaxis, c.point_link[kp], c.ppos + 3 * kp, c.sph + 4 * o, j);
  if (c.point == ROWS_PROGRAM) {
    if (q.r < c.R1) {
      if (j > 1) return 0.0;
      const double dx = th[0] - c.obs[3 * q.r], dy = th[1] - c.obs[3 * q.r + 1];
      return -(j == 0 ? dx : dy) / sqrt(dx * dx + dy * dy);
    }
    return prog_dual(c, c.ppar + q.t * c.par_step, q.r - c.R1, th, j);
  }
  if (c.point == ROWS_QUADRATIC) {
    const double *Q = c.qQ + (size_t)o * c.d * c.d;
    double g = c.qa[(size_t)o * c.d + j];
    for (int i = 0; i < c.d; i++) g += Q[j * c.d + i] * th[i];
    return g;
  }
  if (c.point == ROWS_POINT) {
    if (j > 1) return 0.0;
    const double dx = th[0] - c.obs[3 * o], dy = th[1] - c.obs[3 * o + 1];
    return -(j == 0 ? dx : dy) / sqrt(dx * dx + dy * dy);
  }
  return arm_row_grad(th, c.len, c.point_link[kp], c.point_frac[kp], c.obs[3 * o], c.obs[3 * o + 1], j);
}
__device__ __forceinline__ bool row_ignores(const RowCtx &c, const RowRef &q, int j) {
  return c.point == ROWS_SPATIAL && j > c.point_link[q.r / c.O];
}
struct ObjCtx { int kind ; const double *len; int d; double tx, ty, w; };
__device__ __forceinline__ double obj_value(const ObjCtx &oc, const RowCtx &c, int t, const double *th, int pi, double hi, int pj, double hj) {
  if (obj_is_program(oc.kind)) return prog_eval(c, c.ppar + t * c.par_step, c.O - c.R1, th, pi, hi, pj, hj);
  return arm_ee_cost(th, oc.len, oc.d, oc.tx, oc.ty, oc.w, pi, hi, pj, hj);
}
__device__ __forceinline__ double row_rhs(const RowCtx &c, const RowRef &q) { return q.eq == ROW_REACH_EQ ? c.target[q.r] : 0.0; }
__device__ __forceinline__ double row_viol(const RowRef &q, double g) { return q.eq != ROW_HINGE ? fabs(g) : fmax(g, 0.0); }
```

### sco_py_amd/csrc/wv_plan.cpp

```cpp
#include "qp_tier_plans.h"
#include "layout_wv.h"

#include <algorithm>
#include <cstdlib>

static int wv_why_no_blocks(const QpPlan &pl) {
  int bs = 0;
  for (int c = 0; c < pl.n; c++)
    for (int t = pl.Pp[c]; t < pl.Pp[c + 1]; t++) {
      const int r = pl.Pi[t];
      if (r != c && pl.core_of[r] >= 0 && pl.core_of[c] >= 0) bs = std::max(bs, std::abs(pl.core_of[c] - pl.core_of[r]));
    }
  if (bs <= 0 || pl.n_c % bs) return WV_WHY_OTHER;
  int why = WV_WHY_OTHER;
  for (int i = 0; i < pl.m; i++) {
    int nc = 0, c0 = -1, c1 = -1; bool slack = false;
    for (int s = pl.Rp[i]; s < pl.Rp[i + 1]; s++) {
      const int j = pl.Rj[s];
      if (pl.elim_of[j] >= 0) { slack = true; continue; }
      const int c = pl.core_of[j];
      if (!nc) c0 = c1 = c; else { c0 = std::min(c0, c); c1 = std::max(c1, c); }
      nc++;
    }
    if (slack || nc < 2) continue;
    if (nc >= 3) return WV_WHY_THREE_CORE;
    if (c1 / bs == c0 / bs) why = WV_WHY_SAME_BLOCK;
    else if (c1 % bs != c0 % bs) why = WV_WHY_INDEX;
    else if (c1 / bs > c0 / bs + 1) why = WV_WHY_FAR_BLOCKS;
  }
  return why;
}

bool wv_plan_build(const QpPlan &pl, WvHost &wh, bool allow_links) {
  wh = WvHost();
  wh.why = WV_WHY_OTHER;
  const int n_c = pl.n_c, n_e = pl.n_e, m = pl.m;
  if (n_e <= 0 || n_c <= 0) return false;
  int hb = 0;
  for (int id = 0; id < pl.nS; id++) hb = std::max(hb, pl.s_a[id] - pl.s_b[id]);
  auto valid = [&](int bs) {
    if (bs <= 0 || bs > 8 || n_c % bs) return false;
    for (int id = 0; id < pl.nS; id++) {
      const int a = pl.s_a[id], b = pl.s_b[id], ta = a / bs, tb = b / bs;
      if (!(ta == tb || (ta == tb + 1 && a % bs == b % bs))) return false;
    }
    return true;
  };
  int bs = 0;
  if (valid(hb)) bs = hb; else if (valid(n_c)) bs = n_c; else { wh.why = wv_why_no_blocks(pl); return false; }
  const int nb = n_c / bs;
  for (int e = 0; e < n_e; e++) if (pl.Pdiag[pl.elim_var[e]] >= 0) return false;
  std::vector<int> h_of(n_e, -1), b_of(n_e, -1), hblk(n_e, -1);
  std::vector<std::vector<int>> single(n_c), link(n_c);
  for (int i = 0; i < m; i++) {
    int ne = 0, nc = 0, e = -1, blk = -1, c0 = -1, c1 = -1; bool one_blk = true;
    for (int s = pl.Rp[i]; s < pl.Rp[i + 1]; s++) {
      const int j = pl.Rj[s];
      if (pl.elim_of[j] >= 0) { ne++; e = pl.elim_of[j]; }
      else {
        const int c = pl.core_of[j], t = c / bs;
        if (nc && t != blk) one_blk = false;
        if (!nc) c0 = c1 = c; else { c0 = std::min(c0, c); c1 = std::max(c1, c); }
        blk = t; nc++;
      }
    }
    if (ne == 1 && nc >= 1 && one_blk) { if (h_of[e] >= 0) return false; h_of[e] = i; hblk[e] = blk; }
    else if (ne == 1 && nc == 0) { if (b_of[e] >= 0) return false; b_of[e] = i; }
    else if (ne == 0 && nc == 1) single[pl.core_of[pl.Rj[pl.Rp[i]]]].push_back(i);
    else if (ne == 0 && nc == 2) {
      if (one_blk) { wh.why = WV_WHY_SAME_BLOCK; return false; }
      if (c1 % bs != c0 % bs) { wh.why = WV_WHY_INDEX; return false; }
      if (c1 != c0 + bs) { wh.why = WV_WHY_FAR_BLOCKS; return false; }
      if (!allow_links) { wh.why = WV_WHY_LINKS_OFF; return false; }
      if ((int)link[c0].size() >= WV_NL) { wh.why = WV_WHY_THIRD_LINK; return false; }
      link[c0].push_back(i); wh.n_link++;
    }
    else { if (ne == 0 && nc >= 3) wh.why = WV_WHY_THREE_CORE; return false; }
  }
  wh.NL = wh.n_link > 0 ? WV_NL : 0;
  for (int e = 0; e < n_e; e++)
    if (h_of[e] < 0 || b_of[e] < 0 || pl.Ap[pl.elim_var[e] + 1] - pl.Ap[pl.elim_var[e]] != 2) return false;
  int n_extra = 0; bool plain = true;
  std::vector<int> xrow(n_c, -1);
  std::vector<std::vector<int>> stack(n_c);
  for (int c = 0; c < n_c; c++) { if (single[c].size() > 2) plain = false; if (single[c].size() == 2) n_extra++; }
  if (plain && n_extra <= WV_T) {
    for (int c = 0; c < n_c; c++) if (single[c].size() == 2) xrow[c] = single[c][0];
  } else {
    if (!allow_links) return false;
    int n_left = 0;
    for (int c = 0; c < n_c; c++) {
      const int k = (int)single[c].size(), free_slots = WV_NL - (int)link[c].size();
      if (k < 3) continue;
      if (k - 1 > free_slots + 1) { wh.why = WV_WHY_STACKED; return false; }
      const int ns = std::min(free_slots, k - 1);
      stack[c].assign(single[c].end() - 1 - ns, single[c].end() - 1);
      if (k - 1 > ns) { xrow[c] = single[c][0]; n_left++; }
    }
    if (n_left > WV_T) { wh.why = WV_WHY_STACKED; return false; }
    n_extra = n_left;
    for (int c = 0; c < n_c; c++) {
      if (single[c].size() != 2) continue;
      if (n_extra < WV_T) { xrow[c] = single[c][0]; n_extra++; }
      else if ((int)link[c].size() < WV_NL) stack[c].push_back(single[c][0]);
      else { wh.why = WV_WHY_STACKED; return false; }
    }
    for (int c = 0; c < n_c; c++) wh.n_stack += (int)stack[c].size();
  }
  wh.NL = wh.n_link + wh.n_stack > 0 ? WV_NL : 0;
  int lpb = 0;
  for (int L = 8; L >= 1; L--) if (nb <= 4 * (16 / L)) { lpb = L; break; }
  if (!lpb) return false;
  const int bpr = 16 / lpb;
  std::vector<std::vector<int>> hin(nb);
  for (int e = 0; e < n_e; e++) hin[hblk[e]].push_back(e);
  int maxh = 0;
  for (auto &v : hin) maxh = std::max(maxh, (int)v.size());
  const int NS = std::max(1, (maxh + lpb - 1) / lpb), NV = (bs + lpb - 1) / lpb;
  const int mid = nb / 2;
  if (NS <= 1 && NV <= 1 && mid <= 4) { wh.BS = 8; wh.NS = 1; wh.NV = 1; wh.NSTEP = 4; }
  else if (NS <= 2 && NV <= 2 && mid <= 8) { wh.BS = 8; wh.NS = 2; wh.NV = 2; wh.NSTEP = 8; }
  else if (NS <= 2 && NV <= 2 && mid <= 10) { wh.BS = 8; wh.NS = 2; wh.NV = 2; wh.NSTEP = 10; }
  else if (bs == 7 && NS <= 4 && NV <= 3 && mid <= 10) { wh.BS = 7; wh.NS = 4; wh.NV = 3; wh.NSTEP = 10; }
  else { wh.why = WV_WHY_SHAPE; return false; }
  wh.bs = bs; wh.nb = nb; wh.mid = mid; wh.lpb = lpb; wh.n_extra = n_extra;
  const int NSTEP = wh.NSTEP, lenB = nb - 1 - mid, npos = 2 * NSTEP + 2, dummy = npos - 1;
  auto pos_of = [&](int t) { return t < mid ? NSTEP - mid + t : t == mid ? NSTEP : 2 * NSTEP + 1 - lenB + (nb - 1 - t); };
  auto apos = [&](int row, int var) {
    for (int s = pl.Rp[row]; s < pl.Rp[row + 1]; s++) if (pl.Rj[s] == var) return pl.Rpos[s];
    return -1;
  };
  auto ppos = [&](int va, int vb) {
    const int r = std::min(va, vb), c = std::max(va, vb);
    for (int t = pl.Pp[c]; t < pl.Pp[c + 1]; t++) if (pl.Pi[t] == r) return t;
    return -1;
  };
  const WvTab T = wv_tab_layout(wh.NS, wh.NV, wh.NL);
  wh.tab.assign((size_t)T.total * 64, -1);
  auto at = [&](int off, int lane) -> int & { return wh.tab[(size_t)off * 64 + lane]; };
  for (int l = 0; l < 64; l++) {
    at(T.pos, l) = dummy;
    for (int v = 0; v < wh.NV; v++) { at(T.vpk + v, l) = wv_vidx(npos, dummy, v & 7); at(T.vpkm + v, l) = wv_vidx(npos, dummy, 0); at(T.vpkp + v, l) = wv_vidx(npos, dummy, 0); }
    at(T.xpk, l) = wv_vidx(npos, dummy, 0);
  }
  int xl = 0;
  for (int t = 0; t < nb; t++) {
    const int base = 16 * (t / bpr) + lpb * (t % bpr), p = pos_of(t);
    for (int sub = 0; sub < lpb; sub++) at(T.pos, base + sub) = p;
    for (int r = 0; r < (int)hin[t].size(); r++) {
      const int e = hin[t][r], l = base + r % lpb, q = r / lpb, ve = pl.elim_var[e];
      at(T.hrow + q, l) = h_of[e]; at(T.hbrow + q, l) = b_of[e]; at(T.hevar + q, l) = ve; at(T.heidx + q, l) = e;
      at(T.hepos + q, l) = apos(h_of[e], ve); at(T.hbpos + q, l) = apos(b_of[e], ve);
      for (int k = 0; k < bs; k++) at(T.hjpos + q * 8 + k, l) = apos(h_of[e], pl.core_var[t * bs + k]);
    }
    for (int k = 0; k < bs; k++) {
      const int l = base + k % lpb, v = k / lpb, c = t * bs + k, var = pl.core_var[c];
      at(T.vvar + v, l) = var; at(T.vpk + v, l) = wv_vidx(npos, p, k);
      at(T.vpkm + v, l) = t > 0 ? wv_vidx(npos, pos_of(t - 1), k) : wv_vidx(npos, dummy, 0);
      at(T.vpkp + v, l) = t + 1 < nb ? wv_vidx(npos, pos_of(t + 1), k) : wv_vidx(npos, dummy, 0);
      if (!single[c].empty()) { at(T.vrow + v, l) = single[c].back(); at(T.vpos + v, l) = apos(single[c].back(), var); }
      for (int k2 = 0; k2 < bs; k2++) at(T.vpd + v * 8 + k2, l) = ppos(var, pl.core_var[t * bs + k2]);
      at(T.vpm + v, l) = t > 0 ? ppos(var, pl.core_var[(t - 1) * bs + k]) : -1;
      at(T.vpp + v, l) = t + 1 < nb ? ppos(var, pl.core_var[(t + 1) * bs + k]) : -1;
      if (xrow[c] >= 0) { at(T.xrow, xl) = xrow[c]; at(T.xpos, xl) = apos(xrow[c], var); at(T.xpk, xl) = wv_vidx(npos, p, k); xl++; }
      const int nlk = (int)link[c].size();
      for (int s = 0; s < nlk; s++) {
        const int i = v * wh.NL + s, row = link[c][s];
        at(T.lrow + i, l) = row; at(T.lplo + i, l) = apos(row, var); at(T.lphi + i, l) = apos(row, pl.core_var[c + bs]);
      }
      for (int s = 0; s < (int)stack[c].size(); s++) {
        const int i = v * wh.NL + nlk + s, row = stack[c][s];
        at(T.lrow + i, l) = row; at(T.lplo + i, l) = apos(row, var); at(T.lphi + i, l) = -1;
      }
    }
  }
  const bool jreg = wv_jreg(wh.NS, wh.BS);
  wh.g_doubles = (size_t)npos * 64 + 2 * (size_t)npos * 8 + 8;
  wh.lds_doubles = wh.g_doubles + 4 * (size_t)npos * 8 + (jreg ? 0 : (size_t)wh.NS * 512) + (size_t)npos * lpb * 8 + (size_t)wv_ck_slots(wh.NS, wh.NV) * 64;
  wh.cst_slots = wv_cst_slots(wh.NS, wh.NV, 0);
  if (wh.NL) {
    const int nl = wh.NV * wh.NL;
    wh.lds_doubles += (size_t)npos * 8;
    if (!wv_link_regs(wh.BS)) wh.lds_doubles = wh.lds_doubles - (size_t)wv_ck_slots(wh.NS, wh.NV) * 64 + (size_t)nl * 4 * 64;
    wh.cst_slots = wv_cst_slots(wh.NS, wh.NV, nl);
  }
  wh.lds_bytes = wh.lds_doubles * sizeof(double);
  wh.per_cu = SCO_WV_PER_CU;
  const bool fits = wh.lds_bytes <= 40 * 1024;
  wh.why = fits ? WV_OK : WV_WHY_LDS;
  return fits;
}
```

Before: 6960.

## Specialize wave ADMM kernel on per-slot Jacobian row widths

Computes per-row nonzero widths for arm/spatial collision rows, where a row depends only on joints up to its point's link. The wave plan can sort rows within a block by width, and a compile-time width profile is chosen for each of the four row slots. FMAs on columns known to be zero are then skipped in the register-resident Jacobian loops. This adds kernel instantiations and a device check that flags a nonzero in a skipped column. It only applies to the BS=7/NS=4/lpb=3 shape without adaptive rho.

```diff
diff --git a/include/sco_hip.h b/include/sco_hip.h
--- a/include/sco_hip.h
+++ b/include/sco_hip.h
@@ -59,6 +59,8 @@
                 const int *row_weight);
 
 int sco_qp_set_bounds(sco_qp *qp, const double *l, const double *u);
+
+int sco_qp_set_row_widths(sco_qp *qp, const int *row_width);
 
 int sco_qp_solve(sco_qp *qp, const sco_qp_settings *settings,
                  double *x, double *y, int *status, int *iters, double *resid);
@@ -202,6 +204,9 @@
 
 int sco_debug_wv_gres_slot(int nstep, int pos, int out[5]);
 
+int sco_debug_wv_widths(const int *row_width, int info[12]);
+int sco_debug_sqp_row_widths(const sco_trajopt_desc *desc, const int *point_link, int *out);
+
 int sco_debug_sqp_schedule(const int in[12], int plan[20], const int round_in[3], int round_out[8]);
 int sco_debug_stage_sweep(int n, const double *begin_ms, const double *end_ms, const int *stage, double ms[5]);
 
diff --git a/sco_py_amd/_lib.py b/sco_py_amd/_lib.py
--- a/sco_py_amd/_lib.py
+++ b/sco_py_amd/_lib.py
@@ -65,6 +65,7 @@
     "sco_qp_destroy": (C.c_int, [C.c_void_p]),
     "sco_qp_load": (C.c_int, [C.c_void_p, _DP, _DP, _DP, _DP, _DP, _IP]),
     "sco_qp_set_bounds": (C.c_int, [C.c_void_p, _DP, _DP]),
+    "sco_qp_set_row_widths": (C.c_int, [C.c_void_p, _IP]),
     "sco_qp_solve": (C.c_int, [C.c_void_p, C.POINTER(QpSettings), _DP, _DP, _IP, _IP, _DP]),
     "sco_qp_info": (C.c_int, [C.c_void_p, _IP]),
     "sco_qp_adaptive_info": (C.c_int, [C.c_void_p, _DP, _IP]),
@@ -98,6 +99,8 @@
     "sco_debug_sqp_mixed": (C.c_int, [C.c_void_p, _IP]),
     "sco_debug_mix_split": (C.c_int, [C.c_int, C.c_int, C.c_int, C.c_int, C.c_int]),
     "sco_debug_wv_gres_slot": (C.c_int, [C.c_int, C.c_int, _IP]),
+    "sco_debug_wv_widths": (C.c_int, [_IP, _IP]),
+    "sco_debug_sqp_row_widths": (C.c_int, [C.POINTER(TrajoptDesc), _IP, _IP]),
     "sco_debug_sqp_schedule": (C.c_int, [_IP, _IP, _IP, _IP]),
     "sco_debug_stage_sweep": (C.c_int, [C.c_int, _DP, _DP, _IP, _DP]),
     "sco_debug_sqp_layout": (C.c_int, [C.POINTER(TrajoptDesc), C.c_int, _IP, _IP, _IP, _IP, _IP, _IP, _DP]),
@@ -224,6 +227,10 @@
         l = self._arr(l, (self.batch, self.m)); u = self._arr(u, (self.batch, self.m))
         check(load().sco_qp_set_bounds(self._h, dptr(l), dptr(u)))
 
+    def set_row_widths(self, row_width):
+        w = None if row_width is None else self._arr(row_width, (self.m,), np.int32)
+        check(load().sco_qp_set_row_widths(self._h, iptr(w)))
+
     def solve(self, settings=None):
         st = settings if settings is not None else default_qp_settings()
         B = self.batch
diff --git a/sco_py_amd/csrc/layout_wv.h b/sco_py_amd/csrc/layout_wv.h
--- a/sco_py_amd/csrc/layout_wv.h
+++ b/sco_py_amd/csrc/layout_wv.h
@@ -8,6 +8,12 @@
 #define WV_JREG 1
 #endif
 SCO_HD constexpr bool wv_jreg(int NS, int BS) { return WV_JREG && NS * BS <= 28; }
+
+#define WV_JW_PACK(a, b, c, d) ((a) | ((b) << 4) | ((c) << 8) | ((d) << 12))
+#define WV_JW_PROFILES(X) \
+  X(3, 5, 7, 7)       \
+  X(7, 6, 3, 2)
+SCO_HD constexpr int wv_jw(int JW, int q, int BS) { return JW ? (JW >> (4 * q)) & 15 : BS; }
 
 SCO_HD inline size_t wv_tri(int i, int j) { return (size_t)i * (i + 1) / 2 + j; }
 
diff --git a/sco_py_amd/csrc/qp_debug.cpp b/sco_py_amd/csrc/qp_debug.cpp
--- a/sco_py_amd/csrc/qp_debug.cpp
+++ b/sco_py_amd/csrc/qp_debug.cpp
@@ -59,6 +59,18 @@
   info[10] = wh.n_link; info[11] = wh.NL; info[12] = wh.per_cu; info[13] = wh.why; info[14] = wh.n_stack;
   return SCO_OK;
 }
+extern "C" int sco_debug_wv_widths(const int *row_width, int info[12]) {
+  if (!info) return SCO_ERR_ARG;
+  WvHost wh;
+  const QpCreateEnv env = qp_create_env();
+  const bool ok = wv_plan_build(g_dbg_plan, wh, true, env.wv_jsort && !env.wv_jw_off ? row_width : nullptr);
+  if (ok) wv_plan_widths(wh, row_width, env.wv_jw_off);
+  info[0] = ok ? 1 : 0;
+  for (int q = 0; q < 4; q++) info[1 + q] = wh.jw[q];
+  info[5] = wh.jw_profile; info[6] = (int)wh.lds_bytes; info[7] = wh.BS; info[8] = wh.NS; info[9] = wh.NV; info[10] = wh.NSTEP;
+  info[11] = wh.lpb;
+  return SCO_OK;
+}
 extern "C" int sco_debug_bt_plan(int *info) {
   BigHost bh; BtHost th;
   const bool ok = g_dbg_plan.n_c <= 1024 && big_plan_build(g_dbg_plan, bh) && bt_plan_build(g_dbg_plan, bh, th, qp_create_env().no_mfma);
diff --git a/sco_py_amd/csrc/qp_tier.cpp b/sco_py_amd/csrc/qp_tier.cpp
--- a/sco_py_amd/csrc/qp_tier.cpp
+++ b/sco_py_amd/csrc/qp_tier.cpp
@@ -14,6 +14,8 @@
   e.rl_closed = on("SCO_QP_RL_ALIGNED") || on("SCO_QP_RL_CLOSED"); e.rl_lay8 = on("SCO_QP_RL_LAY8");
   { const char *v = getenv("SCO_QP_RL_SPLIT"); e.rl_split_off = v && v[0] == '0'; }
   e.debug_plan = getenv("SCO_DEBUG_PLAN") != nullptr;
+  { const char *v = getenv("SCO_WV_JW"); e.wv_jw_off = v && v[0] == '0'; }
+  { const char *v = getenv("SCO_WV_JSORT"); e.wv_jsort = !(v && v[0] == '0'); }
   return e;
 }
 
diff --git a/sco_py_amd/csrc/qp_tier.h b/sco_py_amd/csrc/qp_tier.h
--- a/sco_py_amd/csrc/qp_tier.h
+++ b/sco_py_amd/csrc/qp_tier.h
@@ -14,6 +14,8 @@
   bool rl_lay8 = false;
   bool rl_split_off = false;
   bool debug_plan = false;
+  bool wv_jsort = true;
+  bool wv_jw_off = false;
 };
 QpCreateEnv qp_create_env();
 
diff --git a/sco_py_amd/csrc/qp_tier_plans.h b/sco_py_amd/csrc/qp_tier_plans.h
--- a/sco_py_amd/csrc/qp_tier_plans.h
+++ b/sco_py_amd/csrc/qp_tier_plans.h
@@ -55,12 +55,15 @@
   std::vector<int> tab;
   int n_link = 0, NL = 0, per_cu = SCO_WV_PER_CU, why = 0;
   int n_stack = 0;
+  int jw[4] = {0, 0, 0, 0}, jw_profile = 0;
+  bool jsorted = false;
 };
+void wv_plan_widths(WvHost &wh, const int *row_width, bool off);
 #define WV_NL 2
 enum WvWhy { WV_OK = 0, WV_WHY_OTHER = 1, WV_WHY_LINKS_OFF = 2, WV_WHY_THIRD_LINK = 3, WV_WHY_SAME_BLOCK = 4, WV_WHY_FAR_BLOCKS = 5,
              WV_WHY_INDEX = 6, WV_WHY_THREE_CORE = 7, WV_WHY_LDS = 8, WV_WHY_SHAPE = 9,
              WV_WHY_STACKED = 10 };
-bool wv_plan_build(const QpPlan &pl, WvHost &wh, bool allow_links);
+bool wv_plan_build(const QpPlan &pl, WvHost &wh, bool allow_links, const int *sort_width = nullptr);
 
 struct BigHost {
   std::vector<int> row_elim, row_epos, er_ptr, er_row, free_rows, pc_ptr, pc_pos, pc_core;
diff --git a/sco_py_amd/csrc/sco_admm_wv.hip b/sco_py_amd/csrc/sco_admm_wv.hip
--- a/sco_py_amd/csrc/sco_admm_wv.hip
+++ b/sco_py_amd/csrc/sco_admm_wv.hip
@@ -29,6 +29,9 @@
 #endif
 #ifndef WV_HANDOVER
 #define WV_HANDOVER 1
+#endif
+#ifndef WV_JWIDTH
+#define WV_JWIDTH 1
 #endif
 #if WV_VARIANT == 1
 #define WV_FMAC_DPP(acc, w, g, k) asm("v_fmac_f64 %0, %1, %2" : "+v"(acc) : "v"(w), "v"(g))
@@ -71,6 +74,7 @@
   double *sx, *sz, *sy, *st, *sg;
   int ablate;
   int warm, ad_interval; double ad_tol; double *rho_b; int *rflag, *smask, *nupd;
+  int jw;
 };
 
 __device__ __forceinline__ double wv_wmax(double v) { return wave_reduce_all<true>(v); }
@@ -113,6 +117,11 @@
       if (!(ls[h] < -WV_BIG) || rho[h] != rho_base || w[h] != wk) bad = 1;
       if (!(us[br] > WV_BIG) || ls[br] != 0.0 || rho[br] != rho_base || w[br] != 1) bad = 1;
       eh = E[h]; eb = E[br]; de = D[ev];
+      if (a.jw)
+        for (int k = wv_jw(a.jw, q, bs); k < bs; k++) {
+          const int jp = tab[(T.hjpos + q * 8 + k) * 64 + lane];
+          if (jp >= 0 && a.As[(size_t)b * a.nnzA + jp] != 0.0) bad = 1;
+        }
     }
     double *c = cst + (size_t)wv_cst_h(q) * 64 + lane;
     c[0] = h >= 0 ? 1.0 / eh : 0.0; c[64] = h >= 0 ? 1.0 / eb : 0.0; c[128] = h >= 0 ? 1.0 / de : 0.0;
@@ -284,9 +293,11 @@
   if (BS == 7 && LPB == 3 && EXT == 1) sl &= 4;
   return sl;
 }
-template <int BS, int NS, int NV, int NSTEP, int LPB, int EXT, int LNK>
+template <int BS, int NS, int NV, int NSTEP, int LPB, int EXT, int LNK, int JW>
 __global__ __launch_bounds__(WV_T) void qp_admm_wv_kernel(WvArgs a) {
   constexpr bool ADAPT = (EXT & 2) != 0;
+  static_assert(JW == 0 || (wv_jreg(NS, BS) && NS <= 4), "width profiles: Jacobian rows in registers, four slots");
+#define WV_COL(q, k) (JW == 0 || (k) < wv_jw(JW, q, BS))
   static_assert(!(LNK > 0 && ADAPT), "adaptive rho on link patterns stays on the row-local kernel (qp_launch_plan)");
   constexpr int NLK = LNK > 0 ? NV * LNK : 1;
   constexpr bool LREG = wv_link_regs(BS);
@@ -378,7 +389,7 @@
 #pragma unroll
     for (int k = 0; k < 4; k++) {
       const int j0 = on ? tab0[(oHJPOS + q * 8 + 2 * k) * 64 + lane] : -1, j1 = on ? tab0[(oHJPOS + q * 8 + 2 * k + 1) * 64 + lane] : -1;
-      d2 v; v.x = j0 >= 0 ? As[j0] : 0.0; v.y = j1 >= 0 ? As[j1] : 0.0;
+      d2 v; v.x = j0 >= 0 && WV_COL(q, 2 * k) ? As[j0] : 0.0; v.y = j1 >= 0 && WV_COL(q, 2 * k + 1) ? As[j1] : 0.0;
       if (JREG) { hJ[q][2 * k] = v.x; hJ[q][2 * k + 1] = v.y; }
       else *(d2 *)(jl_p + (q * 4 + k) * 128) = v;
     }
@@ -477,7 +488,7 @@
       if (MODE) {
         double s = J[0] * xt[0];
 #pragma unroll
-        for (int k = 1; k < BS; k++) s = __builtin_fma(J[k], xt[k], s);
+        for (int k = 1; k < BS; k++) if (WV_COL(q, k)) s = __builtin_fma(J[k], xt[k], s);
         const double xte = h_ge[q] - (kinv * c2) * s;
         const double zth = __builtin_fma(ae, xte, s), ztb = ab * xte;
         {
@@ -517,7 +528,7 @@
       h_ge[q] = ge;
       const double tp = th - c2 * ge;
 #pragma unroll
-      for (int k = 0; k < BS; k++) part[k] = __builtin_fma(J[k], tp, part[k]);
+      for (int k = 0; k < BS; k++) if (WV_COL(q, k)) part[k] = __builtin_fma(J[k], tp, part[k]);
     }
     {
       d2 v0, v1, v2, v3;
@@ -782,7 +793,7 @@
       }
       double s = J[0] * xc[0];
 #pragma unroll
-      for (int k = 1; k < BS; k++) s = __builtin_fma(J[k], xc[k], s);
+      for (int k = 1; k < BS; k++) if (WV_COL(q, k)) s = __builtin_fma(J[k], xc[k], s);
       if (h >= 0) {
         h_xe[q] = xg[ev] / Dg[ev];
         h_z[q] = s + h_ae[q] * h_xe[q]; h_zb[q] = h_ab[q] * h_xe[q];
@@ -832,7 +843,7 @@
           }
           double s = J[0] * xc[0];
 #pragma unroll
-          for (int k = 1; k < BS; k++) s = __builtin_fma(J[k], xc[k], s);
+          for (int k = 1; k < BS; k++) if (WV_COL(q, k)) s = __builtin_fma(J[k], xc[k], s);
           const double ax = s + h_ae[q] * h_xe[q], axb = h_ab[q] * h_xe[q];
           const double eh = CKH(q, 0), eb = CKH(q, 1), de = CKH(q, 2);
           w_pri = fmax(w_pri, fmax(eh * fabs(ax - h_z[q]), eb * fabs(axb - h_zb[q])));
@@ -847,7 +858,7 @@
             v_dua = fmax(v_dua, fabs(h_q[q] + aty)); v_dn = fmax(v_dn, fmax(fabs(h_q[q]), fabs(aty)));
           }
 #pragma unroll
-          for (int k = 0; k < BS; k++) part[k] = __builtin_fma(J[k], wy, part[k]);
+          for (int k = 0; k < BS; k++) if (WV_COL(q, k)) part[k] = __builtin_fma(J[k], wy, part[k]);
         }
         d2 v0, v1, v2, v3;
         v0.x = part[0]; v0.y = part[1]; v1.x = part[2]; v1.y = part[3]; v2.x = part[4]; v2.y = part[5]; v3.x = part[6]; v3.y = BS > 7 ? part[7] : 0.0;
@@ -942,7 +953,7 @@
             const double wd = wc * dsv.h[q];
             nat = fmax(nat, CKH(q, 2) * fabs(h_ae[q] * wd + h_ab[q] * dsv.b[q]));
 #pragma unroll
-            for (int k = 0; k < BS; k++) part[k] = __builtin_fma(J[k], wd, part[k]);
+            for (int k = 0; k < BS; k++) if (WV_COL(q, k)) part[k] = __builtin_fma(J[k], wd, part[k]);
           }
           d2 v0, v1, v2, v3;
           v0.x = part[0]; v0.y = part[1]; v1.x = part[2]; v1.y = part[3]; v2.x = part[4]; v2.y = part[5]; v3.x = part[6]; v3.y = BS > 7 ? part[7] : 0.0;
@@ -1022,7 +1033,7 @@
             }
             double s2 = J[0] * dxb[0];
 #pragma unroll
-            for (int k = 1; k < BS; k++) s2 = __builtin_fma(J[k], dxb[k], s2);
+            for (int k = 1; k < BS; k++) if (WV_COL(q, k)) s2 = __builtin_fma(J[k], dxb[k], s2);
             const double adh = CKH(q, 0) * (s2 + h_ae[q] * dsv.e[q]), adb = CKH(q, 1) * (h_ab[q] * dsv.e[q]);
             if (h_on[q] && ((h_u[q] < WV_BIG && adh > thr) || adb < -thr)) badv = 1.0;
           }
@@ -1127,6 +1138,11 @@
       atomicAdd(a.it_count, (unsigned long long)(iter - it0));
     }
   }
+}
+#undef WV_COL
+
+static int wv_launch_jw(const WvHost &wh, const AdmmArgs &aa) {
+  return (WV_JWIDTH != 0 && wv_jreg(wh.NS, wh.BS) && !aa.adaptive) ? wh.jw_profile : 0;
 }
 
 static void wv_fill_args(const AdmmArgs &aa, const WvHost &wh, const WvDev &wd, const int *setup_mask, WvArgs &a) {
@@ -1146,6 +1162,7 @@
   a.warm = aa.warm; a.ad_interval = aa.adaptive ? aa.ad_interval : 0; a.ad_tol = aa.ad_tol;
   a.rho_b = aa.adaptive ? d.rho_b : nullptr; a.rflag = aa.adaptive ? d.rflag : nullptr;
   a.smask = aa.adaptive ? d.smask : nullptr; a.nupd = aa.adaptive ? d.nupd : nullptr;
+  a.jw = wv_launch_jw(wh, aa);
 #ifdef WV_ABLATE
   { const char *ab = getenv("SCO_WV_ABLATE"); a.ablate = ab ? atoi(ab) : 0; }
 #else
@@ -1180,17 +1197,18 @@
   return SCO_OK;
 }
 
-template <int BS, int NS, int NV, int NSTEP, int LPB, int EXT, int LNK>
+template <int BS, int NS, int NV, int NSTEP, int LPB, int EXT, int LNK, int JW = 0>
 static int wv_launch_k(const WvArgs &a, int nwg, size_t lds, hipStream_t st) {
   static bool attr_done[64] = {};
-  SCO_LDS_ATTR((qp_admm_wv_kernel<BS, NS, NV, NSTEP, LPB, EXT, LNK>), 64 * 1024, attr_done);
-  hipLaunchKernelGGL((qp_admm_wv_kernel<BS, NS, NV, NSTEP, LPB, EXT, LNK>), dim3(nwg), dim3(WV_T), lds, st, a);
+  SCO_LDS_ATTR((qp_admm_wv_kernel<BS, NS, NV, NSTEP, LPB, EXT, LNK, JW>), 64 * 1024, attr_done);
+  hipLaunchKernelGGL((qp_admm_wv_kernel<BS, NS, NV, NSTEP, LPB, EXT, LNK, JW>), dim3(nwg), dim3(WV_T), lds, st, a);
   SCO_HIP(hipGetLastError());
   return SCO_OK;
 }
 
-template <int BS, int NS, int NV, int NSTEP, int LPB>
+template <int BS, int NS, int NV, int NSTEP, int LPB, int JW = 0>
 static int wv_launch_one(const WvArgs &a, int nwg, size_t lds, hipStream_t st) {
+  if constexpr (JW != 0) return a.warm ? wv_launch_k<BS, NS, NV, NSTEP, LPB, 1, 0, JW>(a, nwg, lds, st) : wv_launch_k<BS, NS, NV, NSTEP, LPB, 0, 0, JW>(a, nwg, lds, st);
   if (a.NL) {
     if (LPB > 0 || a.ad_interval > 0) { sco_set_error("wv_launch: no instantiation with link rows for this launch"); return SCO_ERR_STATE; }
     if constexpr (LPB == 0 && BS == 7) return wv_launch_k<BS, NS, NV, NSTEP, LPB, 1, WV_NL>(a, nwg, lds, st);
@@ -1204,7 +1222,19 @@
   WvArgs a; wv_fill_args(aa, wh, wd, nullptr, a);
   const int nwg = qp_launch_nwg(aa.d);
   const size_t lds = std::max(wh.lds_bytes, (size_t)36 * 1024);
-  if (wh.NSTEP == 10 && wh.NS == 4 && wh.lpb == 3 && !wh.NL) return wv_launch_one<7, 4, 3, 10, 3>(a, nwg, lds, st);
+  if (wh.NSTEP == 10 && wh.NS == 4 && wh.lpb == 3 && !wh.NL) {
+    if constexpr (wv_jreg(4, 7)) {
+      switch (a.jw) {
+#define X(w0, w1, w2, w3) case WV_JW_PACK(w0, w1, w2, w3): return wv_launch_one<7, 4, 3, 10, 3, WV_JW_PACK(w0, w1, w2, w3)>(a, nwg, lds, st);
+        WV_JW_PROFILES(X)
+#undef X
+        default: break;
+      }
+    }
+    if (a.jw) { sco_set_error("wv_launch: no instantiation of the plan's width profile"); return SCO_ERR_STATE; }
+    return wv_launch_one<7, 4, 3, 10, 3>(a, nwg, lds, st);
+  }
+  if (a.jw) { sco_set_error("wv_launch: no instantiation of the plan's width profile"); return SCO_ERR_STATE; }
   if (wh.NSTEP == 10 && wh.NS == 4) return wv_launch_one<7, 4, 3, 10, 0>(a, nwg, lds, st);
   if (wh.NSTEP == 10) return wv_launch_one<8, 2, 2, 10, 0>(a, nwg, lds, st);
   if (wh.NSTEP == 4) return wv_launch_one<8, 1, 1, 4, 0>(a, nwg, lds, st);
diff --git a/sco_py_amd/csrc/sco_qp.hip b/sco_py_amd/csrc/sco_qp.hip
--- a/sco_py_amd/csrc/sco_qp.hip
+++ b/sco_py_amd/csrc/sco_qp.hip
@@ -742,6 +742,24 @@
   return SCO_OK;
 }
 
+extern "C" int sco_qp_set_row_widths(sco_qp *qp, const int *row_width) {
+  if (!qp) { sco_set_error("sco_qp_set_row_widths: null pointer"); return SCO_ERR_ARG; }
+  if (!qp->use_wv) return SCO_OK;
+  const QpCreateEnv env = qp_create_env();
+  const bool sort = env.wv_jsort && !env.wv_jw_off && row_width;
+  if (sort || qp->wv.jsorted) {
+    WvHost nw;
+    if (wv_plan_build(qp->plan, nw, true, sort ? row_width : nullptr) && nw.tab.size() == qp->wv.tab.size()) {
+      SCO_ON_DEVICE(qp->device);
+      SCO_HIP(hipStreamSynchronize(qp->stream));
+      SCO_HIP(hipMemcpy((void *)qp->wvd.tab, nw.tab.data(), nw.tab.size() * sizeof(int), hipMemcpyHostToDevice));
+      qp->wv = nw;
+    }
+  }
+  wv_plan_widths(qp->wv, row_width, env.wv_jw_off);
+  return SCO_OK;
+}
+
 int sco_qp_launch(sco_qp *qp, const sco_qp_settings *st, const int *active_dev, hipEvent_t mid) {
   return sco_qp_launch_sliced(qp, st, active_dev, active_dev, 0, mid, nullptr);
 }
@@ -972,3 +990,4 @@
   if (!qp || !out) return SCO_ERR_ARG;
   return sco_qp_wv_iters(qp, out);
 }
+extern "C" int sco_debug_qp_wv_profile(const sco_qp *qp) { return qp && qp->use_wv ? qp->wv.jw_profile : 0; }
diff --git a/sco_py_amd/csrc/sco_sqp.hip b/sco_py_amd/csrc/sco_sqp.hip
--- a/sco_py_amd/csrc/sco_sqp.hip
+++ b/sco_py_amd/csrc/sco_sqp.hip
@@ -953,6 +953,11 @@
   SCO_HIP(hipMemcpyAsync((void *)s.point_link, point_link, s.K * sizeof(int), hipMemcpyHostToDevice, h->stream));
   SCO_HIP(hipMemcpyAsync((void *)s.point_frac, point_frac, s.K * sizeof(double), hipMemcpyHostToDevice, h->stream));
   SCO_HIP(hipStreamSynchronize(h->stream));
+  {
+    std::vector<int> w;
+    const bool hint = sqp_row_widths(s.point, s.S, s.d, s.O, s.R, s.NBt, s.m_lin, s.m, point_link, w);
+    if (int rc = sco_qp_set_row_widths(h->qp1, hint ? w.data() : nullptr)) return rc;
+  }
   h->loaded = true; h->solved = false;
   return SCO_OK;
 }
@@ -1667,6 +1672,16 @@
   }
   return SCO_OK;
 }
+extern "C" int sco_debug_sqp_row_widths(const sco_trajopt_desc *desc, const int *point_link, int *out) {
+  const char *err = "";
+  if (int rc = sqp_check_desc(desc, 0, nullptr, nullptr, nullptr, &err)) { sco_set_error(err); return rc; }
+  if (!point_link || !out) { sco_set_error("sco_debug_sqp_row_widths: null pointer"); return SCO_ERR_ARG; }
+  const SqpLayout L = sqp_layout_build(*desc, 0, nullptr, nullptr, nullptr);
+  std::vector<int> w;
+  const bool hint = sqp_row_widths(L.point, L.S, desc->dof, desc->n_obstacles, L.R, L.NBt, L.m_lin, L.m, point_link, w);
+  std::copy(w.begin(), w.end(), out);
+  return hint ? 1 : 0;
+}
 extern "C" int sco_debug_sqp_check_program(const sco_trajopt_desc *desc, int n_circle_rows, int n_words, const int *words,
                                            const int *row_ptr, int n_consts, int n_params) {
   const char *err = "";
diff --git a/sco_py_amd/csrc/sqp_layout.cpp b/sco_py_amd/csrc/sqp_layout.cpp
--- a/sco_py_amd/csrc/sqp_layout.cpp
+++ b/sco_py_amd/csrc/sqp_layout.cpp
@@ -165,6 +165,17 @@
   return L;
 }
 
+bool sqp_row_widths(int point, int S, int dof, int O, int R, int NBt, int m_lin, int m, const int *point_link, std::vector<int> &out) {
+  out.assign(m, 0);
+  if ((point != ROWS_ARM && point != ROWS_SPATIAL) || S != 1 || O <= 0 || !point_link) return false;
+  for (int blk = 0; blk < NBt; blk++)
+    for (int r = 0; r < R; r++) {
+      const int lk = point_link[r / O];
+      out[m_lin + blk * R + r] = (lk >= 0 && lk < dof) ? lk + 1 : 0;
+    }
+  return true;
+}
+
 int sqp_check_program(int n_prog_rows, int cost, int ds, int dof, int n_words, const int *words, const int *row_ptr,
                       int n_consts, int n_params, const char **err) {
   auto refuse = [&](const char *text) { *err = text; return SCO_ERR_ARG; };
diff --git a/sco_py_amd/csrc/sqp_layout.h b/sco_py_amd/csrc/sqp_layout.h
--- a/sco_py_amd/csrc/sqp_layout.h
+++ b/sco_py_amd/csrc/sqp_layout.h
@@ -39,5 +39,7 @@
 };
 SqpLayout sqp_layout_build(const sco_trajopt_desc &desc, int m_gen, const int *gen_ptr, const int *gen_col, const int *gen_iseq);
 
+bool sqp_row_widths(int point, int S, int dof, int O, int R, int NBt, int m_lin, int m, const int *point_link, std::vector<int> &out);
+
 int sqp_check_program(int n_prog_rows, int cost, int ds, int dof, int n_words, const int *words, const int *row_ptr,
                       int n_consts, int n_params, const char **err);
diff --git a/sco_py_amd/csrc/sqp_rows.h b/sco_py_amd/csrc/sqp_rows.h
--- a/sco_py_amd/csrc/sqp_rows.h
+++ b/sco_py_amd/csrc/sqp_rows.h
@@ -293,6 +293,7 @@
   }
   return arm_row_grad(th, c.len, c.point_link[kp], c.point_frac[kp], c.obs[3 * o], c.obs[3 * o + 1], j);
 }
+
 __device__ __forceinline__ bool row_ignores(const RowCtx &c, const RowRef &q, int j) {
   return c.point == ROWS_SPATIAL && j > c.point_link[q.r / c.O];
 }
diff --git a/sco_py_amd/csrc/wv_plan.cpp b/sco_py_amd/csrc/wv_plan.cpp
--- a/sco_py_amd/csrc/wv_plan.cpp
+++ b/sco_py_amd/csrc/wv_plan.cpp
@@ -31,7 +31,7 @@
   return why;
 }
 
-bool wv_plan_build(const QpPlan &pl, WvHost &wh, bool allow_links) {
+bool wv_plan_build(const QpPlan &pl, WvHost &wh, bool allow_links, const int *sort_width) {
   wh = WvHost();
   wh.why = WV_WHY_OTHER;
   const int n_c = pl.n_c, n_e = pl.n_e, m = pl.m;
@@ -114,6 +114,11 @@
   const int bpr = 16 / lpb;
   std::vector<std::vector<int>> hin(nb);
   for (int e = 0; e < n_e; e++) hin[hblk[e]].push_back(e);
+  if (sort_width) {
+    auto width = [&](int e) { const int w = sort_width[h_of[e]]; return (w > 0 && w < bs) ? w : bs; };
+    for (auto &v : hin) std::stable_sort(v.begin(), v.end(), [&](int a, int b) { return width(a) > width(b); });
+    wh.jsorted = true;
+  }
   int maxh = 0;
   for (auto &v : hin) maxh = std::max(maxh, (int)v.size());
   const int NS = std::max(1, (maxh + lpb - 1) / lpb), NV = (bs + lpb - 1) / lpb;
@@ -188,5 +193,30 @@
   wh.per_cu = SCO_WV_PER_CU;
   const bool fits = wh.lds_bytes <= 40 * 1024;
   wh.why = fits ? WV_OK : WV_WHY_LDS;
+  wv_plan_widths(wh, nullptr, false);
   return fits;
 }
+
+void wv_plan_widths(WvHost &wh, const int *row_width, bool off) {
+  const WvTab T = wv_tab_layout(wh.NS, wh.NV, wh.NL);
+  wh.jw_profile = 0;
+  for (int q = 0; q < WV_MAXNS; q++) wh.jw[q] = 0;
+  if (wh.tab.size() < (size_t)T.total * 64) return;
+  for (int q = 0; q < wh.NS && q < WV_MAXNS; q++)
+    for (int l = 0; l < 64; l++) {
+      const int h = wh.tab[(size_t)(T.hrow + q) * 64 + l];
+      if (h < 0) continue;
+      const int w = row_width ? row_width[h] : 0;
+      wh.jw[q] = std::max(wh.jw[q], (w > 0 && w < wh.bs) ? w : wh.bs);
+    }
+  if (off || !row_width) return;
+  if (!(wh.BS == 7 && wh.NS == 4 && wh.NSTEP == 10 && wh.lpb == 3 && !wh.NL) || !wv_jreg(wh.NS, wh.BS)) return;
+  int best = 0, best_cols = 4 * wh.BS;
+#define X(a, b, c, d) \
+  if (wh.jw[0] <= (a) && wh.jw[1] <= (b) && wh.jw[2] <= (c) && wh.jw[3] <= (d) && (a) + (b) + (c) + (d) < best_cols) { \
+    best = WV_JW_PACK(a, b, c, d); best_cols = (a) + (b) + (c) + (d); \
+  }
+  WV_JW_PROFILES(X)
+#undef X
+  wh.jw_profile = best;
+}
```

Result: faster. 7213, median of 6 (+3.6%).
